# ddemidov/amgcl

Hardware: NVIDIA H100
Metric: cg_iterations_per_second (higher is better)
Workload: dtype f64

## Files before the change

### amgcl_b200/__init__.py

```python
import ctypes
import os

import numpy as np

from . import build as _build

__all__ = ["lib", "dropin_lib", "Context", "Vector", "Csr", "Coarse", "Krylov", "DropinSolver",
           "poisson3d", "unstructured3d", "B200Error", "RELAX", "KRYLOV", "nccl_unique_id",
           "partition", "dist_split", "coarse_lu_plan"]

_c = ctypes
_i64 = _c.c_int64
_dbl = _c.c_double
_vp = _c.c_void_p
_P = _c.POINTER

RELAX = {"damped_jacobi": 0, "spai0": 1, "chebyshev": 2, "ilu0": 3}
KRYLOV = {"cg": 0, "bicgstab": 1, "gmres": 2, "bicgstabl": 3}


class B200Error(RuntimeError):
    pass


class ProfileEntry(_c.Structure):
    _fields_ = [("nrows", _i64), ("ncols", _i64), ("nnz", _i64), ("mode", _c.c_int),
                ("launches", _i64), ("total_ms", _dbl), ("min_ms", _dbl)]


class ProfileFormatEntry(_c.Structure):
    _fields_ = [("entry", ProfileEntry), ("format", _c.c_int), ("value_bytes", _c.c_int)]


FORMAT_NAMES = ("plain", "window", "offset", "pattern", "col16", "col24")


MODE_NAMES = {0: "spmv", 1: "spmv_acc", 2: "residual", 3: "relax", 4: "residual_scaled", 10: "vec1", 11: "vec2",
              12: "vec3", 13: "vec4", 14: "vec5", 15: "vec6", 16: "vec7",
              20: "dot", 21: "relax_zero", 22: "coarse_gemv", 23: "memset", 24: "coarse_tail", 25: "coarse_lu",
              30: "comm"}


_lib = None
_dropin = None


def lib():
    global _lib
    if _lib is not None:
        return _lib
    path = os.environ.get("B200_LIB") or _build.LIB_CUDA
    if not os.path.isfile(path):
        path = _build.build_cuda()
    L = _c.CDLL(path, mode=_c.RTLD_GLOBAL)
    L.b200_last_error.restype = _c.c_char_p
    L.b200_version.restype = _c.c_char_p
    sigs = {
        "b200_device_count": [],
        "b200_ctx_create": [_c.c_int, _P(_vp)],
        "b200_ctx_destroy": [_vp],
        "b200_ctx_default": [_P(_vp)],
        "b200_ctx_set_stream": [_vp, _vp],
        "b200_ctx_get_stream": [_vp, _P(_vp)],
        "b200_ctx_device": [_vp, _P(_c.c_int)],
        "b200_ctx_sync": [_vp],
        "b200_ctx_flush": [_vp],
        "b200_tail_stats": [_vp, _P(_c.c_uint64), _P(_c.c_uint64)],
        "b200_ctx_launch_count": [_vp, _P(_c.c_uint64)],
        "b200_ctx_reset_launch_count": [_vp],
        "b200_ctx_set_option": [_vp, _c.c_char_p, _i64],
        "b200_ctx_get_option": [_vp, _c.c_char_p, _P(_i64)],
        "b200_vec_create": [_vp, _c.c_size_t, _P(_vp)],
        "b200_vec_wrap": [_vp, _vp, _c.c_size_t, _P(_vp)],
        "b200_vec_destroy": [_vp],
        "b200_vec_size": [_vp, _P(_c.c_size_t)],
        "b200_vec_bytes": [_vp, _P(_c.c_size_t)],
        "b200_vec_data": [_vp, _P(_vp)],
        "b200_vec_upload": [_vp, _vp, _c.c_size_t],
        "b200_vec_download": [_vp, _vp, _c.c_size_t],
        "b200_vec_download_local": [_vp, _vp, _c.c_size_t],
        "b200_vec_local_range": [_vp, _P(_c.c_size_t), _P(_c.c_size_t)],
        "b200_vec_create_f32": [_vp, _c.c_size_t, _P(_vp)],
        "b200_vec_upload_f32": [_vp, _vp, _c.c_size_t],
        "b200_vec_download_f32": [_vp, _vp, _c.c_size_t],
        "b200_vec_dtype": [_vp, _P(_c.c_int)],
        "b200_csr_create_i64_f32": [_vp, _i64, _i64, _vp, _vp, _vp, _P(_vp)],
        "b200_csr_create_i32_f32": [_vp, _i64, _i64, _vp, _vp, _vp, _P(_vp)],
        "b200_csr_dtype": [_vp, _P(_c.c_int)],
        "b200_coarse_create_i64_f32": [_vp, _i64, _vp, _vp, _vp, _P(_vp)],
        "b200_coarse_create_i32_f32": [_vp, _i64, _vp, _vp, _vp, _P(_vp)],
        "b200_csr_create_i64": [_vp, _i64, _i64, _vp, _vp, _vp, _P(_vp)],
        "b200_csr_create_i32": [_vp, _i64, _i64, _vp, _vp, _vp, _P(_vp)],
        "b200_csr_destroy": [_vp],
        "b200_csr_rows": [_vp, _P(_c.c_size_t)],
        "b200_csr_cols": [_vp, _P(_c.c_size_t)],
        "b200_csr_nonzeros": [_vp, _P(_c.c_size_t)],
        "b200_csr_bytes": [_vp, _P(_c.c_size_t)],
        "b200_csr_plan": [_vp, _P(_c.c_int), _P(_i64), _P(_i64)],
        "b200_spmv": [_vp, _dbl, _vp, _vp, _dbl, _vp],
        "b200_residual": [_vp, _vp, _vp, _vp, _vp],
        "b200_clear": [_vp, _vp],
        "b200_copy": [_vp, _vp, _vp],
        "b200_dot": [_vp, _vp, _vp, _P(_dbl)],
        "b200_axpby": [_vp, _dbl, _vp, _dbl, _vp],
        "b200_axpbypcz": [_vp, _dbl, _vp, _dbl, _vp, _dbl, _vp],
        "b200_vmul": [_vp, _dbl, _vp, _vp, _dbl, _vp],
        "b200_relax": [_vp, _vp, _vp, _vp, _vp, _vp, _dbl],
        "b200_coarse_create_i64": [_vp, _i64, _vp, _vp, _vp, _P(_vp)],
        "b200_coarse_create_i32": [_vp, _i64, _vp, _vp, _vp, _P(_vp)],
        "b200_coarse_destroy": [_vp],
        "b200_coarse_bytes": [_vp, _P(_c.c_size_t)],
        "b200_coarse_info": [_vp, _P(_c.c_int), _P(_i64), _P(_i64), _P(_i64)],
        "b200_coarse_lu_plan_i64": [_i64, _vp, _vp, _vp, _vp, _vp, _vp, _vp, _i64, _P(_i64), _P(_c.c_int),
                                    _P(_i64), _P(_c.c_size_t), _P(_c.c_size_t)],
        "b200_coarse_solve": [_vp, _vp, _vp, _vp],
        "b200_nccl_unique_id": [_c.c_char_p, _c.c_size_t],
        "b200_dist_init": [_vp, _c.c_char_p, _c.c_size_t, _c.c_int, _c.c_int, _i64],
        "b200_dist_info": [_vp, _P(_c.c_int), _P(_c.c_int), _P(_i64), _P(_c.c_int)],
        "b200_partition": [_i64, _c.c_int, _c.c_int, _P(_i64), _P(_i64), _P(_i64)],
        "b200_dist_split_i64": [_c.c_int, _c.c_int, _c.c_int, _i64, _i64, _vp, _vp, _vp, _P(_vp)],
        "b200_split_info": [_vp, _P(_i64), _P(_i64), _P(_i64), _P(_i64), _P(_i64), _P(_i64)],
        "b200_split_copy": [_vp, _vp, _vp, _vp, _vp],
        "b200_split_destroy": [_vp],
        "b200_plan_i64": [_i64, _vp, _c.c_int, _c.c_int, _vp, _i64, _P(_i64), _P(_c.c_int),
                          _P(_c.c_int), _P(_i64)],
        "b200_ctx_largest_operator": [_vp, _P(_i64), _P(_c.c_int)],
        "b200_csr_patterns": [_vp, _P(_c.c_int), _P(_c.c_int), _P(_c.c_int)],
        "b200_pattern_plan_i64": [_i64, _i64, _vp, _vp, _vp, _vp, _vp, _P(_c.c_int), _P(_c.c_int), _P(_c.c_int)],
        "b200_csr_offsets": [_vp, _P(_c.c_int), _P(_c.c_int)],
        "b200_offset_plan_i64": [_i64, _i64, _vp, _vp, _vp, _vp, _P(_c.c_int), _P(_c.c_int)],
        "b200_csr_narrow": [_vp, _P(_c.c_int)],
        "b200_csr_value_bytes": [_vp, _P(_c.c_int)],
        "b200_values_fit_f32": [_vp, _i64, _P(_c.c_int)],
        "b200_value_index_plan_i64": [_vp, _i64, _vp, _i64, _vp, _P(_c.c_int), _P(_c.c_int)],
        "b200_narrow_plan_i64": [_i64, _i64, _vp, _vp, _c.c_int, _c.c_int, _vp, _i64, _vp, _vp, _vp,
                                 _P(_i64), _P(_c.c_int)],
        "b200_csr_window": [_vp, _P(_c.c_int), _P(_c.c_int), _P(_c.c_int), _P(_i64)],
        "b200_window_plan_i64": [_i64, _i64, _vp, _vp, _c.c_int, _c.c_int, _c.c_int, _c.c_int, _c.c_int, _vp, _vp, _i64,
                                 _vp, _i64, _P(_i64), _P(_i64), _P(_c.c_int), _P(_c.c_int), _P(_c.c_int)],
        "b200_index_create_i64": [_vp, _vp, _c.c_size_t, _c.c_size_t, _P(_vp)],
        "b200_index_destroy": [_vp],
        "b200_index_size": [_vp, _P(_c.c_size_t)],
        "b200_gather": [_vp, _vp, _vp, _vp],
        "b200_gather_host": [_vp, _vp, _vp, _vp],
        "b200_scatter": [_vp, _vp, _vp, _vp],
        "b200_graph_begin": [_vp, _P(_c.c_int)],
        "b200_graph_end": [_vp, _P(_vp)],
        "b200_graph_abort": [_vp],
        "b200_graph_launch": [_vp, _vp, _P(_c.c_int)],
        "b200_graph_info": [_vp, _P(_i64), _P(_i64), _P(_i64), _P(_c.c_int)],
        "b200_graph_destroy": [_vp],
        "b200_krylov_create": [_vp, _c.c_size_t, _P(_vp)],
        "b200_krylov_destroy": [_vp],
        "b200_krylov_residual": [_vp, _vp, _vp, _vp, _vp, _P(_dbl)],
        "b200_krylov_scalars": [_vp, _vp, _c.c_int],
        "b200_cg_direction": [_vp, _vp, _vp, _vp],
        "b200_cg_step": [_vp, _vp, _vp, _vp, _vp, _vp, _P(_dbl)],
        "b200_bicg_start": [_vp, _vp, _vp],
        "b200_bicg_direction": [_vp, _vp, _vp, _vp],
        "b200_bicg_step_s": [_vp, _vp, _vp, _vp, _vp, _vp, _vp, _vp, _P(_dbl), _P(_dbl)],
        "b200_bicg_step_r": [_vp, _vp, _vp, _vp, _vp, _vp, _vp, _vp, _P(_dbl), _P(_dbl)],
        "b200_profile_begin": [_vp],
        "b200_profile_end": [_vp, _vp, _i64, _P(_i64)],
        "b200_profile_end_formats": [_vp, _vp, _i64, _P(_i64)],
    }
    for name, args in sigs.items():
        fn = getattr(L, name)
        fn.argtypes = args
        fn.restype = _c.c_int
    _lib = L
    return L


def dropin_lib():
    global _dropin
    if _dropin is not None:
        return _dropin
    lib()
    path = _build.LIB_DROPIN
    if not os.path.isfile(path):
        path = _build.build_dropin()
    D = _c.CDLL(path)
    D.dropin_last_error.restype = _c.c_char_p
    D.dropin_create.argtypes = [_vp, _i64, _vp, _vp, _vp, _c.c_int, _c.c_int, _dbl, _c.c_int,
                                _c.c_int, _P(_vp)]
    D.dropin_create.restype = _c.c_int
    D.dropin_create_mixed.argtypes = D.dropin_create.argtypes
    D.dropin_create_mixed.restype = _c.c_int
    D.dropin_create_graph.argtypes = [_vp, _i64, _vp, _vp, _vp, _c.c_int, _c.c_int, _c.c_int, _dbl,
                                      _c.c_int, _c.c_int, _P(_vp)]
    D.dropin_create_graph.restype = _c.c_int
    D.dropin_graph_stats.argtypes = [_vp, _P(_i64), _P(_i64), _P(_i64)]
    D.dropin_graph_stats.restype = _c.c_int
    D.dropin_gather_scatter.argtypes = [_vp, _i64, _vp, _i64, _vp, _dbl, _vp, _vp, _vp]
    D.dropin_gather_scatter.restype = _c.c_int
    D.dropin_destroy.argtypes = [_vp]
    D.dropin_destroy.restype = None
    D.dropin_solve.argtypes = [_vp, _vp, _vp, _P(_i64), _P(_dbl)]
    D.dropin_solve.restype = _c.c_int
    D.dropin_solve_zero_guess.argtypes = [_vp, _vp, _vp, _P(_i64), _P(_dbl)]
    D.dropin_solve_zero_guess.restype = _c.c_int
    D.dropin_upload_rhs.argtypes = [_vp, _vp]
    D.dropin_upload_rhs.restype = _c.c_int
    D.dropin_solve_resident.argtypes = [_vp, _P(_i64), _P(_dbl)]
    D.dropin_solve_resident.restype = _c.c_int
    D.dropin_download_x.argtypes = [_vp, _vp]
    D.dropin_download_x.restype = _c.c_int
    D.dropin_apply_precond.argtypes = [_vp, _vp, _vp]
    D.dropin_apply_precond.restype = _c.c_int
    D.dropin_report.argtypes = [_vp, _c.c_char_p, _i64]
    D.dropin_report.restype = _i64
    D.dropin_bytes.argtypes = [_vp]
    D.dropin_bytes.restype = _i64
    D.dropin_set_num_threads.argtypes = [_c.c_int]
    D.dropin_set_num_threads.restype = None
    D.dropin_num_threads.restype = _c.c_int
    _dropin = D
    return D


def _check(rc, what=""):
    if rc != 0:
        msg = lib().b200_last_error().decode(errors="replace")
        raise B200Error("%s failed (%d): %s" % (what or "b200 call", rc, msg))


def _f64(a):
    a = np.ascontiguousarray(a, dtype=np.float64)
    return a


def _ptr(a):
    return a.ctypes.data_as(_vp)


class Context:

    def __init__(self, device=0, stream=None):
        L = lib()
        if L.b200_device_count() <= 0:
            raise B200Error("amgcl_b200 requires a CUDA device (no CPU fallback)")
        self.h = _vp()
        _check(L.b200_ctx_create(int(device), _c.byref(self.h)), "b200_ctx_create")
        if stream is not None:
            self.set_stream(stream)

    def set_stream(self, cuda_stream):
        if cuda_stream is None:
            handle = 0
        else:
            handle = int(cuda_stream) or 1
        _check(lib().b200_ctx_set_stream(self.h, _vp(handle)))

    def sync(self):
        _check(lib().b200_ctx_sync(self.h), "b200_ctx_sync")

    def flush(self):
        _check(lib().b200_ctx_flush(self.h), "b200_ctx_flush")

    def tail_stats(self):
        f, c = _c.c_uint64(), _c.c_uint64()
        _check(lib().b200_tail_stats(self.h, _c.byref(f), _c.byref(c)))
        return f.value, c.value

    def set_option(self, key, value):
        _check(lib().b200_ctx_set_option(self.h, key.encode(), int(value)), "b200_ctx_set_option")

    def get_option(self, key):
        v = _i64()
        _check(lib().b200_ctx_get_option(self.h, key.encode(), _c.byref(v)))
        return v.value

    @property
    def launches(self):
        v = _c.c_uint64()
        _check(lib().b200_ctx_launch_count(self.h, _c.byref(v)))
        return v.value

    def reset_launches(self):
        _check(lib().b200_ctx_reset_launch_count(self.h))

    def dist_init(self, unique_id, nranks, rank, dist_min_rows):
        buf = _c.create_string_buffer(bytes(unique_id), 128)
        _check(lib().b200_dist_init(self.h, buf, 128, int(nranks), int(rank), int(dist_min_rows)),
               "b200_dist_init")

    def dist_info(self):
        r, n, p = _c.c_int(), _c.c_int(), _c.c_int()
        m = _i64()
        _check(lib().b200_dist_info(self.h, _c.byref(r), _c.byref(n), _c.byref(m), _c.byref(p)))
        return {"rank": r.value, "nranks": n.value, "dist_min_rows": m.value, "p2p": bool(p.value)}

    def largest_operator(self):
        nnz, fmt = _i64(), _c.c_int()
        _check(lib().b200_ctx_largest_operator(self.h, _c.byref(nnz), _c.byref(fmt)))
        return nnz.value, FORMAT_NAMES[fmt.value]

    def profile_begin(self):
        _check(lib().b200_profile_begin(self.h), "b200_profile_begin")

    def profile_end(self):
        cap = 256
        buf = (ProfileFormatEntry * cap)()
        cnt = _i64()
        _check(lib().b200_profile_end_formats(self.h, buf, cap, _c.byref(cnt)), "b200_profile_end_formats")
        out = []
        for i in range(min(cap, cnt.value)):
            e, fmt, vb = buf[i].entry, buf[i].format, buf[i].value_bytes
            out.append({"nrows": e.nrows, "ncols": e.ncols, "nnz": e.nnz,
                        "mode": MODE_NAMES.get(e.mode, str(e.mode)), "launches": e.launches,
                        "total_ms": e.total_ms, "min_ms": e.min_ms, "format": FORMAT_NAMES[fmt],
                        "value_bytes": vb})
        return out

    def close(self):
        if self.h:
            lib().b200_ctx_destroy(self.h)
            self.h = _vp()

    def vector(self, data_or_n):
        return Vector(self, data_or_n)

    def csr(self, nrows, ncols, ptr, col, val):
        return Csr(self, nrows, ncols, ptr, col, val)

    def coarse(self, n, ptr, col, val):
        return Coarse(self, n, ptr, col, val)

    def spmv(self, alpha, A, x, beta, y):
        _check(lib().b200_spmv(self.h, alpha, A.h, x.h, beta, y.h), "b200_spmv")

    def residual(self, f, A, x, r):
        _check(lib().b200_residual(self.h, f.h, A.h, x.h, r.h), "b200_residual")

    def clear(self, x):
        _check(lib().b200_clear(self.h, x.h), "b200_clear")

    def copy(self, x, y):
        _check(lib().b200_copy(self.h, x.h, y.h), "b200_copy")

    def dot(self, x, y):
        r = _dbl()
        _check(lib().b200_dot(self.h, x.h, y.h, _c.byref(r)), "b200_dot")
        return r.value

    def axpby(self, a, x, b, y):
        _check(lib().b200_axpby(self.h, a, x.h, b, y.h), "b200_axpby")

    def axpbypcz(self, a, x, b, y, c, z):
        _check(lib().b200_axpbypcz(self.h, a, x.h, b, y.h, c, z.h), "b200_axpbypcz")

    def vmul(self, alpha, x, y, beta, z):
        _check(lib().b200_vmul(self.h, alpha, x.h, y.h, beta, z.h), "b200_vmul")

    def index(self, idx, size):
        return Index(self, idx, size)

    def gather(self, I, src, dst):
        _check(lib().b200_gather(self.h, I.h, src.h, dst.h), "b200_gather")

    def gather_host(self, I, src):
        out = np.empty(I.n, dtype=np.float64)
        _check(lib().b200_gather_host(self.h, I.h, src.h, _ptr(out)), "b200_gather_host")
        return out

    def scatter(self, I, src, dst):
        _check(lib().b200_scatter(self.h, I.h, src.h, dst.h), "b200_scatter")

    def graph_begin(self):
        rec = _c.c_int(0)
        _check(lib().b200_graph_begin(self.h, _c.byref(rec)), "b200_graph_begin")
        return bool(rec.value)

    def graph_end(self):
        g = _vp()
        _check(lib().b200_graph_end(self.h, _c.byref(g)), "b200_graph_end")
        return Graph(self, g)

    def graph_abort(self):
        _check(lib().b200_graph_abort(self.h), "b200_graph_abort")

    def relax(self, A, rhs, x, tmp, diag, omega):
        _check(lib().b200_relax(self.h, A.h, rhs.h, x.h, tmp.h, diag.h, omega), "b200_relax")

    def coarse_solve(self, S, rhs, x):
        _check(lib().b200_coarse_solve(self.h, S.h, rhs.h, x.h), "b200_coarse_solve")


class Krylov:

    SCALARS = ("rho", "qp", "alpha", "ts", "tt", "omega", "rr", "ss", "rho_next")

    def __init__(self, ctx, n):
        self.ctx = ctx
        self.h = _vp()
        _check(lib().b200_krylov_create(ctx.h, int(n), _c.byref(self.h)), "b200_krylov_create")

    def residual(self, rhs, A, x, r):
        out = _dbl()
        _check(lib().b200_krylov_residual(self.h, rhs.h, A.h, x.h, r.h, _c.byref(out)), "b200_krylov_residual")
        return out.value

    def scalars(self):
        buf = (_dbl * 9)()
        _check(lib().b200_krylov_scalars(self.h, buf, 9), "b200_krylov_scalars")
        return dict(zip(self.SCALARS, list(buf)))

    def cg_direction(self, r, s, p):
        _check(lib().b200_cg_direction(self.h, r.h, s.h, p.h), "b200_cg_direction")

    def cg_step(self, A, p, q, x, r):
        out = _dbl()
        _check(lib().b200_cg_step(self.h, A.h, p.h, q.h, x.h, r.h, _c.byref(out)), "b200_cg_step")
        return out.value

    def bicg_start(self, r, rh):
        _check(lib().b200_bicg_start(self.h, r.h, rh.h), "b200_bicg_start")

    def bicg_direction(self, r, v, p):
        _check(lib().b200_bicg_direction(self.h, r.h, v.h, p.h), "b200_bicg_direction")

    def bicg_step_s(self, A, rh, T, v, r, s, x):
        out = _dbl()
        _check(lib().b200_bicg_step_s(self.h, A.h, rh.h, T.h, v.h, r.h, s.h, x.h, _c.byref(out), None),
               "b200_bicg_step_s")
        return out.value

    def bicg_step_r(self, A, rh, T, t, s, r, x):
        out = _dbl()
        _check(lib().b200_bicg_step_r(self.h, A.h, rh.h, T.h, t.h, s.h, r.h, x.h, _c.byref(out), None),
               "b200_bicg_step_r")
        return out.value

    def close(self):
        if self.h:
            lib().b200_krylov_destroy(self.h)
            self.h = _vp()

    def __del__(self):
        try:
            self.close()
        except Exception:
            pass


class Vector:

    def __init__(self, ctx, data_or_n):
        self.ctx = ctx
        self.h = _vp()
        if isinstance(data_or_n, (int, np.integer)):
            self.n = int(data_or_n)
            _check(lib().b200_vec_create(ctx.h, self.n, _c.byref(self.h)), "b200_vec_create")
        else:
            a = _f64(data_or_n)
            self.n = a.size
            _check(lib().b200_vec_create(ctx.h, self.n, _c.byref(self.h)), "b200_vec_create")
            self.upload(a)

    def upload(self, a):
        a = _f64(a)
        _check(lib().b200_vec_upload(self.h, _ptr(a), a.size), "b200_vec_upload")

    def numpy(self):
        out = np.empty(self.n, dtype=np.float64)
        _check(lib().b200_vec_download(self.h, _ptr(out), self.n), "b200_vec_download")
        return out

    def data_ptr(self):
        p = _vp()
        _check(lib().b200_vec_data(self.h, _c.byref(p)))
        return p.value or 0

    def __del__(self):
        try:
            if self.h:
                lib().b200_vec_destroy(self.h)
                self.h = _vp()
        except Exception:
            pass


class Csr:

    def __init__(self, ctx, nrows, ncols, ptr, col, val):
        self.ctx = ctx
        self.h = _vp()
        val = _f64(val)
        ptr = np.ascontiguousarray(ptr)
        col = np.ascontiguousarray(col)
        if ptr.dtype == np.int32 and col.dtype == np.int32:
            fn = lib().b200_csr_create_i32
        else:
            ptr = np.ascontiguousarray(ptr, dtype=np.int64)
            col = np.ascontiguousarray(col, dtype=np.int64)
            fn = lib().b200_csr_create_i64
        _check(fn(ctx.h, int(nrows), int(ncols), _ptr(ptr), _ptr(col), _ptr(val),
                  _c.byref(self.h)), "b200_csr_create")
        self.nrows, self.ncols, self.nnz = int(nrows), int(ncols), int(ptr[-1])

    def plan(self):
        lanes = _c.c_int()
        nb = _i64()
        nl = _i64()
        _check(lib().b200_csr_plan(self.h, _c.byref(lanes), _c.byref(nb), _c.byref(nl)))
        return {"lanes": lanes.value, "blocks": nb.value, "long_blocks": nl.value}

    def bytes(self):
        b = _c.c_size_t()
        _check(lib().b200_csr_bytes(self.h, _c.byref(b)))
        return b.value

    def patterns(self):
        on, cnt, tot = _c.c_int(), _c.c_int(), _c.c_int()
        _check(lib().b200_csr_patterns(self.h, _c.byref(on), _c.byref(cnt), _c.byref(tot)))
        return {"pattern_indexed": bool(on.value), "count": cnt.value, "total": tot.value}

    def offsets(self):
        on, cnt = _c.c_int(), _c.c_int()
        _check(lib().b200_csr_offsets(self.h, _c.byref(on), _c.byref(cnt)))
        return {"offset_indexed": bool(on.value), "count": cnt.value}

    def narrow(self):
        w = _c.c_int()
        _check(lib().b200_csr_narrow(self.h, _c.byref(w)))
        return w.value

    def value_bytes(self):
        b = _c.c_int()
        _check(lib().b200_csr_value_bytes(self.h, _c.byref(b)))
        return b.value

    def window(self):
        w, ms, mr, tot = _c.c_int(), _c.c_int(), _c.c_int(), _i64()
        _check(lib().b200_csr_window(self.h, _c.byref(w), _c.byref(ms), _c.byref(mr), _c.byref(tot)))
        return {"windowed": bool(w.value), "max_slots": ms.value, "max_runs": mr.value, "total_slots": tot.value}

    def __del__(self):
        try:
            if self.h and lib().b200_csr_destroy(self.h) == 0:
                self.h = _vp()
        except Exception:
            pass


def pattern_plan(nrows, ncols, ptr, col):
    ptr = np.ascontiguousarray(ptr, dtype=np.int64)
    col = np.ascontiguousarray(col, dtype=np.int64)
    pid = np.zeros(max(1, nrows), dtype=np.uint8)
    start = np.zeros(257, dtype=np.uint16)
    off = np.zeros(1024, dtype=np.int32)
    cnt, tot, ok = _c.c_int(), _c.c_int(), _c.c_int()
    _check(lib().b200_pattern_plan_i64(nrows, ncols, ptr.ctypes.data, col.ctypes.data, pid.ctypes.data,
                                       start.ctypes.data, off.ctypes.data, _c.byref(cnt), _c.byref(tot),
                                       _c.byref(ok)))
    if not ok.value:
        return None
    return {"pid": pid[:nrows], "start": start, "off": off, "count": cnt.value, "total": tot.value}


def offset_plan(nrows, ncols, ptr, col):
    ptr = np.ascontiguousarray(ptr, dtype=np.int64)
    col = np.ascontiguousarray(col, dtype=np.int64)
    nnz = int(ptr[-1]) if nrows else 0
    idx8 = np.zeros(max(1, nnz), dtype=np.uint8)
    tab = np.zeros(256, dtype=np.int32)
    cnt, ok = _c.c_int(), _c.c_int()
    _check(lib().b200_offset_plan_i64(nrows, ncols, ptr.ctypes.data, col.ctypes.data, idx8.ctypes.data,
                                      tab.ctypes.data, _c.byref(cnt), _c.byref(ok)))
    if not ok.value:
        return None
    return {"idx8": idx8[:nnz], "tab": tab, "count": cnt.value}


def narrow_plan(nrows, ncols, ptr, col, lanes=0, nnz_cap=2048):
    ptr = np.ascontiguousarray(ptr, dtype=np.int64)
    col = np.ascontiguousarray(col, dtype=np.int64)
    nnz = int(ptr[-1]) if nrows else 0
    cap = nrows // 4 + 2 + (nnz // 256 + 1)
    base = np.zeros(cap, dtype=np.int32)
    lo16 = np.zeros(max(1, nnz), dtype=np.uint16)
    hi8 = np.zeros(max(1, nnz), dtype=np.uint8)
    ptr16 = np.zeros(max(1, nrows), dtype=np.uint16)
    nb, w = _i64(), _c.c_int()
    _check(lib().b200_narrow_plan_i64(nrows, ncols, ptr.ctypes.data, col.ctypes.data, int(lanes), int(nnz_cap),
                                      base.ctypes.data, cap, lo16.ctypes.data, hi8.ctypes.data,
                                      ptr16.ctypes.data, _c.byref(nb), _c.byref(w)))
    out = {"nblocks": nb.value, "ptr16": ptr16[:nrows], "width": w.value}
    if w.value:
        out.update(base=base[:nb.value], lo16=lo16[:nnz])
        if w.value == 24:
            out["hi8"] = hi8[:nnz]
    return out


def values_fit_f32(val):
    val = np.ascontiguousarray(val, dtype=np.float64)
    ok = _c.c_int()
    _check(lib().b200_values_fit_f32(val.ctypes.data, val.size, _c.byref(ok)))
    return bool(ok.value)


def value_index_plan(val):
    val = np.ascontiguousarray(val, dtype=np.float64)
    tab = np.zeros(4096, dtype=np.float64)
    idx = np.zeros(max(1, 2 * val.size), dtype=np.uint8)
    cnt, w = _c.c_int(), _c.c_int()
    _check(lib().b200_value_index_plan_i64(val.ctypes.data, val.size, tab.ctypes.data, tab.size,
                                            idx.ctypes.data, _c.byref(cnt), _c.byref(w)))
    out = {"width": w.value, "count": cnt.value}
    if w.value:
        out["table"] = tab[:cnt.value]
        out["index"] = idx[:val.size] if w.value == 8 else idx[:2 * val.size].view(np.uint16)
    return out


def window_plan(nrows, ncols, ptr, col, lanes=0, nnz_cap=2048, slot_cap=1400, max_ratio=75, gap=2):
    ptr = np.ascontiguousarray(ptr, dtype=np.int64)
    col = np.ascontiguousarray(col, dtype=np.int64)
    nnz = int(ptr[-1]) if nrows else 0
    nb, nr = _i64(), _i64()
    ms, mr, ok = _c.c_int(), _c.c_int(), _c.c_int()
    L = lib()
    _check(L.b200_window_plan_i64(nrows, ncols, ptr.ctypes.data, col.ctypes.data, lanes, nnz_cap, slot_cap,
                                  max_ratio, gap, None, None, 0, None, 0, _c.byref(nb), _c.byref(nr),
                                  _c.byref(ms), _c.byref(mr), _c.byref(ok)))
    if not ok.value:
        return None
    blk = np.zeros((nb.value, 6), dtype=np.int32)
    runs = np.zeros((max(1, nr.value), 2), dtype=np.int32)
    col16 = np.zeros(max(1, nnz), dtype=np.uint16)
    _check(L.b200_window_plan_i64(nrows, ncols, ptr.ctypes.data, col.ctypes.data, lanes, nnz_cap, slot_cap,
                                  max_ratio, gap, col16.ctypes.data, runs.ctypes.data, runs.shape[0],
                                  blk.ctypes.data, blk.shape[0], _c.byref(nb), _c.byref(nr),
                                  _c.byref(ms), _c.byref(mr), _c.byref(ok)))
    return {"blk": blk, "runs": runs[:nr.value], "col16": col16[:nnz], "max_slots": ms.value,
            "max_runs": mr.value}


def coarse_lu_plan(n, ptr, col):
    L = lib()
    n = int(n)
    ptr = np.ascontiguousarray(ptr, dtype=np.int64)
    col = np.ascontiguousarray(col, dtype=np.int64)
    tiles, rows, bw = _i64(), _c.c_int(), _i64()
    fb, sb = _c.c_size_t(), _c.c_size_t()
    _check(L.b200_coarse_lu_plan_i64(n, _ptr(ptr), _ptr(col), None, None, None, None, None, 0,
                                     _c.byref(tiles), _c.byref(rows), _c.byref(bw), _c.byref(fb),
                                     _c.byref(sb)), "b200_coarse_lu_plan_i64")
    perm = np.empty(n, dtype=np.int32)
    lower = np.empty(n, dtype=np.int32)
    upper = np.empty(n, dtype=np.int32)
    lfirst = np.empty(tiles.value, dtype=np.int64)
    ulast = np.empty(tiles.value, dtype=np.int64)
    _check(L.b200_coarse_lu_plan_i64(n, _ptr(ptr), _ptr(col), _ptr(perm), _ptr(lower), _ptr(upper),
                                     _ptr(lfirst), _ptr(ulast), tiles.value, None, None, None, None, None),
           "b200_coarse_lu_plan_i64")
    return {"perm": perm, "lower": lower, "upper": upper, "lfirst": lfirst, "ulast": ulast,
            "tile_rows": rows.value, "bandwidth": bw.value, "factor_bytes": fb.value,
            "setup_bytes": sb.value}


class Coarse:

    def __init__(self, ctx, n, ptr, col, val):
        self.ctx = ctx
        self.h = _vp()
        ptr = np.ascontiguousarray(ptr, dtype=np.int64)
        col = np.ascontiguousarray(col, dtype=np.int64)
        val = _f64(val)
        _check(lib().b200_coarse_create_i64(ctx.h, int(n), _ptr(ptr), _ptr(col), _ptr(val),
                                            _c.byref(self.h)), "b200_coarse_create")
        self.n = int(n)

    COARSE_KINDS = ("dense_inverse", "banded_lu")

    def info(self):
        k, n, bw, t = _c.c_int(), _i64(), _i64(), _i64()
        _check(lib().b200_coarse_info(self.h, _c.byref(k), _c.byref(n), _c.byref(bw), _c.byref(t)),
               "b200_coarse_info")
        return {"kind": self.COARSE_KINDS[k.value], "n": n.value, "bandwidth": bw.value, "tiles": t.value}

    def bytes(self):
        b = _c.c_size_t()
        _check(lib().b200_coarse_bytes(self.h, _c.byref(b)), "b200_coarse_bytes")
        return b.value

    def __del__(self):
        try:
            if self.h and lib().b200_coarse_destroy(self.h) == 0:
                self.h = _vp()
        except Exception:
            pass


class Index:

    def __init__(self, ctx, idx, size):
        idx = np.ascontiguousarray(idx, dtype=np.int64)
        self.ctx = ctx
        self.n = idx.size
        self.h = _vp()
        _check(lib().b200_index_create_i64(ctx.h, _ptr(idx), idx.size, int(size), _c.byref(self.h)),
               "b200_index_create_i64")

    def __del__(self):
        try:
            if self.h and lib().b200_index_destroy(self.h) == 0:
                self.h = _vp()
        except Exception:
            pass


class Graph:

    def __init__(self, ctx, h):
        self.ctx = ctx
        self.h = h

    def launch(self):
        ok = _c.c_int(0)
        _check(lib().b200_graph_launch(self.ctx.h, self.h, _c.byref(ok)), "b200_graph_launch")
        return bool(ok.value)

    def info(self):
        k, n, r, st = _i64(), _i64(), _i64(), _c.c_int(0)
        _check(lib().b200_graph_info(self.h, _c.byref(k), _c.byref(n), _c.byref(r), _c.byref(st)))
        return {"kernels": k.value, "nodes": n.value, "replays": r.value, "stale": bool(st.value)}

    def close(self):
        if self.h:
            lib().b200_graph_destroy(self.h)
            self.h = _vp()

    def __del__(self):
        try:
            self.close()
        except Exception:
            pass


class DropinSolver:

    def __init__(self, ptr, col, val, relax="damped_jacobi", krylov="cg", tol=1e-8,
                 maxiter=100, coarse_enough=-1, ctx=None, precision="f64", graph=False):
        D = dropin_lib()
        self.ptr = np.ascontiguousarray(ptr, dtype=np.int64)
        self.col = np.ascontiguousarray(col, dtype=np.int64)
        self.val = _f64(val)
        self.n = self.ptr.size - 1
        self.ctx = ctx
        self.h = _vp()
        if graph:
            rc = D.dropin_create_graph(ctx.h if ctx is not None else None, self.n, _ptr(self.ptr),
                                       _ptr(self.col), _ptr(self.val), RELAX[relax], KRYLOV[krylov],
                                       1 if precision == "mixed" else 0, float(tol), int(maxiter),
                                       int(coarse_enough), _c.byref(self.h))
        else:
            create = D.dropin_create_mixed if precision == "mixed" else D.dropin_create
            rc = create(ctx.h if ctx is not None else None, self.n, _ptr(self.ptr),
                        _ptr(self.col), _ptr(self.val), RELAX[relax], KRYLOV[krylov],
                        float(tol), int(maxiter), int(coarse_enough), _c.byref(self.h))
        if rc != 0:
            raise B200Error("dropin_create: " + D.dropin_last_error().decode(errors="replace"))

    def _err(self, what):
        raise B200Error(what + ": " + dropin_lib().dropin_last_error().decode(errors="replace"))

    def solve(self, rhs, x0=None):
        rhs = _f64(rhs)
        x = np.zeros(self.n) if x0 is None else _f64(x0).copy()
        it = _i64()
        res = _dbl()
        if dropin_lib().dropin_solve(self.h, _ptr(rhs), _ptr(x), _c.byref(it), _c.byref(res)):
            self._err("dropin_solve")
        return x, it.value, res.value

    def solve_into(self, rhs, x):
        it = _i64()
        res = _dbl()
        if dropin_lib().dropin_solve(self.h, _ptr(rhs), _ptr(x), _c.byref(it), _c.byref(res)):
            self._err("dropin_solve")
        return it.value, res.value

    def solve_zero_guess_into(self, rhs, x_out):
        it = _i64()
        res = _dbl()
        if dropin_lib().dropin_solve_zero_guess(self.h, _ptr(rhs), _ptr(x_out), _c.byref(it),
                                                _c.byref(res)):
            self._err("dropin_solve_zero_guess")
        return it.value, res.value

    def upload_rhs(self, rhs):
        rhs = _f64(rhs)
        if dropin_lib().dropin_upload_rhs(self.h, _ptr(rhs)):
            self._err("dropin_upload_rhs")

    def solve_resident(self):
        it = _i64()
        res = _dbl()
        if dropin_lib().dropin_solve_resident(self.h, _c.byref(it), _c.byref(res)):
            self._err("dropin_solve_resident")
        return it.value, res.value

    def download_x(self):
        x = np.empty(self.n)
        if dropin_lib().dropin_download_x(self.h, _ptr(x)):
            self._err("dropin_download_x")
        return x

    def apply_precond(self, f):
        f = _f64(f)
        x = np.empty(self.n)
        if dropin_lib().dropin_apply_precond(self.h, _ptr(f), _ptr(x)):
            self._err("dropin_apply_precond")
        return x

    def graph_stats(self):
        g, k, r = _i64(), _i64(), _i64()
        dropin_lib().dropin_graph_stats(self.h, _c.byref(g), _c.byref(k), _c.byref(r))
        return g.value, k.value, r.value

    def report(self):
        need = dropin_lib().dropin_report(self.h, None, 0)
        buf = _c.create_string_buffer(int(need))
        dropin_lib().dropin_report(self.h, buf, need)
        return buf.value.decode(errors="replace")

    def close(self):
        if self.h:
            dropin_lib().dropin_destroy(self.h)
            self.h = _vp()

    def __del__(self):
        try:
            self.close()
        except Exception:
            pass


def set_setup_threads(n):
    dropin_lib().dropin_set_num_threads(int(n))


def nccl_unique_id():
    buf = _c.create_string_buffer(128)
    _check(lib().b200_nccl_unique_id(buf, 128), "b200_nccl_unique_id")
    return bytes(buf.raw)


def partition(n, nranks, rank):
    b, lo, hi = _i64(), _i64(), _i64()
    _check(lib().b200_partition(int(n), int(nranks), int(rank), _c.byref(b), _c.byref(lo),
                                _c.byref(hi)), "b200_partition")
    return b.value, lo.value, hi.value


def dist_split(kind, nranks, rank, nrows, ncols, ptr, col, val):
    k = {"halo": 1, "square": 1, "replicated": 2}[kind]
    ptr = np.ascontiguousarray(ptr, dtype=np.int64)
    col = np.ascontiguousarray(col, dtype=np.int64)
    val = _f64(val)
    h = _vp()
# ... 82 lines not shown
```

### amgcl_b200/csrc/api_context.cu

```cuda
#include "internal.cuh"

#include <mutex>

namespace b200 {

static thread_local std::string g_last_error;

void set_error(const std::string &msg) { g_last_error = msg; }

int fail(int code, const std::string &msg) {
    g_last_error = msg;
    return code;
}

int cuda_fail(cudaError_t rc, const char *what, const char *file, int line) {
    char buf[512];
    snprintf(buf, sizeof(buf), "CUDA error %d (%s) in %s at %s:%d", (int)rc,
             cudaGetErrorString(rc), what, file, line);
    g_last_error = buf;
    cudaGetLastError();
    return rc == cudaErrorMemoryAllocation ? B200_ENOMEM : B200_ECUDA;
}

}

using namespace b200;

extern "C" const char *b200_last_error(void) { return g_last_error.c_str(); }

extern "C" const char *b200_version(void) { return "amgcl_b200 0.1.0 sm_90a"; }

extern "C" int b200_device_count(void) {
    int n = 0;
    if (cudaGetDeviceCount(&n) != cudaSuccess) {
        cudaGetLastError();
        return 0;
    }
    return n;
}

static int ctx_init(b200_ctx_t ctx, int device) {
    cudaDeviceProp prop;
    B200_CUDA(cudaGetDeviceProperties(&prop, device));
    ctx->sm_count = prop.multiProcessorCount;
    if (prop.major != 9 || prop.minor != 0)
        return fail(B200_ECUDA, "amgcl_b200 needs an sm_90a (Hopper H100) device");
    B200_CUDA(cudaStreamCreateWithFlags(&ctx->own_stream, cudaStreamNonBlocking));
    ctx->stream = ctx->own_stream;
    B200_CUDA(cudaMalloc(&ctx->dot_partial, kDotMaxBlocks * sizeof(double)));
    B200_CUDA(cudaMalloc(&ctx->dot_ticket, sizeof(unsigned int)));
    B200_CUDA(cudaMemset(ctx->dot_ticket, 0, sizeof(unsigned int)));
    B200_CUDA(cudaHostAlloc(&ctx->dot_result_h, 8 * sizeof(double), cudaHostAllocMapped));
    B200_CUDA(cudaHostGetDevicePointer(&ctx->dot_result_d, ctx->dot_result_h, 0));
    B200_CUDA(cudaMalloc(&ctx->dot_dev, 2 * sizeof(double)));
    return scal_create(ctx);
}

extern "C" int b200_ctx_create(int device, b200_ctx_t *out) {
    B200_REQUIRE(out != nullptr, "null output pointer");
    *out = nullptr;
    int ndev = 0;
    B200_CUDA(cudaGetDeviceCount(&ndev));
    if (device < 0 || device >= ndev) return fail(B200_EINVAL, "no such CUDA device");
    DeviceGuard guard(device);
    if (!guard.ok) return fail(B200_ECUDA, "cudaSetDevice failed");

    b200_ctx_s *ctx = new (std::nothrow) b200_ctx_s();
    if (!ctx) return fail(B200_ENOMEM, "out of host memory");
    ctx->device = device;
    if (const char *e = getenv("B200_PDL")) ctx->opt_pdl = atoi(e) ? 1 : 0;
    if (const char *e = getenv("B200_CYCLE_GRAPH")) ctx->opt_cycle_graph = atoi(e) ? 1 : 0;
    if (const char *e = getenv("B200_GRAPH_PDL")) ctx->opt_graph_pdl = atoi(e) ? 1 : 0;
    if (const char *e = getenv("B200_FUSED_KRYLOV")) ctx->opt_fused_krylov = atoi(e) ? 1 : 0;
    if (const char *e = getenv("B200_COARSE_TAIL")) ctx->opt_coarse_tail = atoi(e) ? 1 : 0;
    if (const char *e = getenv("B200_FUSE_FIRST_SWEEP")) ctx->opt_fuse_first_sweep = atoi(e) ? 1 : 0;
    if (const char *e = getenv("B200_POLL_SCALARS")) ctx->opt_poll_scalars = atoi(e) ? 1 : 0;
    if (const char *e = getenv("B200_PATTERNS")) ctx->opt_patterns = atoi(e) ? 1 : 0;
    if (const char *e = getenv("B200_PATTERNS_MIN_NNZ")) ctx->opt_patterns_min_nnz = atoll(e);
    if (const char *e = getenv("B200_OFFSETS")) ctx->opt_offsets = atoi(e) ? 1 : 0;
    if (const char *e = getenv("B200_OFFSETS_MIN_NNZ")) ctx->opt_offsets_min_nnz = atoll(e);
    if (const char *e = getenv("B200_NARROW_COLUMNS")) ctx->opt_narrow = atoi(e) ? 1 : 0;
    if (const char *e = getenv("B200_NARROW_VALUES")) ctx->opt_narrow_values = atoi(e) ? 1 : 0;
    if (const char *e = getenv("B200_WINDOW")) ctx->opt_window = atoi(e) ? 1 : 0;
    if (const char *e = getenv("B200_WINDOW_MIN_NNZ")) ctx->opt_window_min_nnz = atoll(e);
    if (const char *e = getenv("B200_WINDOW_GAP")) ctx->opt_window_gap = std::max(1, std::min(8, atoi(e)));
    if (const char *e = getenv("B200_WINDOW_RATIO")) ctx->opt_window_ratio = atoll(e);
    if (const char *e = getenv("B200_WINDOW_LANES")) ctx->opt_window_lanes = atoll(e) & 15;
    if (const char *e = getenv("B200_SMALL_KERNEL_MAX_NNZ")) ctx->opt_small_kernel_max_nnz = atoll(e);
    const int rc = ctx_init(ctx, device);
    if (rc != B200_OK) {
        const std::string msg = g_last_error;
        b200_ctx_destroy(ctx);
        g_last_error = msg;
        return rc;
    }
    *out = ctx;
    return B200_OK;
}

extern "C" int b200_ctx_destroy(b200_ctx_t ctx) {
    if (!ctx) return B200_OK;
    tail_destroy(ctx);
    ctx->lazy_vec = nullptr;
    GUARD(ctx);
    if (ctx->stream) cudaStreamSynchronize(ctx->stream);
    scal_destroy(ctx);
    tail_destroy(ctx);
    for (int k = 0; k < 2; ++k) {
        if (ctx->stage_host[k]) cudaFreeHost(ctx->stage_host[k]);
        if (ctx->stage_event[k]) cudaEventDestroy(ctx->stage_event[k]);
    }
    if (ctx->gather_ticket) cudaFree(ctx->gather_ticket);
    if (ctx->scal_x_local) {
        for (int q = 0; q < ctx->nranks; ++q)
            if (q != ctx->rank && ctx->scal_x_peer[q]) cudaIpcCloseMemHandle(ctx->scal_x_peer[q]);
        cudaFree(ctx->scal_x_local);
    }
    if (ctx->dot_partial) cudaFree(ctx->dot_partial);
    if (ctx->dot_ticket) cudaFree(ctx->dot_ticket);
    if (ctx->dot_result_h) cudaFreeHost(ctx->dot_result_h);
    if (ctx->dot_dev) cudaFree(ctx->dot_dev);
    if (ctx->push_ticket) cudaFree(ctx->push_ticket);
    if (ctx->ipc_dev) cudaFree(ctx->ipc_dev);
    if (ctx->probe_pb_local) {
        for (int q = 0; q < ctx->nranks; ++q)
            if (q != ctx->rank && ctx->probe_pb_peer[q]) cudaIpcCloseMemHandle(ctx->probe_pb_peer[q]);
        cudaFree(ctx->probe_pb_local);
    }
    for (void *ptr : ctx->deferred_free) cudaFree(ptr);
    if (ctx->comm && nccl().handle) nccl().CommDestroy(comm_of(ctx));
    if (ctx->own_stream) cudaStreamDestroy(ctx->own_stream);
    for (cudaEvent_t e : ctx->prof_events) cudaEventDestroy(e);
    delete ctx;
    return B200_OK;
}

extern "C" int b200_ctx_default(b200_ctx_t *out) {
    B200_REQUIRE(out != nullptr, "null output pointer");
    static std::mutex mtx;
    static b200_ctx_t def = nullptr;
    std::lock_guard<std::mutex> lock(mtx);
    if (!def) {
        int dev = 0;
        B200_CUDA(cudaGetDevice(&dev));
        int rc = b200_ctx_create(dev, &def);
        if (rc != B200_OK) return rc;
    }
    *out = def;
    return B200_OK;
}

extern "C" int b200_ctx_set_stream(b200_ctx_t ctx, void *cuda_stream) {
    CHECK_CTX(ctx);
    NOT_RECORDING(ctx, "stream change");
    {
        GUARD(ctx);
    }
    ctx->option_epoch++;
    ctx->stream = cuda_stream ? static_cast<cudaStream_t>(cuda_stream) : ctx->own_stream;
    return B200_OK;
}

extern "C" int b200_ctx_get_stream(b200_ctx_t ctx, void **cuda_stream) {
    CHECK_CTX(ctx);
    B200_REQUIRE(cuda_stream != nullptr, "null output pointer");
    *cuda_stream = ctx->stream;
    return B200_OK;
}

extern "C" int b200_ctx_device(b200_ctx_t ctx, int *device) {
    CHECK_CTX(ctx);
    B200_REQUIRE(device != nullptr, "null output pointer");
    *device = ctx->device;
    return B200_OK;
}

extern "C" int b200_ctx_sync(b200_ctx_t ctx) {
    CHECK_CTX(ctx);
    NOT_RECORDING(ctx, "sync");
    GUARD(ctx);
    B200_CUDA(cudaStreamSynchronize(ctx->stream));
    return B200_OK;
}

extern "C" int b200_ctx_flush(b200_ctx_t ctx) {
    CHECK_CTX(ctx);
    GUARD(ctx);
    return B200_OK;
}

extern "C" int b200_ctx_launch_count(b200_ctx_t ctx, uint64_t *count) {
    CHECK_CTX(ctx);
    B200_REQUIRE(count != nullptr, "null output pointer");
    *count = ctx->launches;
    return B200_OK;
}

extern "C" int b200_ctx_reset_launch_count(b200_ctx_t ctx) {
    CHECK_CTX(ctx);
    ctx->launches = 0;
    return B200_OK;
}

extern "C" int b200_profile_begin(b200_ctx_t ctx) {
    CHECK_CTX(ctx);
    NOT_RECORDING(ctx, "profiling");
    {
        GUARD(ctx);
    }
    ctx->prof_used = 0;
    ctx->prof_recs.clear();
    ctx->profiling = true;
    return B200_OK;
}

static int profile_collect(b200_ctx_t ctx, std::vector<b200_profile_format_entry> &agg) {
    GUARD(ctx);
    ctx->profiling = false;
    B200_CUDA(cudaStreamSynchronize(ctx->stream));
    for (const auto &r : ctx->prof_recs) {
        float ms = 0.f;
        B200_CUDA(cudaEventElapsedTime(&ms, ctx->prof_events[r.ev], ctx->prof_events[r.ev + 1]));
        b200_profile_format_entry *hit = nullptr;
        for (auto &a : agg)
            if (a.entry.nrows == r.nrows && a.entry.ncols == r.ncols && a.entry.nnz == r.nnz &&
                a.entry.mode == r.mode && a.format == r.fmt && a.value_bytes == r.vbytes) {
                hit = &a;
                break;
            }
        if (!hit) {
            agg.push_back({{r.nrows, r.ncols, r.nnz, r.mode, 0, 0.0, 1e30}, r.fmt, r.vbytes});
            hit = &agg.back();
        }
        hit->entry.launches += 1;
        hit->entry.total_ms += ms;
        if (ms < hit->entry.min_ms) hit->entry.min_ms = ms;
    }
    ctx->prof_recs.clear();
    ctx->prof_used = 0;
    return B200_OK;
}

extern "C" int b200_profile_end(b200_ctx_t ctx, b200_profile_entry *out, int64_t capacity,
                                int64_t *count) {
    CHECK_CTX(ctx);
    B200_REQUIRE(count != nullptr, "null output pointer");
    std::vector<b200_profile_format_entry> agg;
    const int rc = profile_collect(ctx, agg);
    if (rc) return rc;
    *count = (int64_t)agg.size();
    if (out) {
        const int64_t m = std::min<int64_t>(capacity, (int64_t)agg.size());
        for (int64_t i = 0; i < m; ++i) out[i] = agg[(size_t)i].entry;
    }
    return B200_OK;
}

extern "C" int b200_profile_end_formats(b200_ctx_t ctx, b200_profile_format_entry *out, int64_t capacity,
                                        int64_t *count) {
    CHECK_CTX(ctx);
    B200_REQUIRE(count != nullptr, "null output pointer");
    std::vector<b200_profile_format_entry> agg;
    const int rc = profile_collect(ctx, agg);
    if (rc) return rc;
    *count = (int64_t)agg.size();
    if (out) {
        const int64_t m = std::min<int64_t>(capacity, (int64_t)agg.size());
        for (int64_t i = 0; i < m; ++i) out[i] = agg[(size_t)i];
    }
    return B200_OK;
}


static int64_t *option_slot(b200_ctx_t ctx, const char *key) {
    if (!key) return nullptr;
    if (!strcmp(key, "spmv_variant")) return &ctx->opt_spmv_variant;
    if (!strcmp(key, "fuse_relax")) return &ctx->opt_fuse_relax;
    if (!strcmp(key, "zero_shortcut")) return &ctx->opt_zero_shortcut;
    if (!strcmp(key, "nnz_cap")) return &ctx->opt_nnz_cap;
    if (!strcmp(key, "lanes")) return &ctx->opt_lanes;
    if (!strcmp(key, "ctas_per_sm")) return &ctx->opt_ctas_per_sm;
    if (!strcmp(key, "stages")) return &ctx->opt_stages;
    if (!strcmp(key, "p2p")) return &ctx->opt_p2p;
    if (!strcmp(key, "pdl")) return &ctx->opt_pdl;
    if (!strcmp(key, "cycle_graph")) return &ctx->opt_cycle_graph;
    if (!strcmp(key, "graph_pdl")) return &ctx->opt_graph_pdl;
    if (!strcmp(key, "fused_krylov")) return &ctx->opt_fused_krylov;
    if (!strcmp(key, "coarse_tail")) return &ctx->opt_coarse_tail;
    if (!strcmp(key, "poll_scalars")) return &ctx->opt_poll_scalars;
    if (!strcmp(key, "small_kernel_max_nnz")) return &ctx->opt_small_kernel_max_nnz;
    if (!strcmp(key, "patterns")) return &ctx->opt_patterns;
    if (!strcmp(key, "patterns_min_nnz")) return &ctx->opt_patterns_min_nnz;
    if (!strcmp(key, "offsets")) return &ctx->opt_offsets;
    if (!strcmp(key, "offsets_min_nnz")) return &ctx->opt_offsets_min_nnz;
    if (!strcmp(key, "narrow_columns")) return &ctx->opt_narrow;
    if (!strcmp(key, "narrow_values")) return &ctx->opt_narrow_values;
    if (!strcmp(key, "narrow_values_min_nnz")) return &ctx->opt_narrow_values_min_nnz;
    if (!strcmp(key, "window")) return &ctx->opt_window;
    if (!strcmp(key, "window_min_nnz")) return &ctx->opt_window_min_nnz;
    if (!strcmp(key, "window_ratio")) return &ctx->opt_window_ratio;
    if (!strcmp(key, "window_gap")) return &ctx->opt_window_gap;
    if (!strcmp(key, "window_lanes")) return &ctx->opt_window_lanes;
    if (!strcmp(key, "fuse_first_sweep")) return &ctx->opt_fuse_first_sweep;
    if (!strcmp(key, "tail_max_nnz")) return &ctx->opt_tail_max_nnz;
    if (!strcmp(key, "tail_max_vec")) return &ctx->opt_tail_max_vec;
    return nullptr;
}

extern "C" int b200_ctx_set_option(b200_ctx_t ctx, const char *key, int64_t value) {
    CHECK_CTX(ctx);
    int64_t *slot = option_slot(ctx, key);
    if (!slot) return fail(B200_EINVAL, std::string("unknown option: ") + (key ? key : "(null)"));
    if (slot == &ctx->opt_nnz_cap) {
        if (value < 256 || value > kNnzCapMax || (value % 8))
            return fail(B200_EINVAL, "nnz_cap must be a multiple of 8 in [256, 6144]");
    } else if (slot == &ctx->opt_lanes) {
        if (value != 0 && (value < 1 || value > 32 || (value & (value - 1))))
            return fail(B200_EINVAL, "lanes must be 0 (auto) or a power of two <= 32");
    } else if (slot == &ctx->opt_stages) {
        if (value < 1 || value > 8) return fail(B200_EINVAL, "stages must be in [1, 8]");
    } else if (slot == &ctx->opt_ctas_per_sm) {
        if (value < 1 || value > 8) return fail(B200_EINVAL, "ctas_per_sm must be in [1, 8]");
    } else if (slot == &ctx->opt_spmv_variant) {
        if (value < 0 || value > 1) return fail(B200_EINVAL, "spmv_variant must be 0 or 1");
    }
    B200_REQUIRE(!ctx->recording, "options cannot change while a graph is being recorded");
    {
        GUARD(ctx);
    }
    if (*slot != value) ctx->option_epoch++;
    *slot = value;
    return B200_OK;
}

extern "C" int b200_ctx_get_option(b200_ctx_t ctx, const char *key, int64_t *value) {
    CHECK_CTX(ctx);
    B200_REQUIRE(value != nullptr, "null output pointer");
    int64_t *slot = option_slot(ctx, key);
    if (!slot) return fail(B200_EINVAL, std::string("unknown option: ") + (key ? key : "(null)"));
    *value = *slot;
    return B200_OK;
}

namespace b200 {
static void graph_free(b200_graph_s *g) {
    if (!g) return;
    if (g->exec) cudaGraphExecDestroy(g->exec);
    if (g->graph) cudaGraphDestroy(g->graph);
    delete g;
}
static void graph_release_deferred(b200_ctx_t ctx) {
    for (void *p : ctx->graph_deferred) cudaFree(p);
    ctx->graph_deferred.clear();
}
static void graph_rollback(b200_graph_s *g) {
    for (const GraphSlot &s : g->slots) {
        *s.slot = s.p0;
        if (s.zp) *s.zp = s.z0;
        if (s.gen) ++*s.gen;
    }
}
}

extern "C" int b200_graph_begin(b200_ctx_t ctx, int *recording) {
    CHECK_CTX(ctx);
    B200_REQUIRE(recording != nullptr, "null output pointer");
    B200_REQUIRE(!ctx->recording, "graph_begin: already recording");
    *recording = 0;
    if (ctx->profiling || ctx->dist || !ctx->opt_cycle_graph) return B200_OK;
    if (ctx->stream == nullptr || ctx->stream == cudaStreamLegacy) return B200_OK;
    GUARD(ctx);
    b200_graph_s *g = new (std::nothrow) b200_graph_s();
    if (!g) return fail(B200_ENOMEM, "out of host memory");
    g->ctx = ctx;
    g->destroy_epoch = ctx->destroy_epoch;
    g->option_epoch = ctx->option_epoch;
    g->launches0 = ctx->launches;
    const cudaError_t rc = cudaStreamBeginCapture(ctx->stream, cudaStreamCaptureModeRelaxed);
    if (rc != cudaSuccess) {
        delete g;
        return cuda_fail(rc, "cudaStreamBeginCapture", __FILE__, __LINE__);
    }
    ctx->recording = g;
    *recording = 1;
    return B200_OK;
}

extern "C" int b200_graph_abort(b200_ctx_t ctx) {
    CHECK_CTX(ctx);
    b200_graph_s *g = ctx->recording;
    if (!g) return B200_OK;
    GUARD(ctx);
    cudaGraph_t junk = nullptr;
    cudaStreamEndCapture(ctx->stream, &junk);
    if (junk) cudaGraphDestroy(junk);
    cudaGetLastError();
    graph_rollback(g);
    ctx->launches = g->launches0;
    ctx->recording = nullptr;
    graph_free(g);
    graph_release_deferred(ctx);
    return B200_OK;
}

extern "C" int b200_graph_end(b200_ctx_t ctx, b200_graph_t *out) {
    CHECK_CTX(ctx);
    B200_REQUIRE(out != nullptr, "null output pointer");
    *out = nullptr;
    b200_graph_s *g = ctx->recording;
    B200_REQUIRE(g != nullptr, "graph_end: not recording");
    GUARD(ctx);
    ctx->recording = nullptr;
    cudaError_t rc = cudaStreamEndCapture(ctx->stream, &g->graph);
    if (rc == cudaSuccess) rc = cudaGraphInstantiate(&g->exec, g->graph, 0);
    if (rc == cudaSuccess) rc = cudaGraphGetNodes(g->graph, nullptr, &g->nodes);
    if (rc == cudaSuccess) rc = cudaGraphLaunch(g->exec, ctx->stream);
    if (rc != cudaSuccess) {
        cudaGetLastError();
        graph_rollback(g);
        ctx->launches = g->launches0;
        graph_free(g);
        graph_release_deferred(ctx);
        return cuda_fail(rc, "graph_end (capture / instantiate / launch)", __FILE__, __LINE__);
    }
    graph_release_deferred(ctx);
    for (GraphSlot &s : g->slots) {
        s.p1 = *s.slot;
        s.z1 = s.zp ? *s.zp : false;
    }
    g->launches = ctx->launches - g->launches0;
    *out = g;
    return B200_OK;
}

extern "C" int b200_graph_launch(b200_ctx_t ctx, b200_graph_t g, int *launched) {
    CHECK_CTX(ctx);
    B200_REQUIRE(g && launched, "null argument");
    *launched = 0;
    B200_REQUIRE(g->ctx == ctx, "graph belongs to another context");
    B200_REQUIRE(!ctx->recording, "graph_launch: a graph is being recorded");
    if (ctx->profiling || !ctx->opt_cycle_graph) return B200_OK;
    if (g->destroy_epoch != ctx->destroy_epoch || g->option_epoch != ctx->option_epoch)
        return B200_OK;
    for (const GraphSlot &s : g->slots)
        if (*s.slot != s.p0 || (s.zp && *s.zp != s.z0)) return B200_OK;
    GUARD(ctx);
    B200_CUDA(cudaGraphLaunch(g->exec, ctx->stream));
    for (const GraphSlot &s : g->slots) {
        *s.slot = s.p1;
        if (s.zp) *s.zp = s.z1;
        if (s.gen) ++*s.gen;
    }
    for (const GraphProduct &p : g->products) product_record(ctx, p.a, p.b, p.slot);
    ctx->launches += g->launches;
    g->replays++;
    *launched = 1;
    return B200_OK;
}

extern "C" int b200_graph_info(b200_graph_t g, int64_t *kernels, int64_t *nodes, int64_t *replays,
                               int *stale) {
    B200_REQUIRE(g != nullptr, "null argument");
    if (kernels) *kernels = (int64_t)g->launches;
    if (nodes) *nodes = (int64_t)g->nodes;
    if (replays) *replays = (int64_t)g->replays;
    if (stale)
        *stale = (g->destroy_epoch != g->ctx->destroy_epoch || g->option_epoch != g->ctx->option_epoch);
    return B200_OK;
}

extern "C" int b200_graph_destroy(b200_graph_t g) {
    if (!g) return B200_OK;
    GUARD(g->ctx);
    graph_free(g);
    return B200_OK;
}
```

### amgcl_b200/csrc/api_matrices.cu

```cuda
#include "internal.cuh"
#include "csr_kernels.cuh"
#include "csr_launch.cuh"
#include "window.cuh"
#include "offsets.cuh"
#include "patterns.cuh"
#include "narrow.cuh"
#include "values.cuh"

namespace b200 {
int tail_enqueue_csr(b200_ctx_t ctx, int mode, b200_csr_t A, const CsrArgsT<PrecDD> &a);
bool small_csr_accepts(b200_ctx_t ctx, b200_csr_t A);
int small_csr_launch(b200_ctx_t ctx, int mode, b200_csr_t A, const CsrArgsT<PrecDD> &a);
}

using namespace b200;

namespace b200 {

static int choose_lanes(double avg) {
    if (avg <= 12.0) return 1;
    if (avg <= 40.0) return 2;
    if (avg <= 64.0) return 4;
    if (avg <= 160.0) return 8;
    if (avg <= 320.0) return 16;
    return 32;
}

struct RowBlockPlan {
    int lanes = 1, rows_cap = 256, nnz_cap = 2048;
    int64_t nlong = 0;
    std::vector<int2> blk;
};

template <class Ptr>
static void build_plan(int64_t nrows, const Ptr *ptr, int lanes_opt, int nnz_cap,
                       RowBlockPlan &plan) {
    const int64_t nnz = nrows ? (int64_t)ptr[nrows] : 0;
    const double avg = nrows ? (double)nnz / (double)nrows : 0.0;
    const int lanes = lanes_opt ? lanes_opt : choose_lanes(avg);
    const int groups = kThreads / lanes;
    int k = 1;
    if (avg > 0.0) k = (int)std::floor((double)nnz_cap / (avg * groups));
    k = std::max(1, std::min(k, kRowsCapMax / groups));
    int rows_cap = std::min(kRowsCapMax, groups * k);
    rows_cap = std::max(4, rows_cap & ~3);
    plan.lanes = lanes; plan.rows_cap = rows_cap; plan.nnz_cap = nnz_cap; plan.nlong = 0;
    plan.blk.clear();
    plan.blk.reserve((size_t)(nnz / std::max(1, nnz_cap / 2) + nrows / rows_cap + 16));
    int64_t r = 0;
    while (r < nrows) {
        const int64_t r0 = r;
        const int64_t e0 = (int64_t)ptr[r0];
        int64_t r1 = std::min<int64_t>(nrows, r0 + 4);
        while (r1 < nrows) {
            const int64_t rn = std::min<int64_t>(nrows, r1 + 4);
            if (rn - r0 > rows_cap) break;
            if ((int64_t)ptr[rn] - e0 > nnz_cap) break;
            r1 = rn;
        }
        if ((int64_t)ptr[r1] - e0 > nnz_cap) ++plan.nlong;
        plan.blk.push_back(make_int2((int)r0, (int)e0));
        r = r1;
    }
    plan.blk.push_back(make_int2((int)nrows, (int)nnz));
}

template <class Ptr, class Col>
static int csr_validate(int64_t nrows, int64_t ncols, const Ptr *ptr, const Col *col, bool have_val) {
    B200_REQUIRE(nrows >= 0 && ncols >= 0, "negative matrix dimension");
    B200_REQUIRE(ptr != nullptr, "null row pointer array");
    const int64_t imax = std::numeric_limits<int32_t>::max();
    if (nrows >= imax - 8 || ncols >= imax) return fail(B200_ERANGE, "matrix dimension exceeds int32");
    B200_REQUIRE(ptr[0] == 0, "ptr[0] must be 0");
    for (int64_t i = 1; i <= nrows; ++i)
        if ((int64_t)ptr[i] < (int64_t)ptr[i - 1]) return fail(B200_EINVAL, "row pointers not monotone");
    const int64_t nnz = (int64_t)ptr[nrows];
    if (nnz < 0) return fail(B200_EINVAL, "negative number of non-zeros");
    if (nnz >= imax - 8) return fail(B200_ERANGE, "number of non-zeros exceeds int32");
    B200_REQUIRE(nnz == 0 || (col != nullptr && have_val), "null col/val array");
    int bad = 0;
#pragma omp parallel for reduction(| : bad) schedule(static)
    for (int64_t e = 0; e < nnz; ++e) {
        const int64_t c = (int64_t)col[e];
        bad |= (c < 0 || c >= ncols) ? 1 : 0;
    }
    if (bad) return fail(B200_EINVAL, "column index out of range");
    return B200_OK;
}

template <class Dst, class Src>
static cudaError_t staged_upload(b200_ctx_t ctx, Dst *dst, const Src *src, size_t count) {
    const size_t stage_bytes = (size_t)32 << 20;
    cudaError_t rc = cudaSuccess;
    for (int k = 0; k < 2 && rc == cudaSuccess; ++k) {
        if (!ctx->stage_host[k]) rc = cudaHostAlloc(&ctx->stage_host[k], stage_bytes, cudaHostAllocDefault);
        if (rc == cudaSuccess && !ctx->stage_event[k])
            rc = cudaEventCreateWithFlags(&ctx->stage_event[k], cudaEventDisableTiming);
    }
    if (rc != cudaSuccess) return rc;
    const size_t chunk = stage_bytes / sizeof(Dst);
    int k = 0;
    for (size_t off = 0; off < count && rc == cudaSuccess; off += chunk, k ^= 1) {
        const size_t m = std::min(chunk, count - off);
        rc = cudaEventSynchronize(ctx->stage_event[k]);
        if (rc != cudaSuccess) break;
        Dst *buf = static_cast<Dst *>(ctx->stage_host[k]);
        const Src *from = src + off;
#pragma omp parallel for schedule(static)
        for (int64_t i = 0; i < (int64_t)m; ++i) buf[i] = (Dst)from[i];
        rc = cudaMemcpyAsync(dst + off, buf, m * sizeof(Dst), cudaMemcpyHostToDevice, ctx->stream);
        if (rc == cudaSuccess) rc = cudaEventRecord(ctx->stage_event[k], ctx->stream);
    }
    return rc;
}

static bool values_fit_f32(const double *val, int64_t n) {
    int bad = 0;
#pragma omp parallel for reduction(| : bad) schedule(static)
    for (int64_t e = 0; e < n; ++e) {
        const double w = (double)(float)val[e];
        uint64_t a, b;
        memcpy(&a, val + e, 8);
        memcpy(&b, &w, 8);
        bad |= a != b ? 1 : 0;
    }
    return !bad;
}

template <class Ptr, class Col, class Val>
static int csr_upload(b200_ctx_t ctx, int64_t nrows, int64_t ncols, const Ptr *ptr,
                      const Col *col, const Val *val, b200_csr_t *out, int64_t halo_from = -1) {
    CHECK_CTX(ctx);
    B200_REQUIRE(out != nullptr, "null output pointer");
    *out = nullptr;
    int vrc = csr_validate(nrows, ncols, ptr, col, val != nullptr);
    if (vrc) return vrc;
    const int64_t nnz = (int64_t)ptr[nrows];
    GUARD(ctx);

    std::vector<int32_t> hptr((size_t)nrows + 1);
#pragma omp parallel for schedule(static)
    for (int64_t i = 0; i <= nrows; ++i) hptr[(size_t)i] = (int32_t)ptr[i];

    RowBlockPlan plan;
    build_plan(nrows, hptr.data(), (int)ctx->opt_lanes, (int)ctx->opt_nnz_cap, plan);
    const int lanes = plan.lanes, rows_cap = plan.rows_cap, nnz_cap = plan.nnz_cap;
    const int64_t nlong = plan.nlong;
    std::vector<int2> &blk = plan.blk;
    int64_t nblocks = (int64_t)blk.size() - 1;

    std::vector<int4> blk4((size_t)nblocks + 1);
    if (halo_from >= 0 && nblocks > 0) {
        std::vector<char> outer((size_t)nblocks, 0);
#pragma omp parallel for schedule(dynamic, 64)
        for (int64_t b = 0; b < nblocks; ++b) {
            bool halo = false;
            for (int64_t e = blk[(size_t)b].y; e < blk[(size_t)b + 1].y && !halo; ++e)
                halo = (int64_t)col[e] >= halo_from;
            outer[(size_t)b] = halo;
        }
        size_t k = 0;
        for (int pass = 0; pass < 2; ++pass)
            for (int64_t b = 0; b < nblocks; ++b)
                if (outer[(size_t)b] == pass) {
                    const int2 lo = blk[(size_t)b], hi = blk[(size_t)b + 1];
                    blk4[k++] = make_int4(pass ? ~lo.x : lo.x, hi.x, lo.y, hi.y);
                }
    } else {
        for (int64_t b = 0; b < nblocks; ++b)
            blk4[(size_t)b] = make_int4(blk[(size_t)b].x, blk[(size_t)b + 1].x, blk[(size_t)b].y, blk[(size_t)b + 1].y);
    }
    blk4[(size_t)nblocks] = make_int4((int)nrows, (int)nrows, (int)nnz, (int)nnz);

    PatternPlan patp;
    const bool pattern_indexed = ctx->opt_patterns && nnz >= ctx->opt_patterns_min_nnz && nlong == 0 &&
                                 lanes <= 4 && build_patterns(nrows, hptr.data(), col, patp);

    OffsetPlan offp;
    const bool offset_indexed = !pattern_indexed && ctx->opt_offsets && nnz >= ctx->opt_offsets_min_nnz && nlong == 0 && lanes <= 4 &&
                                build_offsets(nrows, hptr.data(), col, offp);

    WindowPlan win;
    bool windowed = false;
    if (!offset_indexed && ctx->opt_window && nnz >= ctx->opt_window_min_nnz && nlong == 0 && lanes <= 8 &&
        ((ctx->opt_window_lanes >> (lanes == 1 ? 0 : lanes == 2 ? 1 : lanes == 4 ? 2 : 3)) & 1)) {
        const StageLayout wl = stage_layout(rows_cap, nnz_cap, (int)sizeof(Val), FMT_WINDOW, kWinRunCapMax);
        const int budget = ring_budget(4) - kHeaderBytes - 2 * wl.bytes;
        const int slot_cap = std::min(8192, (budget / 8) & ~3);
        windowed = build_windows(blk4.data(), nblocks, hptr.data(), col, ncols, nnz, slot_cap, kWinRunCapMax,
                                 (double)ctx->opt_window_ratio / 100.0, (int)ctx->opt_window_gap, win);
        if (windowed) {
            blk4.swap(win.blk4);
            nblocks = (int64_t)blk4.size() - 1;
        }
    }

    NarrowPlan nar;
    const bool narrowed = !pattern_indexed && !offset_indexed && !windowed && ctx->opt_narrow && nlong == 0 &&
                          lanes <= 8 && build_narrow(blk4.data(), nblocks, col, nnz, nar);

    bool values32 = false;
    if constexpr (std::is_same<Val, double>::value)
        values32 = ctx->opt_narrow_values && nnz >= ctx->opt_narrow_values_min_nnz && values_fit_f32(val, nnz);

    ValueIndexPlan vip;
    bool indexed = false;
    if constexpr (std::is_same<Val, double>::value) {
        const int fmt = pattern_indexed ? FMT_PATTERN : offset_indexed ? FMT_OFFSET
                      : narrowed ? (nar.width == 24 ? FMT_COL24 : FMT_COL16) : FMT_PLAIN;
        indexed = !values32 && ctx->opt_narrow_values && nnz > 0 && nnz >= ctx->opt_narrow_values_min_nnz &&
                  nlong == 0 && !windowed && !ctx->dist && build_value_index(val, nnz, vip) &&
                  value_index_fits(ctx, rows_cap, nnz_cap, fmt, vip.width / 8, vip.count);
    }

    std::vector<unsigned short> ptr16((size_t)nrows, 0);
    build_ptr16(blk4.data(), nblocks, hptr.data(), nnz_cap, ptr16);

    b200_csr_s *A = new (std::nothrow) b200_csr_s();
    if (!A) return fail(B200_ENOMEM, "out of host memory");
    A->ctx = ctx; A->nrows = nrows; A->ncols = ncols; A->nnz = nnz;
    A->gl_rows = nrows; A->gl_cols = ncols; A->gl_nnz = nnz;
    A->dtype = std::is_same<Val, float>::value ? B200_F32 : B200_F64;
    A->lanes = lanes; A->rows_cap = rows_cap; A->nnz_cap = nnz_cap;
    A->nblocks = nblocks; A->nlong = nlong;
    {
        const int rw = 32 / lanes;
        int64_t few = 0;
        for (int64_t b = 0; b < nblocks; ++b) {
            const int4 q = blk4[(size_t)b];
            const int nr = q.y - (q.x < 0 ? ~q.x : q.x);
            if (q.w - q.z <= nnz_cap && (nr + rw - 1) / rw < kThreads / 32) ++few;
        }
        A->row_stream = 2 * few > nblocks;
    }
    const size_t ptr_bytes = ((size_t)nrows + 1 + 8) * sizeof(int);
    const size_t col_bytes = ((size_t)nnz + 8) * sizeof(int);
    const size_t val_bytes = ((size_t)nnz + 8) * sizeof(Val);
    const size_t v32_bytes = values32 ? ((size_t)nnz + 8) * sizeof(float) : 0;
    const size_t vix_bytes = indexed ? (((size_t)nnz + 32) * (size_t)(vip.width / 8) + 15) & ~(size_t)15 : 0;
    const size_t vtb_bytes = indexed ? (size_t)vip.count * sizeof(double) : 0;
    const size_t blk_bytes = ((size_t)nblocks + 1) * sizeof(int4);
    const size_t c16_bytes = windowed ? ((size_t)nnz + 16) * sizeof(unsigned short) : 0;
    const size_t run_bytes = windowed ? (win.runs.size() + 4) * sizeof(int2) : 0;
    const size_t wbk_bytes = windowed ? ((size_t)nblocks + 1) * sizeof(int2) : 0;
    const size_t ix8_bytes = offset_indexed ? (((size_t)nnz + 32 + 15) & ~(size_t)15) : 0;
    const size_t tab_bytes = offset_indexed ? kOffTabLen * sizeof(int) : 0;
    const size_t pid_bytes = pattern_indexed ? (((size_t)nrows + 32 + 15) & ~(size_t)15) : 0;
    const size_t pat_bytes = pattern_indexed ? kPatOffCap * sizeof(int) + (kPatCap + 1 + 7) * sizeof(unsigned short) : 0;
    const size_t p16_bytes = ((size_t)nrows + 16) * sizeof(unsigned short);
    const size_t lo_bytes  = narrowed ? ((size_t)nnz + 16) * sizeof(unsigned short) : 0;
    const size_t hi_bytes  = narrowed && nar.width == 24 ? (((size_t)nnz + 32 + 15) & ~(size_t)15) : 0;
    const size_t cb_bytes  = narrowed ? ((size_t)nblocks + 1) * sizeof(int) : 0;
    auto cleanup = [&]() {
        if (A->ptr) cudaFree(A->ptr);
        if (A->col) cudaFree(A->col);
        if (A->val) cudaFree(A->val);
        if (A->val32) cudaFree(A->val32);
        if (A->vidx) cudaFree(A->vidx);
        if (A->vtab) cudaFree(A->vtab);
        if (A->blk) cudaFree(A->blk);
        if (A->col16) cudaFree(A->col16);
        if (A->wrun) cudaFree(A->wrun);
        if (A->wblk) cudaFree(A->wblk);
        if (A->idx8) cudaFree(A->idx8);
        if (A->off_tab) cudaFree(A->off_tab);
        if (A->pid) cudaFree(A->pid);
        if (A->pat_start) cudaFree(A->pat_start);
        if (A->pat_off) cudaFree(A->pat_off);
        if (A->ptr16) cudaFree(A->ptr16);
        if (A->clo16) cudaFree(A->clo16);
        if (A->chi8) cudaFree(A->chi8);
        if (A->cbase) cudaFree(A->cbase);
        delete A;
    };
#define CSR_CUDA(call)                                                         \
    do {                                                                       \
        cudaError_t rc__ = (call);                                             \
        if (rc__ != cudaSuccess) {                                             \
            cleanup();                                                         \
            return cuda_fail(rc__, #call, __FILE__, __LINE__);                 \
        }                                                                      \
    } while (0)
    CSR_CUDA(cudaMalloc(&A->ptr, ptr_bytes));
    CSR_CUDA(cudaMalloc(&A->col, col_bytes));
    CSR_CUDA(cudaMalloc(&A->val, val_bytes));
    CSR_CUDA(cudaMalloc(&A->blk, blk_bytes));
    CSR_CUDA(cudaMemsetAsync(A->ptr, 0, ptr_bytes, ctx->stream));
    CSR_CUDA(cudaMemsetAsync(A->col, 0, col_bytes, ctx->stream));
    CSR_CUDA(cudaMemsetAsync(A->val, 0, val_bytes, ctx->stream));
    CSR_CUDA(staged_upload(ctx, A->ptr, hptr.data(), (size_t)nrows + 1));
    if (nnz) {
        CSR_CUDA(staged_upload(ctx, A->col, col, (size_t)nnz));
        CSR_CUDA(staged_upload(ctx, static_cast<Val *>(A->val), val, (size_t)nnz));
    }
    if (values32) {
        CSR_CUDA(cudaMalloc(&A->val32, v32_bytes));
        CSR_CUDA(cudaMemsetAsync(A->val32, 0, v32_bytes, ctx->stream));
        CSR_CUDA(staged_upload(ctx, A->val32, val, (size_t)nnz));
    }
    if (indexed) {
        CSR_CUDA(cudaMalloc(&A->vidx, vix_bytes));
        CSR_CUDA(cudaMalloc(&A->vtab, vtb_bytes));
        CSR_CUDA(cudaMemsetAsync(A->vidx, 0, vix_bytes, ctx->stream));
        if (vip.width == 8) CSR_CUDA(staged_upload(ctx, static_cast<unsigned char *>(A->vidx), vip.idx8.data(), (size_t)nnz));
        else CSR_CUDA(staged_upload(ctx, static_cast<unsigned short *>(A->vidx), vip.idx16.data(), (size_t)nnz));
        CSR_CUDA(staged_upload(ctx, reinterpret_cast<uint64_t *>(A->vtab), vip.tab.data(), (size_t)vip.count));
        A->vidx_bytes = vip.width / 8;
        A->vtab_n = vip.count;
    }
    CSR_CUDA(cudaMemcpyAsync(A->blk, blk4.data(), blk_bytes, cudaMemcpyHostToDevice, ctx->stream));
    CSR_CUDA(cudaMalloc(&A->ptr16, p16_bytes));
    CSR_CUDA(cudaMemsetAsync(A->ptr16, 0, p16_bytes, ctx->stream));
    if (nrows) CSR_CUDA(staged_upload(ctx, A->ptr16, ptr16.data(), (size_t)nrows));
    if (narrowed) {
        CSR_CUDA(cudaMalloc(&A->clo16, lo_bytes));
        CSR_CUDA(cudaMalloc(&A->cbase, cb_bytes));
        CSR_CUDA(cudaMemsetAsync(A->clo16, 0, lo_bytes, ctx->stream));
        CSR_CUDA(cudaMemsetAsync(A->cbase, 0, cb_bytes, ctx->stream));
        CSR_CUDA(staged_upload(ctx, A->clo16, nar.lo16.data(), (size_t)nnz));
        CSR_CUDA(staged_upload(ctx, A->cbase, nar.base.data(), (size_t)nblocks));
        if (nar.width == 24) {
            CSR_CUDA(cudaMalloc(&A->chi8, hi_bytes));
            CSR_CUDA(cudaMemsetAsync(A->chi8, 0, hi_bytes, ctx->stream));
            CSR_CUDA(staged_upload(ctx, A->chi8, nar.hi8.data(), (size_t)nnz));
        }
        A->narrow = nar.width;
    }
    if (windowed) {
        CSR_CUDA(cudaMalloc(&A->col16, c16_bytes));
        CSR_CUDA(cudaMalloc(&A->wrun, run_bytes));
        CSR_CUDA(cudaMalloc(&A->wblk, wbk_bytes));
        CSR_CUDA(cudaMemsetAsync(A->col16, 0, c16_bytes, ctx->stream));
        CSR_CUDA(cudaMemsetAsync(A->wrun, 0, run_bytes, ctx->stream));
        CSR_CUDA(cudaMemsetAsync(A->wblk, 0, wbk_bytes, ctx->stream));
        CSR_CUDA(staged_upload(ctx, A->col16, win.col16.data(), (size_t)nnz));
        if (!win.runs.empty()) CSR_CUDA(staged_upload(ctx, A->wrun, win.runs.data(), win.runs.size()));
        CSR_CUDA(staged_upload(ctx, A->wblk, win.wblk.data(), (size_t)nblocks));
        A->win_slots = (win.max_slots + 3) & ~3;
        A->win_runs = win.max_runs;
        A->win_total = win.total_slots;
    }
    if (offset_indexed) {
        CSR_CUDA(cudaMalloc(&A->idx8, ix8_bytes));
        CSR_CUDA(cudaMalloc(&A->off_tab, tab_bytes));
        CSR_CUDA(cudaMemsetAsync(A->idx8, 0, ix8_bytes, ctx->stream));
        CSR_CUDA(staged_upload(ctx, A->idx8, offp.idx8.data(), (size_t)nnz));
        CSR_CUDA(staged_upload(ctx, A->off_tab, offp.tab, (size_t)kOffTabLen));
        A->off_count = offp.count;
    }
    if (pattern_indexed) {
        CSR_CUDA(cudaMalloc(&A->pid, pid_bytes));
        CSR_CUDA(cudaMalloc(&A->pat_start, (kPatCap + 1 + 7) * sizeof(unsigned short)));
        CSR_CUDA(cudaMalloc(&A->pat_off, kPatOffCap * sizeof(int)));
        CSR_CUDA(cudaMemsetAsync(A->pid, 0, pid_bytes, ctx->stream));
        CSR_CUDA(staged_upload(ctx, A->pid, patp.pid.data(), (size_t)nrows));
        CSR_CUDA(staged_upload(ctx, A->pat_start, patp.start.data(), (size_t)kPatCap + 1));
        CSR_CUDA(staged_upload(ctx, A->pat_off, patp.off.data(), (size_t)kPatOffCap));
        A->pat_count = patp.count;
        A->pat_total = patp.total;
    }
    CSR_CUDA(cudaStreamSynchronize(ctx->stream));
#undef CSR_CUDA
    A->bytes = ptr_bytes + col_bytes + val_bytes + v32_bytes + vix_bytes + vtb_bytes + blk_bytes + c16_bytes + run_bytes + wbk_bytes + ix8_bytes +
               tab_bytes + pid_bytes + pat_bytes + p16_bytes + lo_bytes + hi_bytes + cb_bytes;
    if (nnz > ctx->big_nnz) {
        ctx->big_nnz = nnz;
        ctx->big_fmt = stored_format(A);
    }
    *out = A;
    return B200_OK;
}

static void csr_free(b200_csr_t A) {
    if (!A) return;
    if (A->ptr) cudaFree(A->ptr);
    if (A->col) cudaFree(A->col);
    if (A->val) cudaFree(A->val);
    if (A->val32) cudaFree(A->val32);
    if (A->vidx) cudaFree(A->vidx);
    if (A->vtab) cudaFree(A->vtab);
    if (A->blk) cudaFree(A->blk);
    if (A->col16) cudaFree(A->col16);
    if (A->wrun) cudaFree(A->wrun);
    if (A->wblk) cudaFree(A->wblk);
    if (A->idx8) cudaFree(A->idx8);
    if (A->off_tab) cudaFree(A->off_tab);
    if (A->pid) cudaFree(A->pid);
    if (A->pat_start) cudaFree(A->pat_start);
    if (A->pat_off) cudaFree(A->pat_off);
    if (A->ptr16) cudaFree(A->ptr16);
    if (A->clo16) cudaFree(A->clo16);
    if (A->chi8) cudaFree(A->chi8);
    if (A->cbase) cudaFree(A->cbase);
    if (A->send_idx) cudaFree(A->send_idx);
    if (A->halo_owned) cudaFree(A->halo_owned);
    if (A->ybuf) cudaFree(A->ybuf);
    if (A->scratch64) cudaFree(A->scratch64);
    if (A->pb_local) peer_release(A->ctx, A->pb_local, A->pb_peer);
    if (A->gb_local) peer_release(A->ctx, A->gb_local, A->gb_peer);
    delete A;
}

template <class Ptr, class Col, class Val>
static int csr_create(b200_ctx_t ctx, int64_t nrows, int64_t ncols, const Ptr *ptr,
                      const Col *col, const Val *val, b200_csr_t *out) {
    CHECK_CTX(ctx);
    NOT_RECORDING(ctx, "matrix creation");
    B200_REQUIRE(out != nullptr, "null output pointer");
    *out = nullptr;
    if (!ctx->dist) return csr_upload(ctx, nrows, ncols, ptr, col, val, out);

    int rc = csr_validate(nrows, ncols, ptr, col, val != nullptr);
    if (rc) return rc;
    const int64_t nnz = (int64_t)ptr[nrows];
    const int64_t T = ctx->dist_min_rows;
    const bool rd = nrows >= T, cd = ncols >= T;
    if (!rd && !cd) return csr_upload(ctx, nrows, ncols, ptr, col, val, out);
    GUARD(ctx);

    const int P = ctx->nranks, rank = ctx->rank;
    const Partition rows(nrows, P), cols(ncols, P);
    SplitMatrix sp;
    split_rows(rows, cols, cd, rank, ptr, col, sp);

    b200_csr_t A = nullptr;
    rc = csr_upload(ctx, sp.nrows, sp.ncols, sp.ptr.data(), sp.col.data(), val + sp.val_offset, &A,
                     cd ? sp.n_loc : (int64_t)-1);
    if (rc) return rc;
    A->kind = cd ? B200_CK_HALO : B200_CK_LOCAL;
    A->gl_rows = nrows; A->gl_cols = ncols; A->gl_nnz = nnz;
    A->rows_dist = rd; A->cols_dist = cd;
    A->gather_rows = !rd;
    A->row_off = rows.lo(rank); A->row_B = rows.B;
    A->n_loc = sp.n_loc;
#define DCSR_CUDA(call)                                                        \
    do {                                                                       \
        cudaError_t rc__ = (call);                                             \
        if (rc__ != cudaSuccess) {                                             \
            csr_free(A);                                                       \
            return cuda_fail(rc__, #call, __FILE__, __LINE__);                 \
        }                                                                      \
    } while (0)
    if (cd) {
        A->S = sp.S;
        A->n_send = (int64_t)sp.send_idx.size();
        std::vector<int32_t> idx(sp.send_idx.begin(), sp.send_idx.end());
        DCSR_CUDA(cudaMalloc(&A->send_idx, std::max<size_t>(1, idx.size()) * sizeof(int)));
        const size_t halo_n = std::max<size_t>(2, (size_t)(P * sp.S));
        DCSR_CUDA(cudaMalloc(&A->halo_owned, halo_n * sizeof(double)));
        A->halo = A->halo_owned;
        DCSR_CUDA(cudaMemsetAsync(A->halo, 0, halo_n * sizeof(double), ctx->stream));
        if (!idx.empty())
            DCSR_CUDA(cudaMemcpyAsync(A->send_idx, idx.data(), idx.size() * sizeof(int),
                                      cudaMemcpyHostToDevice, ctx->stream));
        A->bytes += idx.size() * sizeof(int) + (size_t)(P * sp.S) * sizeof(double);
        for (int q = 0; q < P; ++q)
            A->xchg[q] = q != rank && (sp.dep[(size_t)rank * P + q] || sp.dep[(size_t)q * P + rank]);
    }
    if (A->gather_rows && !ctx->p2p) {
        DCSR_CUDA(cudaMalloc((void **)&A->ybuf, ((size_t)P * (size_t)rows.B + 2) * sizeof(double)));
        DCSR_CUDA(cudaMemsetAsync(A->ybuf, 0, ((size_t)P * (size_t)rows.B + 2) * sizeof(double), ctx->stream));
        A->bytes += (size_t)P * (size_t)rows.B * sizeof(double);
    }
    DCSR_CUDA(cudaStreamSynchronize(ctx->stream));
#undef DCSR_CUDA
    if (ctx->p2p) {
        if (cd) {
            size_t half = (size_t)P * (size_t)A->S * sizeof(double);
            half = (std::max<size_t>(half, 16) + 255) & ~size_t(255);
            A->pb_half = half;
            rc = peer_alloc(ctx, kFlagBytes + 2 * half, &A->pb_local, A->pb_peer);
            if (rc) {
                csr_free(A);
                return rc;
            }
            A->bytes += kFlagBytes + 2 * half;
        }
        if (A->gather_rows) {
            size_t half = (size_t)P * (size_t)rows.B * sizeof(double);
            half = (std::max<size_t>(half, 16) + 255) & ~size_t(255);
            A->gb_half = half;
            rc = peer_alloc(ctx, kFlagBytes + 2 * half, &A->gb_local, A->gb_peer);
            if (rc) {
                csr_free(A);
                return rc;
            }
            A->bytes += kFlagBytes + 2 * half;
        }
    }
    *out = A;
    return B200_OK;
}

template <int MODE, int L, bool HALO, class P>
static int launch_csr_LH(b200_ctx_t ctx, b200_csr_t A, const CsrArgsT<P> &args) {
    constexpr bool fp64 = std::is_same<P, PrecDD>::value;
    const StageLayout lay = stage_layout(A->rows_cap, A->nnz_cap, (int)sizeof(typename P::TV));
    if (fp64 && ctx->opt_spmv_variant == 0 && !HALO) {
        const int smem = kHeaderBytes + lay.bytes;
        static bool attr_set[64] = {};
        if (!attr_set[ctx->device & 63]) {
            B200_CUDA(cudaFuncSetAttribute(csr_block_kernel<MODE, L, HALO, PrecDD>,
                                           cudaFuncAttributeMaxDynamicSharedMemorySize, 200 * 1024));
            attr_set[ctx->device & 63] = true;
        }
        csr_block_kernel<MODE, L, HALO, PrecDD><<<(unsigned)A->nblocks, kThreads, smem, ctx->stream>>>(
            *reinterpret_cast<const CsrArgsT<PrecDD> *>(&args));
    } else {
        int rc = B200_OK;
        bool done = false;
        const int fmt = launch_format<P>(ctx, A);
        if constexpr (L <= 4) {
            if (fmt == FMT_PATTERN) {
                rc = launch_ring_pat<MODE, L, HALO, P>(ctx, A, args);
                done = true;
            }
        }
        if constexpr (L <= 4) {
            if (fmt == FMT_OFFSET) {
                rc = launch_ring_off<MODE, L, HALO, P>(ctx, A, args);
                done = true;
            }
        }
        if constexpr (L <= 8 && !IndexedValues<typename P::TV>::value) {
            if (fmt == FMT_WINDOW) {
                rc = launch_ring_win<MODE, L, HALO, P>(ctx, A, args);
                done = true;
            }
        }
        if constexpr (L <= 8) {
            if (fmt == FMT_COL16) {
                rc = launch_ring_c16<MODE, L, HALO, P>(ctx, A, args);
                done = true;
            }
            if (fmt == FMT_COL24) {
                rc = launch_ring_c24<MODE, L, HALO, P>(ctx, A, args);
                done = true;
            }
        }
        if (!done) rc = launch_ring_impl<MODE, L, HALO, P, FMT_PLAIN>(ctx, A, args);
        if (rc) return rc;
    }
    B200_CHECK_LAUNCH();
    ctx->launches++;
    return B200_OK;
}

template <int MODE, int L, class P>
static int launch_csr_L(b200_ctx_t ctx, b200_csr_t A, const CsrArgsT<P> &args) {
    if constexpr (!IndexedValues<typename P::TV>::value) {
        if (args.xh) return launch_csr_LH<MODE, L, true, P>(ctx, A, args);
    }
    return launch_csr_LH<MODE, L, false, P>(ctx, A, args);
}

template <int MODE, class P>
static int launch_csr_lanes(b200_ctx_t ctx, b200_csr_t A, const CsrArgsT<P> &args) {
    if (ctx->recording) A->in_graph = true;
    ProfScope prof(ctx, MODE, A->nrows, A->ncols, A->nnz, launch_format<P>(ctx, A), (int)sizeof(typename P::TV));
    switch (A->lanes) {
    case 1:  return launch_csr_L<MODE, 1>(ctx, A, args);
    case 2:  return launch_csr_L<MODE, 2>(ctx, A, args);
    case 4:  return launch_csr_L<MODE, 4>(ctx, A, args);
    case 8:  return launch_csr_L<MODE, 8>(ctx, A, args);
    case 16: return launch_csr_L<MODE, 16>(ctx, A, args);
    default: return launch_csr_L<MODE, 32>(ctx, A, args);
    }
}

template <class PI>
static CsrArgsT<PI> indexed_args(b200_csr_t A, const CsrArgsT<PrecDD> &args) {
    CsrArgsT<PI> s;
    static_assert(sizeof(s) == sizeof(args), "indexed arguments differ from PrecDD only in the value type");
    memcpy(&s, &args, sizeof(s));
    s.val = static_cast<const typename PI::TV *>(A->vidx);
    s.vtab = A->vtab;
    s.vtab_n = A->vtab_n;
    return s;
}

template <int MODE, class P>
static int launch_csr(b200_ctx_t ctx, b200_csr_t A, const CsrArgsT<P> &args) {
    if (A->nblocks == 0) return B200_OK;
    if (std::is_same<P, PrecDD>::value && !args.ndot && !args.xh && !args.gather_on &&
        tail_accepts_csr(ctx, A))
        return tail_enqueue_csr(ctx, MODE, A, *reinterpret_cast<const CsrArgsT<PrecDD> *>(&args));
    {
        const int trc = tail_flush(ctx);
        if (trc) return trc;
    }
    if (std::is_same<P, PrecDD>::value && MODE != MODE_RESID_SCALED && !args.ndot && !args.xh &&
        !args.gather_on && small_csr_accepts(ctx, A))
        return small_csr_launch(ctx, MODE, A, *reinterpret_cast<const CsrArgsT<PrecDD> *>(&args));
    if constexpr (std::is_same<P, PrecDD>::value) {
        if (A->val32 && ctx->opt_narrow_values && ctx->opt_spmv_variant == 1) {
            CsrArgsT<PrecSD> s;
            static_assert(sizeof(s) == sizeof(args), "PrecSD arguments differ from PrecDD only in the value type");
            memcpy(&s, &args, sizeof(s));
            s.val = A->val32;
            return launch_csr_lanes<MODE>(ctx, A, s);
        }
        if (A->vidx && ctx->opt_narrow_values && ctx->opt_spmv_variant == 1 &&
            value_index_fits(ctx, A->rows_cap, A->nnz_cap, launch_format<PrecDD>(ctx, A), A->vidx_bytes, A->vtab_n)) {
            if (A->vidx_bytes == 1) return launch_csr_lanes<MODE>(ctx, A, indexed_args<PrecI8D>(A, args));
            return launch_csr_lanes<MODE>(ctx, A, indexed_args<PrecI16D>(A, args));
        }
    }
    return launch_csr_lanes<MODE>(ctx, A, args);
}

template <class P>
static CsrArgsT<P> base_args_t(b200_csr_t A) {
    CsrArgsT<P> a;
    memset(&a, 0, sizeof(a));
    a.ptr = A->ptr; a.ptr16 = A->ptr16; a.col = A->col; a.val = static_cast<const typename P::TV *>(A->val); a.blk = A->blk;
    a.nrows = (int)A->nrows; a.nblocks = (int)A->nblocks;
    a.rows_cap = A->rows_cap; a.nnz_cap = A->nnz_cap; a.row_stream = A->row_stream;
    a.col16 = A->col16; a.wrun = A->wrun; a.wblk = A->wblk; a.run_cap = A->win_runs;
    a.idx8 = A->idx8; a.off_tab = A->off_tab;
    a.pid = A->pid; a.pat_start = A->pat_start; a.pat_off = A->pat_off; a.pat_total = A->pat_total;
    a.clo16 = A->clo16; a.chi8 = A->chi8; a.cbase = A->cbase;
    return a;
}
static CsrArgs base_args(b200_csr_t A) { return base_args_t<PrecDD>(A); }

template <class P>
static int halo_into(b200_ctx_t ctx, b200_csr_t A, CsrArgsT<P> &a) {
    typedef typename P::TX TX;
    HaloArgs h;
    const int rc = halo_exchange(ctx, A, a.x, sizeof(TX), h);
    if (rc) return rc;
    a.xh = static_cast<const TX *>(h.xh); a.nloc = h.nloc;
    a.wait_flags = h.wait_flags; a.wait_mask = h.wait_mask; a.wait_seq = h.wait_seq;
    a.send_idx = h.send_idx; a.n_send = h.n_send; a.nranks = h.nranks;
    for (int q = 0; q < kMaxRanks; ++q) {
        a.push_data[q] = static_cast<TX *>(h.push_data[q]);
        a.push_flag[q] = h.push_flag[q];
    }
    a.push_ticket = h.push_ticket; a.push_seq = h.push_seq;
    return B200_OK;
}


}

extern "C" int b200_csr_create_i64(b200_ctx_t ctx, int64_t nrows, int64_t ncols,
                                   const int64_t *ptr, const int64_t *col, const double *val,
                                   b200_csr_t *A) {
    return csr_create(ctx, nrows, ncols, ptr, col, val, A);
}

extern "C" int b200_csr_create_i32(b200_ctx_t ctx, int64_t nrows, int64_t ncols,
                                   const int32_t *ptr, const int32_t *col, const double *val,
                                   b200_csr_t *A) {
    return csr_create(ctx, nrows, ncols, ptr, col, val, A);
}

extern "C" int b200_csr_create_i64_f32(b200_ctx_t ctx, int64_t nrows, int64_t ncols,
                                       const int64_t *ptr, const int64_t *col, const float *val,
                                       b200_csr_t *A) {
    return csr_create(ctx, nrows, ncols, ptr, col, val, A);
}

extern "C" int b200_csr_create_i32_f32(b200_ctx_t ctx, int64_t nrows, int64_t ncols,
                                       const int32_t *ptr, const int32_t *col, const float *val,
                                       b200_csr_t *A) {
    return csr_create(ctx, nrows, ncols, ptr, col, val, A);
}

extern "C" int b200_csr_dtype(b200_csr_t A, int *dtype) {
    B200_REQUIRE(A && dtype, "null argument");
    *dtype = A->dtype;
    return B200_OK;
}

extern "C" int b200_plan_i64(int64_t nrows, const int64_t *ptr, int lanes, int nnz_cap,
                             int32_t *blk_out, int64_t blk_capacity, int64_t *nblocks,
                             int *lanes_out, int *rows_cap_out, int64_t *nlong_out) {
    B200_REQUIRE(nrows >= 0 && ptr != nullptr && nblocks != nullptr, "bad argument");
    B200_REQUIRE(nnz_cap >= 256 && nnz_cap <= kNnzCapMax && nnz_cap % 8 == 0, "bad nnz_cap");
    B200_REQUIRE(lanes == 0 || (lanes >= 1 && lanes <= 32 && !(lanes & (lanes - 1))), "bad lanes");
    RowBlockPlan plan;
    build_plan(nrows, ptr, lanes, nnz_cap, plan);
    *nblocks = (int64_t)plan.blk.size() - 1;
    if (lanes_out) *lanes_out = plan.lanes;
    if (rows_cap_out) *rows_cap_out = plan.rows_cap;
    if (nlong_out) *nlong_out = plan.nlong;
    if (blk_out) {
        if ((int64_t)plan.blk.size() > blk_capacity)
            return fail(B200_EINVAL, "plan output buffer too small");
        for (size_t i = 0; i < plan.blk.size(); ++i) {
            blk_out[2 * i] = plan.blk[i].x;
            blk_out[2 * i + 1] = plan.blk[i].y;
        }
    }
    return B200_OK;
}

extern "C" int b200_window_plan_i64(int64_t nrows, int64_t ncols, const int64_t *ptr, const int64_t *col,
                                    int lanes, int nnz_cap, int slot_cap, int max_ratio_percent, int gap,
                                    uint16_t *col16_out, int32_t *runs_out, int64_t runs_capacity,
                                    int32_t *blk_out, int64_t blk_capacity, int64_t *nblocks_out,
                                    int64_t *nruns_out, int *max_slots_out, int *max_runs_out, int *qualifies) {
    B200_REQUIRE(nrows >= 0 && ncols >= 0 && ptr && nblocks_out && nruns_out && qualifies, "bad argument");
    B200_REQUIRE(nnz_cap >= 256 && nnz_cap <= kNnzCapMax && nnz_cap % 8 == 0, "bad nnz_cap");
    B200_REQUIRE(lanes == 0 || (lanes >= 1 && lanes <= 32 && !(lanes & (lanes - 1))), "bad lanes");
    int rc = csr_validate(nrows, ncols, ptr, col, true);
    if (rc) return rc;
    RowBlockPlan plan;
    build_plan(nrows, ptr, lanes, nnz_cap, plan);
    int64_t nblocks = (int64_t)plan.blk.size() - 1;
    std::vector<int4> blk4((size_t)nblocks + 1);
    for (int64_t b = 0; b < nblocks; ++b)
        blk4[(size_t)b] = make_int4(plan.blk[(size_t)b].x, plan.blk[(size_t)b + 1].x, plan.blk[(size_t)b].y,
                                    plan.blk[(size_t)b + 1].y);
    const int64_t nnz = nrows ? ptr[nrows] : 0;
    blk4[(size_t)nblocks] = make_int4((int)nrows, (int)nrows, (int)nnz, (int)nnz);
    std::vector<int32_t> hptr((size_t)nrows + 1);
    for (int64_t i = 0; i <= nrows; ++i) hptr[(size_t)i] = (int32_t)ptr[i];
    WindowPlan w;
    const bool ok = plan.nlong == 0 && plan.lanes <= 8 &&
                    build_windows(blk4.data(), nblocks, hptr.data(), col, ncols, nnz, slot_cap,
                                  kWinRunCapMax, max_ratio_percent / 100.0, gap, w);
    if (ok) {
        blk4.swap(w.blk4);
        nblocks = (int64_t)blk4.size() - 1;
    }
    *qualifies = ok ? 1 : 0;
    *nblocks_out = nblocks;
    *nruns_out = ok ? (int64_t)w.runs.size() : 0;
    if (max_slots_out) *max_slots_out = ok ? w.max_slots : 0;
    if (max_runs_out) *max_runs_out = ok ? w.max_runs : 0;
    if (!ok) return B200_OK;
    if (blk_out) {
        B200_REQUIRE(blk_capacity >= nblocks, "block output buffer too small");
        for (int64_t b = 0; b < nblocks; ++b) {
            blk_out[6 * b + 0] = blk4[(size_t)b].x; blk_out[6 * b + 1] = blk4[(size_t)b].y;
            blk_out[6 * b + 2] = blk4[(size_t)b].z; blk_out[6 * b + 3] = blk4[(size_t)b].w;
            blk_out[6 * b + 4] = w.wblk[(size_t)b].x; blk_out[6 * b + 5] = w.wblk[(size_t)b].y;
        }
    }
    if (runs_out) {
        B200_REQUIRE(runs_capacity >= (int64_t)w.runs.size(), "run output buffer too small");
        for (size_t i = 0; i < w.runs.size(); ++i) {
            runs_out[2 * i] = w.runs[i].x;
            runs_out[2 * i + 1] = w.runs[i].y;
        }
    }
    if (col16_out) std::copy(w.col16.begin(), w.col16.end(), col16_out);
    return B200_OK;
}

extern "C" int b200_offset_plan_i64(int64_t nrows, int64_t ncols, const int64_t *ptr, const int64_t *col,
                                    uint8_t *idx8_out, int32_t *tab_out, int *count, int *qualifies) {
    B200_REQUIRE(nrows >= 0 && ncols >= 0 && ptr && qualifies, "bad argument");
    int rc = csr_validate(nrows, ncols, ptr, col, true);
    if (rc) return rc;
    std::vector<int32_t> hptr((size_t)nrows + 1);
    for (int64_t i = 0; i <= nrows; ++i) hptr[(size_t)i] = (int32_t)ptr[i];
    OffsetPlan o;
    const bool ok = build_offsets(nrows, hptr.data(), col, o);
    *qualifies = ok ? 1 : 0;
    if (count) *count = ok ? o.count : 0;
    if (!ok) return B200_OK;
    if (idx8_out) std::copy(o.idx8.begin(), o.idx8.end(), idx8_out);
    if (tab_out) std::copy(o.tab, o.tab + kOffTabLen, tab_out);
    return B200_OK;
}

extern "C" int b200_pattern_plan_i64(int64_t nrows, int64_t ncols, const int64_t *ptr, const int64_t *col,
                                     uint8_t *pid_out, uint16_t *start_out, int32_t *off_out, int *count,
                                     int *total, int *qualifies) {
    B200_REQUIRE(nrows >= 0 && ncols >= 0 && ptr && qualifies, "bad argument");
    int rc = csr_validate(nrows, ncols, ptr, col, true);
    if (rc) return rc;
    std::vector<int32_t> hptr((size_t)nrows + 1);
    for (int64_t i = 0; i <= nrows; ++i) hptr[(size_t)i] = (int32_t)ptr[i];
    PatternPlan o;
    const bool ok = build_patterns(nrows, hptr.data(), col, o);
    *qualifies = ok ? 1 : 0;
    if (count) *count = ok ? o.count : 0;
    if (total) *total = ok ? o.total : 0;
    if (!ok) return B200_OK;
    if (pid_out) std::copy(o.pid.begin(), o.pid.end(), pid_out);
    if (start_out) std::copy(o.start.begin(), o.start.end(), start_out);
    if (off_out) std::copy(o.off.begin(), o.off.end(), off_out);
    return B200_OK;
}

extern "C" int b200_narrow_plan_i64(int64_t nrows, int64_t ncols, const int64_t *ptr, const int64_t *col,
                                    int lanes, int nnz_cap, int32_t *base_out, int64_t base_capacity,
                                    uint16_t *lo16_out, uint8_t *hi8_out, uint16_t *ptr16_out,
                                    int64_t *nblocks_out, int *width_out) {
    B200_REQUIRE(nrows >= 0 && ncols >= 0 && ptr && nblocks_out && width_out, "bad argument");
    B200_REQUIRE(nnz_cap >= 256 && nnz_cap <= kNnzCapMax && nnz_cap % 8 == 0, "bad nnz_cap");
    B200_REQUIRE(lanes == 0 || (lanes >= 1 && lanes <= 32 && !(lanes & (lanes - 1))), "bad lanes");
    int rc = csr_validate(nrows, ncols, ptr, col, true);
    if (rc) return rc;
    RowBlockPlan plan;
    build_plan(nrows, ptr, lanes, nnz_cap, plan);
    const int64_t nblocks = (int64_t)plan.blk.size() - 1;
    std::vector<int4> blk4((size_t)nblocks + 1);
    for (int64_t b = 0; b < nblocks; ++b)
        blk4[(size_t)b] = make_int4(plan.blk[(size_t)b].x, plan.blk[(size_t)b + 1].x, plan.blk[(size_t)b].y,
                                    plan.blk[(size_t)b + 1].y);
    const int64_t nnz = nrows ? ptr[nrows] : 0;
    std::vector<int32_t> hptr((size_t)nrows + 1);
    for (int64_t i = 0; i <= nrows; ++i) hptr[(size_t)i] = (int32_t)ptr[i];
    *nblocks_out = nblocks;
    if (ptr16_out) {
        std::vector<unsigned short> p16((size_t)nrows, 0);
        build_ptr16(blk4.data(), nblocks, hptr.data(), nnz_cap, p16);
        std::copy(p16.begin(), p16.end(), ptr16_out);
    }
    NarrowPlan o;
    const bool ok = plan.nlong == 0 && plan.lanes <= 8 && build_narrow(blk4.data(), nblocks, col, nnz, o);
    *width_out = ok ? o.width : 0;
    if (!ok) return B200_OK;
    if (base_out) {
        B200_REQUIRE(base_capacity >= nblocks, "block output buffer too small");
        std::copy(o.base.begin(), o.base.end(), base_out);
    }
    if (lo16_out) std::copy(o.lo16.begin(), o.lo16.end(), lo16_out);
    if (hi8_out && o.width == 24) std::copy(o.hi8.begin(), o.hi8.end(), hi8_out);
    return B200_OK;
}

extern "C" int b200_ctx_largest_operator(b200_ctx_t ctx, int64_t *nnz, int *format) {
    CHECK_CTX(ctx);
    if (nnz) *nnz = ctx->big_nnz;
    if (format) *format = ctx->big_fmt;
    return B200_OK;
}

extern "C" int b200_csr_patterns(b200_csr_t A, int *pattern_indexed, int *count, int *total) {
    B200_REQUIRE(A, "null argument");
    if (pattern_indexed) *pattern_indexed = A->pid ? 1 : 0;
    if (count) *count = A->pat_count;
    if (total) *total = A->pat_total;
    return B200_OK;
}

extern "C" int b200_csr_offsets(b200_csr_t A, int *offset_indexed, int *count) {
    B200_REQUIRE(A, "null argument");
    if (offset_indexed) *offset_indexed = A->idx8 ? 1 : 0;
    if (count) *count = A->off_count;
    return B200_OK;
}

extern "C" int b200_csr_narrow(b200_csr_t A, int *width) {
    B200_REQUIRE(A && width, "null argument");
    *width = A->narrow;
    return B200_OK;
}

extern "C" int b200_csr_value_bytes(b200_csr_t A, int *bytes) {
    B200_REQUIRE(A && bytes, "null argument");
    *bytes = A->val32 || A->dtype == B200_F32 ? 4 : A->vidx ? A->vidx_bytes : 8;
    return B200_OK;
}

extern "C" int b200_value_index_plan_i64(const double *val, int64_t n, double *table_out, int64_t table_capacity,
                                         void *idx_out, int *count_out, int *width_out) {
    B200_REQUIRE(n >= 0 && (val || n == 0) && count_out && width_out, "bad argument");
    ValueIndexPlan p;
    const bool ok = build_value_index(val, n, p);
    *count_out = p.count;
    *width_out = ok ? p.width : 0;
    if (!ok) return B200_OK;
    if (table_out) {
        B200_REQUIRE(table_capacity >= p.count, "table_out too small");
        memcpy(table_out, p.tab.data(), (size_t)p.count * sizeof(double));
    }
    if (idx_out && n) {
        if (p.width == 8) memcpy(idx_out, p.idx8.data(), (size_t)n);
        else memcpy(idx_out, p.idx16.data(), (size_t)n * 2);
    }
    return B200_OK;
}

extern "C" int b200_values_fit_f32(const double *val, int64_t n, int *qualifies) {
    B200_REQUIRE(n >= 0 && (val || n == 0) && qualifies, "bad argument");
    *qualifies = values_fit_f32(val, n) ? 1 : 0;
    return B200_OK;
}

extern "C" int b200_csr_window(b200_csr_t A, int *windowed, int *max_slots, int *max_runs, int64_t *total_slots) {
    B200_REQUIRE(A, "null argument");
    if (windowed) *windowed = A->col16 ? 1 : 0;
    if (max_slots) *max_slots = A->win_slots;
    if (max_runs) *max_runs = A->win_runs;
    if (total_slots) *total_slots = A->win_total;
    return B200_OK;
}

extern "C" int b200_csr_destroy(b200_csr_t A) {
    if (!A) return B200_OK;
    NOT_RECORDING(A->ctx, "matrix destruction");
    if (A->in_graph) A->ctx->destroy_epoch++;
    GUARD(A->ctx);
    csr_free(A);
    return B200_OK;
}

extern "C" int b200_csr_rows(b200_csr_t A, size_t *n) {
    B200_REQUIRE(A && n, "null argument");
    *n = (size_t)A->gl_rows;
    return B200_OK;
}
extern "C" int b200_csr_cols(b200_csr_t A, size_t *n) {
    B200_REQUIRE(A && n, "null argument");
    *n = (size_t)A->gl_cols;
    return B200_OK;
}
extern "C" int b200_csr_nonzeros(b200_csr_t A, size_t *n) {
    B200_REQUIRE(A && n, "null argument");
    *n = (size_t)A->gl_nnz;
    return B200_OK;
}
extern "C" int b200_csr_bytes(b200_csr_t A, size_t *bytes) {
    B200_REQUIRE(A && bytes, "null argument");
    *bytes = A->bytes;
    return B200_OK;
}
extern "C" int b200_csr_plan(b200_csr_t A, int *lanes_per_row, int64_t *n_blocks,
                             int64_t *n_long_blocks) {
    B200_REQUIRE(A, "null argument");
    if (lanes_per_row) *lanes_per_row = A->lanes;
    if (n_blocks) *n_blocks = A->nblocks;
    if (n_long_blocks) *n_long_blocks = A->nlong;
    return B200_OK;
}

namespace b200 {

struct DotReq {
    int           ndot  = 0;
    const double *w     = nullptr;
    const int    *slots = nullptr;
    unsigned      host_mask = 0;
    bool          done  = false;
};
template <class P>
static void apply_req(b200_ctx_t ctx, b200_csr_t A, CsrArgsT<P> &a, DotReq *req) {
    if (!req || !req->ndot || ctx->opt_spmv_variant != 1 || a.nblocks == 0) return;
    if (!std::is_same<typename P::TY, double>::value) return;
    const bool across = A->rows_dist;
    if (across && !ctx->scal_x_table) return;
    a.ndot = req->ndot;
    a.w = req->w;
    red_out(ctx, req->ndot, req->slots, a.red, across, req->host_mask);
    req->done = true;
}

template <class P>
static int spmv_typed(b200_ctx_t ctx, double alpha, b200_csr_t A, b200_vec_t x, double beta,
                      b200_vec_t y, DotReq *req = nullptr) {
    typedef typename P::TX TX;
    typedef typename P::TY TY;
    CsrArgsT<P> a = base_args_t<P>(A);
    const double *px;
    int rc = rd(x, &px);
    if (rc) return rc;
    a.x = tp<TX>(px);
    a.alpha = alpha; a.beta = beta;
    if (ctx->dist) {
        B200_REQUIRE((x->kind == B200_VK_DIST) == A->cols_dist && (y->kind == B200_VK_DIST) == A->rows_dist,
                     "spmv: vectors are not laid out like the operator (partitioned vs replicated)");
    }
    if (A->kind == B200_CK_HALO) {
        rc = halo_into(ctx, A, a);
        if (rc) return rc;
    }
    if (A->gather_rows) {
        B200_REQUIRE(beta == 0.0 || y->zero_pending, "spmv onto a replicated level needs beta == 0");
        GatherArgs g;
        rc = gather_begin(ctx, A, sizeof(TY), g);
        if (rc) return rc;
        a.gather_on = g.on; a.nranks = ctx->nranks;
        for (int q = 0; q < kMaxRanks; ++q) {
            a.gather_data[q] = static_cast<TY *>(g.data[q]);
            a.gather_flag[q] = g.flag[q];
        }
        a.gather_ticket = g.ticket; a.gather_seq = g.seq;
        a.y = static_cast<TY *>(g.y_local);
        rc = launch_csr<MODE_SPMV>(ctx, A, a);
        if (rc) return rc;
        return gather_end(ctx, A, g, y);
    }
    apply_req(ctx, A, a, req);
    if (beta == 0.0 || y->zero_pending) {
        a.y = tp<TY>(wr(y));
        return launch_csr<MODE_SPMV>(ctx, A, a);
    }
    a.y = tp<TY>(mut(y));
    return launch_csr<MODE_SPMV_ACC>(ctx, A, a);
}

template <class P>
static int residual_typed(b200_ctx_t ctx, b200_vec_t f, b200_csr_t A, b200_vec_t x, b200_vec_t r,
                          DotReq *req = nullptr) {
    CsrArgsT<P> a = base_args_t<P>(A);
    const double *px, *pf;
    int rc = rd(x, &px);
    if (rc) return rc;
    rc = rd(f, &pf);
    if (rc) return rc;
    a.x = tp<typename P::TX>(px);
    a.f = tp<typename P::TF>(pf);
    if (A->kind == B200_CK_HALO) {
        B200_REQUIRE(x->kind == B200_VK_DIST && f->kind == B200_VK_DIST && r->kind == B200_VK_DIST,
                     "residual: vectors must be partitioned like the operator");
        rc = halo_into(ctx, A, a);
        if (rc) return rc;
    }
    a.y = tp<typename P::TY>((f == r) ? mut(r) : wr(r));
    apply_req(ctx, A, a, req);
    return launch_csr<MODE_RESID>(ctx, A, a);
}


}

namespace b200 {
static bool first_sweep_fusable(b200_ctx_t ctx, b200_csr_t A);

static int spmv_impl(b200_ctx_t ctx, double alpha, b200_csr_t A, b200_vec_t x, double beta,
                     b200_vec_t y, DotReq *req) {
    CHECK_CTX(ctx);
    B200_REQUIRE(A && x && y, "null argument");
    touch(ctx, {x, y});
    B200_REQUIRE((int64_t)x->n == A->gl_cols, "spmv: x size != matrix columns");
    B200_REQUIRE((int64_t)y->n == A->gl_rows, "spmv: y size != matrix rows");
    B200_REQUIRE(x != y && (x->ptr != y->ptr || !x->ptr), "spmv: x and y must not alias");
    GUARD_DEFER(ctx);
    TailHold hold(ctx, {x, y});
    if (A->dtype == B200_F32) {
        if (all32({x, y})) return spmv_typed<PrecFF>(ctx, alpha, A, x, beta, y);
        if (all64({x, y})) return spmv_typed<PrecFD>(ctx, alpha, A, x, beta, y, req);
        if (x->dtype == B200_F32 && y->dtype == B200_F64)
            return spmv_typed<PrecFFD>(ctx, alpha, A, x, beta, y);
        return B200_BAD_MIX("spmv");
    }
    if (!all64({x, y})) return B200_BAD_MIX("spmv");
    return spmv_typed<PrecDD>(ctx, alpha, A, x, beta, y, req);
}

static int residual_impl(b200_ctx_t ctx, b200_vec_t f, b200_csr_t A, b200_vec_t x, b200_vec_t r,
                         DotReq *req) {
    CHECK_CTX(ctx);
    B200_REQUIRE(f && A && x && r, "null argument");
    touch(ctx, {f, x, r});
    B200_REQUIRE((int64_t)x->n == A->gl_cols, "residual: x size != matrix columns");
    B200_REQUIRE((int64_t)f->n == A->gl_rows && (int64_t)r->n == A->gl_rows,
                 "residual: rhs/r size != matrix rows");
    B200_REQUIRE(x != r && (x->ptr != r->ptr || !x->ptr), "residual: x and r must not alias");
    B200_REQUIRE(!A->gather_rows && (!ctx->dist || A->gl_rows == A->gl_cols || A->kind == B200_CK_LOCAL),
                 "residual: operator must be square");
    GUARD_RAW(ctx);
    TailHold hold(ctx, {f, x, r});
    if (ctx->lazy_vec) {
        if (ctx->lazy_vec == x && x->sc_fvec == f && f != r && x != r && r->ptr != x->ptr &&
            r->ptr != f->ptr && first_sweep_fusable(ctx, A) && all64({f, x, r}) && (!req || !req->ndot) &&
            r->owned && !r->escaped && f->ptr == x->sc_f && !f->zero_pending) {
            ctx->lazy_vec = nullptr;
            x->scale_pending = false;
            CsrArgs a = base_args(A);
            a.x = x->ptr;
            a.xw = x->ptr;
            a.f = x->sc_f; a.d = x->sc_d; a.alpha = x->sc_omega;
            x->sc_d = x->sc_f = nullptr; x->sc_fvec = nullptr;
            a.y = wr(r);
            ctx->fused_first_sweeps++;
            return launch_csr<MODE_RESID_SCALED>(ctx, A, a);
        }
        const int lrc = lazy_flush(ctx);
        if (lrc) return lrc;
    }
    if (A->dtype == B200_F32) {
        if (all32({f, x, r})) return residual_typed<PrecFF>(ctx, f, A, x, r);
        if (all64({f, x, r})) return residual_typed<PrecFD>(ctx, f, A, x, r, req);
        if (all64({f, x}) && r->dtype == B200_F32) return residual_typed<PrecFDF>(ctx, f, A, x, r);
        return B200_BAD_MIX("residual");
    }
    if (!all64({f, x, r})) return B200_BAD_MIX("residual");
    return residual_typed<PrecDD>(ctx, f, A, x, r, req);
}

int spmv_with_dots(b200_ctx_t ctx, b200_csr_t A, b200_vec_t x, b200_vec_t y, b200_vec_t w, int ndot,
                   const int *slots) {
    DotReq req;
    req.ndot = ndot; req.slots = slots;
    const double *pw = nullptr;
    if (w != y) {
        int rc = rd(w, &pw);
        if (rc) return rc;
    }
    req.w = pw;
    int rc = spmv_impl(ctx, 1.0, A, x, 0.0, y, &req);
    if (rc || req.done) return rc;
    return launch_dot_slots(ctx, y, w, ndot == 2 ? y : nullptr, slots);
}

int residual_with_norm(b200_ctx_t ctx, b200_vec_t f, b200_csr_t A, b200_vec_t x, b200_vec_t r, int slot) {
    DotReq req;
    req.ndot = 1; req.slots = &slot; req.host_mask = 1u;
    int rc = residual_impl(ctx, f, A, x, r, &req);
    if (rc || req.done) return rc;
    return launch_dot_slots(ctx, r, r, nullptr, &slot, 1u);
}
}

extern "C" int b200_spmv(b200_ctx_t ctx, double alpha, b200_csr_t A, b200_vec_t x, double beta,
                         b200_vec_t y) {
    return spmv_impl(ctx, alpha, A, x, beta, y, nullptr);
}

extern "C" int b200_residual(b200_ctx_t ctx, b200_vec_t f, b200_csr_t A, b200_vec_t x,
                             b200_vec_t r) {
    return residual_impl(ctx, f, A, x, r, nullptr);
}

namespace b200 {

template <class TD, class TF, class TX>
static int relax_zero_t(b200_ctx_t ctx, double omega, const double *pd, const double *pf, b200_vec_t x) {
    if (x->len && std::is_same<TD, double>::value && std::is_same<TF, double>::value &&
        std::is_same<TX, double>::value && tail_enabled(ctx) && (int64_t)x->len <= ctx->opt_tail_max_vec &&
        x->kind == B200_VK_LOCAL) {
        const int rc = tail_enqueue_relax_zero(ctx, x->len, omega, pd, pf, wr(x));
        x->zero_pending = false;
        return rc;
    }
    if (x->len) {
        const int trc = tail_flush(ctx);
        if (trc) return trc;
        const int grid = grid_for(ctx, x->len, 2);
        ProfScope prof(ctx, B200_PROF_RELAX_ZERO, (int64_t)x->len, 1, 0);
        B200_CUDA(launch_pdl(ctx, relax_zero_kernel<TD, TF, TX>, dim3(grid), dim3(kThreads), 0, x->len, omega,
                             tp<TD>(pd), tp<TF>(pf), tp<TX>(wr(x))));
        B200_CHECK_LAUNCH();
        ctx->launches++;
    }
    x->zero_pending = false;
    return B200_OK;
}

}

namespace b200 {
int lazy_flush(b200_ctx_t ctx) {
    b200_vec_t v = ctx->lazy_vec;
    if (!v) return B200_OK;
    ctx->lazy_vec = nullptr;
    v->scale_pending = false;
    const double *pd = v->sc_d, *pf = v->sc_f;
    v->sc_d = v->sc_f = nullptr;
    v->sc_fvec = nullptr;
    DeviceGuard guard(ctx->device);
    if (!guard.ok) return fail(B200_ECUDA, "cudaSetDevice failed");
    return relax_zero_t<double, double, double>(ctx, v->sc_omega, pd, pf, v);
// ... 145 lines not shown
```

### amgcl_b200/csrc/common.cuh

```cuda
#pragma once

#include <cuda_runtime.h>
#include <stdint.h>
#include <stddef.h>
#include <string>
#include <vector>

#include "../../include/amgcl_b200.h"
#include "../../include/amgcl_b200_formats.h"
#include "../../include/amgcl_b200_coarse.h"

namespace b200 {

void set_error(const std::string &msg);
int  fail(int code, const std::string &msg);
int  cuda_fail(cudaError_t rc, const char *what, const char *file, int line);

#define B200_CUDA(call)                                                        \
    do {                                                                       \
        cudaError_t rc__ = (call);                                             \
        if (rc__ != cudaSuccess)                                               \
            return ::b200::cuda_fail(rc__, #call, __FILE__, __LINE__);         \
    } while (0)

#define B200_CHECK_LAUNCH()                                                    \
    do {                                                                       \
        cudaError_t rc__ = cudaGetLastError();                                 \
        if (rc__ != cudaSuccess)                                               \
            return ::b200::cuda_fail(rc__, "kernel launch", __FILE__, __LINE__); \
    } while (0)

#define B200_REQUIRE(cond, msg)                                                \
    do {                                                                       \
        if (!(cond)) return ::b200::fail(B200_EINVAL, msg);                    \
    } while (0)

constexpr int kThreads      = 256;
constexpr int kRowsCapMax   = 1024;
constexpr int kNnzCapMax    = 6144;
constexpr int kDotMaxBlocks = 2048;
constexpr int kMaxRed       = 3;
constexpr int kScalSlots    = 256;
struct ScalExchange;

constexpr int kMaxRanks   = 16;
constexpr int kFlagStride = 16;
constexpr size_t kFlagBytes = 2 * kFlagStride * sizeof(unsigned long long);

}

struct b200_graph_s;

struct b200_ctx_s {
    int          device      = 0;
    int          sm_count    = 132;
    cudaStream_t own_stream  = nullptr;
    cudaStream_t stream      = nullptr;
    uint64_t     launches    = 0;

    double       *dot_partial = nullptr;
    unsigned int *dot_ticket  = nullptr;
    double       *dot_result_h = nullptr;
    double       *dot_result_d = nullptr;

    double       *scal_d  = nullptr;
    double       *scal_h  = nullptr;
    double       *scal_hd = nullptr;
    unsigned long long *scal_ready_h  = nullptr;
    unsigned long long *scal_ready_hd = nullptr;
    double       *red_partial = nullptr;
    unsigned int *red_ticket  = nullptr;
    bool          scal_used[b200::kScalSlots] = {};
    unsigned long long scal_seq[b200::kScalSlots] = {};
    b200::ScalExchange  *scal_x_local = nullptr;
    void                *scal_x_peer[16] = {};
    b200::ScalExchange **scal_x_table = nullptr;

    struct Product { b200_vec_t a = nullptr, b = nullptr; uint64_t gen_a = 0, gen_b = 0; int slot = -1; };
    Product       products[4];
    int           product_next = 0;
    int           product_slot0 = -1;
    std::vector<size_t> krylov_sizes;

    b200_vec_t    lazy_vec = nullptr;
    int64_t       opt_fuse_first_sweep = 1;
    uint64_t      fused_first_sweeps = 0;

    void         *tail = nullptr;
    unsigned long long *tail_bar = nullptr;
    unsigned long long  tail_bar_count = 0;
    uint64_t      tail_flushes = 0, tail_commands = 0;
    bool          tail_hold = false;

    void        *stage_host[2]  = {};
    cudaEvent_t  stage_event[2] = {};

    bool                      profiling = false;
    std::vector<cudaEvent_t>  prof_events;
    size_t                    prof_used = 0;
    struct ProfRec { int64_t nrows, ncols, nnz; int mode; size_t ev; int fmt, vbytes; };
    std::vector<ProfRec>      prof_recs;

    bool     dist          = false;
    int      rank          = 0;
    int      nranks        = 1;
    void    *comm          = nullptr;
    int64_t  dist_min_rows = 0;
    double  *dot_dev       = nullptr;
    bool     p2p           = false;
    unsigned int *push_ticket = nullptr;
    unsigned int *gather_ticket = nullptr;
    void    *ipc_dev       = nullptr;
    void    *probe_pb_local = nullptr;
    void    *probe_pb_peer[16] = {};
    std::vector<void *> deferred_free;

    int64_t opt_spmv_variant  = 1;
    int64_t opt_fuse_relax    = 1;
    int64_t opt_zero_shortcut = 1;
    int64_t opt_nnz_cap       = 2048;
    int64_t opt_lanes         = 0;
    int64_t opt_ctas_per_sm   = 4;
    int64_t opt_stages        = 2;
    int64_t opt_p2p           = 1;
    int64_t opt_pdl           = 1;
    int64_t opt_cycle_graph   = 1;
    int64_t opt_graph_pdl     = 1;
    int64_t opt_coarse_tail   = 0;
    int64_t opt_tail_max_nnz  = 1500000;
    int64_t opt_tail_max_vec  = 262144;
    int64_t opt_poll_scalars  = 1;
    int64_t big_nnz = -1;
    int     big_fmt = 0;
    int64_t opt_patterns      = 1;
    int64_t opt_patterns_min_nnz = 1000000;
    int64_t opt_offsets       = 1;
    int64_t opt_offsets_min_nnz = 1000000;
    int64_t opt_narrow        = 1;
    int64_t opt_narrow_values = 1;
    int64_t opt_narrow_values_min_nnz = 1000000;
    int64_t opt_window        = 0;
    int64_t opt_window_min_nnz = 1000000;
    int64_t opt_window_ratio  = 75;
    int64_t opt_window_gap    = 2;
    int64_t opt_window_lanes  = 15;
    int64_t opt_small_kernel_max_nnz = 0;
    int64_t opt_fused_krylov  = 1;

    b200_graph_s *recording   = nullptr;
    std::vector<void *> graph_deferred;
    uint64_t     destroy_epoch = 0;
    uint64_t     option_epoch  = 0;
};

enum { B200_VK_LOCAL = 0, B200_VK_DIST = 1 };

struct b200_vec_s {
    b200_ctx_t ctx   = nullptr;
    double    *ptr   = nullptr;
    int        dtype = B200_F64;
    size_t     esz   = sizeof(double);
    size_t     n     = 0;
    size_t     len   = 0;
    size_t     off   = 0;
    size_t     cap   = 0;
    int        kind  = B200_VK_LOCAL;
    bool       owned = true;
    bool       zero_pending = false;
    bool       in_graph     = false;
    bool       scale_pending = false;
    const double *sc_d = nullptr, *sc_f = nullptr;
    b200_vec_t sc_fvec = nullptr;
    double     sc_omega = 0.0;
    uint64_t   gen          = 0;
    bool       escaped      = false;
};

enum { B200_CK_LOCAL = 0, B200_CK_HALO = 1 };

struct b200_csr_s {
    b200_ctx_t ctx   = nullptr;
    int64_t    nrows = 0, ncols = 0, nnz = 0;
    int        kind    = B200_CK_LOCAL;
    int64_t    gl_rows = 0, gl_cols = 0, gl_nnz = 0;
    bool       rows_dist = false;
    bool       cols_dist = false;
    bool       gather_rows = false;
    int64_t    row_off = 0, row_B = 0;
    int64_t    n_loc   = 0;
    int64_t    S       = 0;
    int64_t    n_send  = 0;
    int       *send_idx = nullptr;
    void      *halo    = nullptr;
    void      *halo_owned = nullptr;
    double    *ybuf    = nullptr;
    void      *pb_local = nullptr;
    void      *pb_peer[16] = {};
    size_t     pb_half  = 0;
    void      *gb_local = nullptr;
    void      *gb_peer[16] = {};
    size_t     gb_half  = 0;
    unsigned long long seq = 0;
    unsigned long long gseq = 0;
    bool       xchg[16] = {};
    int       *ptr   = nullptr;
    int       *col   = nullptr;
    void      *val   = nullptr;
    float     *val32 = nullptr;
    void      *vidx  = nullptr;
    double    *vtab  = nullptr;
    int        vidx_bytes = 0;
    int        vtab_n     = 0;
    int        dtype = B200_F64;
    double    *scratch64 = nullptr;
    bool       in_graph  = false;
    int        lanes    = 1;
    int        rows_cap = 256;
    int        nnz_cap  = 2048;
    int64_t    nblocks  = 0;
    int64_t    nlong    = 0;
    bool       row_stream = false;
    unsigned short *col16 = nullptr;
    int2      *wrun     = nullptr;
    int2      *wblk     = nullptr;
    int        win_slots = 0;
    int        win_runs  = 0;
    int64_t    win_total = 0;
    unsigned char *idx8 = nullptr;
    int       *off_tab  = nullptr;
    int        off_count = 0;
    unsigned char  *pid       = nullptr;
    unsigned short *pat_start = nullptr;
    int            *pat_off   = nullptr;
    int        pat_count = 0, pat_total = 0;
    unsigned short *ptr16 = nullptr;
    int        narrow   = 0;
    unsigned short *clo16 = nullptr;
    unsigned char  *chi8  = nullptr;
    int       *cbase    = nullptr;
    int4      *blk      = nullptr;
    size_t     bytes    = 0;
};

struct b200_index_s {
    b200_ctx_t ctx  = nullptr;
    size_t     n    = 0;
    size_t     range = 0;
    int       *idx  = nullptr;
    void      *stage_d = nullptr;
    bool       in_graph = false;
};

namespace b200 { struct CoarseLu; }

struct b200_coarse_s {
    b200_ctx_t ctx  = nullptr;
    int        kind = B200_COARSE_DENSE;
    b200::CoarseLu *lu = nullptr;
    int        dtype = B200_F64;
    bool       replicated = false;
    double    *gbuf = nullptr;
    int64_t    block = 0;
    int64_t    n    = 0;
    double    *Ainv = nullptr;
    size_t     bytes = 0;
    bool       in_graph = false;
};

namespace b200 {
namespace ptx {

__device__ __forceinline__ uint32_t smem_addr(const void *p) {
    return static_cast<uint32_t>(__cvta_generic_to_shared(p));
}

__device__ __forceinline__ void mbar_init(uint64_t *bar, uint32_t count) {
    asm volatile("mbarrier.init.shared::cta.b64 [%0], %1;" ::"r"(smem_addr(bar)), "r"(count)
                 : "memory");
}

__device__ __forceinline__ void fence_mbar_init() {
    asm volatile("fence.mbarrier_init.release.cluster;" ::: "memory");
}

__device__ __forceinline__ void fence_proxy_async() {
    asm volatile("fence.proxy.async.shared::cta;" ::: "memory");
}

__device__ __forceinline__ void mbar_expect_tx(uint64_t *bar, uint32_t bytes) {
    asm volatile("mbarrier.arrive.expect_tx.shared::cta.b64 _, [%0], %1;" ::"r"(smem_addr(bar)),
                 "r"(bytes)
                 : "memory");
}

__device__ __forceinline__ void mbar_wait(uint64_t *bar, uint32_t parity) {
    asm volatile(
        "{\n"
        ".reg .pred p;\n"
        "B200_WAIT_%=:\n"
        "mbarrier.try_wait.parity.shared::cta.b64 p, [%0], %1;\n"
        "@p bra B200_DONE_%=;\n"
        "bra B200_WAIT_%=;\n"
        "B200_DONE_%=:\n"
        "}\n" ::"r"(smem_addr(bar)),
        "r"(parity)
        : "memory");
}

__device__ __forceinline__ uint64_t policy_evict_first() {
    uint64_t pol;
    asm volatile("createpolicy.fractional.L2::evict_first.b64 %0, 1.0;" : "=l"(pol));
    return pol;
}

__device__ __forceinline__ void bulk_g2s(void *dst, const void *src, uint32_t bytes,
                                         uint64_t *bar, uint64_t policy) {
    asm volatile(
        "cp.async.bulk.shared::cluster.global.mbarrier::complete_tx::bytes.L2::cache_hint "
        "[%0], [%1], %2, [%3], %4;" ::"r"(smem_addr(dst)),
        "l"(src), "r"(bytes), "r"(smem_addr(bar)), "l"(policy)
        : "memory");
}

__device__ __forceinline__ void bulk_g2s(void *dst, const void *src, uint32_t bytes,
                                         uint64_t *bar) {
    asm volatile(
        "cp.async.bulk.shared::cluster.global.mbarrier::complete_tx::bytes "
        "[%0], [%1], %2, [%3];" ::"r"(smem_addr(dst)),
        "l"(src), "r"(bytes), "r"(smem_addr(bar))
        : "memory");
}

__device__ __forceinline__ void pdl_wait() { asm volatile("griddepcontrol.wait;" ::: "memory"); }

__device__ __forceinline__ double2 ld_stream2(const double *p) {
    double2 r;
    asm volatile("ld.global.nc.L1::no_allocate.v2.f64 {%0, %1}, [%2];"
                 : "=d"(r.x), "=d"(r.y)
                 : "l"(p));
    return r;
}

}
}
```

### amgcl_b200/csrc/csr_kernels.cuh

```cuda
#pragma once
#include "common.cuh"
#include "reduce.cuh"
#include <type_traits>

namespace b200 {

enum { FMT_PLAIN = 0,
       FMT_WINDOW = 1,
       FMT_OFFSET = 2,
       FMT_PATTERN = 3,
       FMT_COL16 = 4,
       FMT_COL24 = 5 };
static_assert(FMT_PLAIN == B200_FMT_PLAIN && FMT_WINDOW == B200_FMT_WINDOW && FMT_OFFSET == B200_FMT_OFFSET &&
              FMT_PATTERN == B200_FMT_PATTERN && FMT_COL16 == B200_FMT_COL16 && FMT_COL24 == B200_FMT_COL24,
              "formats as include/amgcl_b200_formats.h reports them");

enum { MODE_SPMV = 0, MODE_SPMV_ACC = 1, MODE_RESID = 2, MODE_RELAX = 3,
       MODE_RESID_SCALED = 4 };

#ifndef B200_GATHER_BATCH
#define B200_GATHER_BATCH 4
#endif
constexpr int kGatherBatch = B200_GATHER_BATCH;

template <class TV_, class TX_, class TF_, class TY_, class TD_>
struct Prec {
    typedef TV_ TV;
    typedef TX_ TX;
    typedef TF_ TF;
    typedef TY_ TY;
    typedef TD_ TD;
};
typedef Prec<double, double, double, double, double> PrecDD;
typedef Prec<float, float, float, float, float>      PrecFF;
typedef Prec<float, double, double, double, float>   PrecFD;
typedef Prec<float, double, double, float, float>    PrecFDF;
typedef Prec<float, float, float, double, float>     PrecFFD;
typedef Prec<float, double, double, double, double>  PrecSD;
typedef Prec<unsigned char, double, double, double, double>  PrecI8D;
typedef Prec<unsigned short, double, double, double, double> PrecI16D;

template <class TV> struct IndexedValues : std::false_type {};
template <> struct IndexedValues<unsigned char> : std::true_type {};
template <> struct IndexedValues<unsigned short> : std::true_type {};

template <class TS, class TV>
__device__ __forceinline__ TS value_of(TV v, const double *vtab) {
    if constexpr (IndexedValues<TV>::value) return (TS)vtab[v];
    else return (TS)v;
}

template <class P>
struct CsrArgsT {
    const int    *ptr;
    const unsigned short *ptr16;
    const int    *col;
    const typename P::TV *val;
    const double *vtab;
    int           vtab_n;
    const int4   *blk;
    int           nrows;
    int           nblocks;
    int           rows_cap;
    int           nnz_cap;
    int           row_stream;
    const typename P::TX *x;
    const typename P::TX *xh;
    int           nloc;
    const unsigned long long *wait_flags;
    unsigned int              wait_mask;
    unsigned long long        wait_seq;
    const int                *send_idx;
    int                       n_send;
    int                       nranks;
    typename P::TX           *push_data[kMaxRanks];
    unsigned long long       *push_flag[kMaxRanks];
    unsigned int             *push_ticket;
    unsigned long long        push_seq;
    int                       gather_on;
    typename P::TY           *gather_data[kMaxRanks];
    unsigned long long       *gather_flag[kMaxRanks];
    unsigned int             *gather_ticket;
    unsigned long long        gather_seq;
    const unsigned short *col16;
    const int2   *wrun;
    const int2   *wblk;
    int           run_cap;
    const unsigned char *idx8;
    const int    *off_tab;
    const unsigned char  *pid;
    const unsigned short *pat_start;
    const int    *pat_off;
    int           pat_total;
    const unsigned short *clo16;
    const unsigned char  *chi8;
    const int    *cbase;
    typename P::TY       *y;
    typename P::TX       *xw;
    const typename P::TF *f;
    const typename P::TD *d;
    double        alpha;
    double        beta;
    int           ndot;
    const double *w;
    RedOut        red;
};
typedef CsrArgsT<PrecDD> CsrArgs;

struct StageLayout {
    int val_off, col_off, hi_off, ptr_off, run_off, pid_off, bytes;
};
__host__ __device__ inline StageLayout stage_layout(int rows_cap, int nnz_cap, int val_size,
                                                    int fmt = FMT_PLAIN, int run_cap = 0) {
    StageLayout s;
    s.val_off = 0;
    int val_bytes = nnz_cap * val_size + 16;
    val_bytes = (val_bytes + 15) & ~15;
    s.col_off = s.val_off + val_bytes;
    const bool narrow = fmt == FMT_COL16 || fmt == FMT_COL24;
    int col_bytes = fmt == FMT_WINDOW || narrow ? (nnz_cap + 16) * 2
                  : fmt == FMT_OFFSET  ? (nnz_cap + 32)
                  : fmt == FMT_PATTERN ? 0
                                       : (nnz_cap + 8) * 4;
    col_bytes = (col_bytes + 15) & ~15;
    s.hi_off = s.col_off + col_bytes;
    int hi_bytes = fmt == FMT_COL24 ? nnz_cap + 32 : 0;
    hi_bytes = (hi_bytes + 15) & ~15;
    s.ptr_off = s.hi_off + hi_bytes;
    int ptr_bytes = (rows_cap + 16) * 2;
    ptr_bytes = (ptr_bytes + 15) & ~15;
    s.run_off = s.ptr_off + ptr_bytes;
    int run_bytes = fmt == FMT_WINDOW ? (run_cap + 2) * 8 : 0;
    run_bytes = (run_bytes + 15) & ~15;
    s.pid_off = s.run_off + run_bytes;
    int pid_bytes = fmt == FMT_PATTERN ? rows_cap + 32 : 0;
    pid_bytes = (pid_bytes + 15) & ~15;
    s.bytes = s.pid_off + pid_bytes;
    return s;
}
constexpr int kMaxStages   = 8;
constexpr int kHeaderBytes = 448;
constexpr int kWinRunLen   = 64;
constexpr int kOffTabLen   = 256;
constexpr int kPatCap      = 256;
constexpr int kPatOffCap   = 1024;
constexpr int kPatTabBytes = kPatOffCap * 4 + ((kPatCap + 1) * 2 + 15) / 16 * 16;
__host__ __device__ constexpr int fmt_table_bytes(int fmt) {
    return fmt == FMT_OFFSET ? kOffTabLen * 4 : fmt == FMT_PATTERN ? kPatTabBytes : 0;
}

struct BlockDesc {
    int r0, r1;
    int e0, e1;
    int halo;
    int q0, q1;
    int cb;
};
static_assert(sizeof(BlockDesc) * kMaxStages <= 384 - 128, "descriptors overflow the header");

template <int FMT = FMT_PLAIN, class P>
__device__ __forceinline__ BlockDesc load_desc(const CsrArgsT<P> &a, int b) {
    const int4 q = __ldg(a.blk + b);
    BlockDesc d;
    d.halo = q.x < 0;
    d.r0 = q.x < 0 ? ~q.x : q.x;
    d.r1 = q.y; d.e0 = q.z; d.e1 = q.w;
    d.q0 = d.q1 = 0; d.cb = 0;
    if (FMT == FMT_WINDOW) {
        const int2 w = __ldg(a.wblk + b);
        d.q0 = w.x; d.q1 = w.y;
    }
    if (FMT == FMT_COL16 || FMT == FMT_COL24) d.cb = __ldg(a.cbase + b);
    return d;
}

template <int FMT = FMT_PLAIN, class P>
__device__ __forceinline__ bool issue_block(const CsrArgsT<P> &a, const BlockDesc &d, char *stage,
                                            const StageLayout &lay, uint64_t *bar,
                                            uint64_t policy) {
    typedef typename P::TV TV;
    constexpr int VA = 16 / (int)sizeof(TV);
    const int nnz = d.e1 - d.e0;
    if (FMT == FMT_PLAIN && nnz > a.nnz_cap) {
        asm volatile("mbarrier.arrive.shared::cta.b64 _, [%0];" ::"r"(ptx::smem_addr(bar))
                     : "memory");
        return false;
    }
    const int a0 = d.e0 & ~(VA - 1);
    const int nval = ((d.e1 - a0) + VA - 1) & ~(VA - 1);
    const int p0 = d.r0 & ~7;
    const int nptr = ((d.r1 + 1 - p0) + 7) & ~7;
    int ncol = 0, nhi = 0, nrun = 0, npid = 0;
    const void *csrc = nullptr, *hsrc = nullptr, *psrc = nullptr;
    if (FMT == FMT_PLAIN) {
        const int c0 = d.e0 & ~3;
        ncol = (((d.e1 - c0) + 3) & ~3) * 4;
        csrc = a.col + c0;
    } else if (FMT == FMT_WINDOW || FMT == FMT_COL16 || FMT == FMT_COL24) {
        const int c0 = d.e0 & ~7;
        ncol = (((d.e1 - c0) + 7) & ~7) * 2;
        csrc = (FMT == FMT_WINDOW ? a.col16 : a.clo16) + c0;
    } else if (FMT == FMT_OFFSET) {
        const int c0 = d.e0 & ~15;
        ncol = ((d.e1 - c0) + 15) & ~15;
        csrc = a.idx8 + c0;
    }
    if (FMT == FMT_COL24) {
        const int h0 = d.e0 & ~15;
        nhi = ((d.e1 - h0) + 15) & ~15;
        hsrc = a.chi8 + h0;
    }
    if (FMT == FMT_WINDOW) {
        const int qa = d.q0 & ~1;
        nrun = (((d.q1 - qa) + 1) & ~1) * 8;
        psrc = a.wrun + qa;
    }
    if (FMT == FMT_PATTERN) {
        const int q0 = d.r0 & ~15;
        npid = ((d.r1 - q0) + 15) & ~15;
        psrc = a.pid + q0;
    }
    const uint32_t bytes = nval * (int)sizeof(TV) + ncol + nhi + nptr * 2 + nrun + npid;
    ptx::mbar_expect_tx(bar, bytes);
    if (nval) ptx::bulk_g2s(stage + lay.val_off, a.val + a0, nval * (int)sizeof(TV), bar, policy);
    if (ncol) ptx::bulk_g2s(stage + lay.col_off, csrc, ncol, bar, policy);
    if (nhi) ptx::bulk_g2s(stage + lay.hi_off, hsrc, nhi, bar, policy);
    ptx::bulk_g2s(stage + lay.ptr_off, a.ptr16 + p0, nptr * 2, bar, policy);
    if (nrun) ptx::bulk_g2s(stage + lay.run_off, psrc, nrun, bar, policy);
    if (npid) ptx::bulk_g2s(stage + lay.pid_off, psrc, npid, bar, policy);
    return true;
}

struct RowAcc { double s0, s1; };

template <class P>
struct RowOps {
    typename P::TF f;
    typename P::TD d;
    typename P::TX x;
    typename P::TY y;
    double         w;
};
template <int MODE, class P>
__device__ __forceinline__ RowOps<P> load_row_ops(const CsrArgsT<P> &a, int r) {
    RowOps<P> o;
    o.f = 0; o.d = 0; o.x = 0; o.y = 0; o.w = 0.0;
    if (MODE == MODE_SPMV_ACC) o.y = a.y[r];
    if (MODE == MODE_RESID || MODE == MODE_RESID_SCALED || MODE == MODE_RELAX) o.f = a.f[r];
    if (MODE == MODE_RESID_SCALED || MODE == MODE_RELAX) o.d = a.d[r];
    if (MODE == MODE_RELAX) o.x = a.x[r];
    if (a.ndot && a.w) o.w = a.w[r];
    return o;
}

template <int MODE, class P>
__device__ __forceinline__ void store_row(const CsrArgsT<P> &a, int r, typename P::TY sum, RowAcc &acc,
                                          const RowOps<P> &o) {
    typedef typename P::TY TY;
    TY out;
    double wv = 0.0;
    if (MODE == MODE_SPMV) {
        out = (TY)(a.alpha * sum);
    } else if (MODE == MODE_SPMV_ACC) {
        out = (TY)(a.alpha * sum + a.beta * o.y);
    } else if (MODE == MODE_RESID) {
        out = (TY)(o.f - sum);
    } else if (MODE == MODE_RESID_SCALED) {
        const typename P::TF fr = o.f;
        out = (TY)(fr - sum);
        a.xw[r] = fma((typename P::TX)(a.alpha * o.d), (typename P::TX)fr, (typename P::TX)0);
    } else {
        const typename P::TF fr = o.f;
        const TY t = (TY)(fr - sum);
        const TY w = (TY)(a.alpha * o.d);
        out = fma(w, t, (TY)o.x);
        wv = (double)fr;
    }
    a.y[r] = out;
    if (a.gather_on) {
#pragma unroll 1
        for (int q = 0; q < a.nranks; ++q)
            if (a.gather_data[q]) a.gather_data[q][r] = out;
    }
    if (a.ndot) {
        const double yv = (double)out;
        if (a.w) wv = o.w;
        else if (MODE != MODE_RELAX) wv = yv;
        acc.s0 = fma(yv, wv, acc.s0);
        if (a.ndot > 1) acc.s1 = fma(yv, yv, acc.s1);
    }
}
template <int MODE, class P>
__device__ __forceinline__ void store_row(const CsrArgsT<P> &a, int r, typename P::TY sum, RowAcc &acc) {
    store_row<MODE>(a, r, sum, acc, load_row_ops<MODE>(a, r));
}

template <bool HALO, class P>
__device__ __forceinline__ typename P::TX gather(const CsrArgsT<P> &a,
                                                 const typename P::TX *__restrict__ x, int c) {
    if (HALO) {
        if (c < a.nloc) return __ldg(x + c);
        return __ldcg(a.xh + (c - a.nloc));
    }
    return __ldg(x + c);
}

template <int MODE, bool HALO, class P>
__device__ __forceinline__ typename P::TX gather_m(const CsrArgsT<P> &a,
                                                   const typename P::TX *__restrict__ x, int c) {
    typedef typename P::TX TX;
    if (MODE == MODE_RESID_SCALED)
        return fma((TX)(a.alpha * __ldg(a.d + c)), (TX)__ldg(a.f + c), (TX)0);
    return gather<HALO>(a, x, c);
}

template <bool HALO, class P>
__device__ __forceinline__ void wait_for_halo(const CsrArgsT<P> &a, const BlockDesc &d) {
    if (!HALO) return;
    if (!d.halo || !a.wait_mask) return;
    if (threadIdx.x == 0) {
        unsigned int m = a.wait_mask;
        while (m) {
            const int q = __ffs(m) - 1;
            m &= m - 1;
            unsigned long long v;
            do {
                asm volatile("ld.acquire.sys.global.u64 %0, [%1];" : "=l"(v) : "l"(a.wait_flags + q) : "memory");
            } while (v < a.wait_seq);
        }
    }
    __syncthreads();
}

template <int MODE, bool HALO, class P>
__device__ __forceinline__ void fill_window(const CsrArgsT<P> &a, const BlockDesc &d, const char *stage,
                                            const StageLayout &lay, typename P::TX *win) {
    const int2 *runs = reinterpret_cast<const int2 *>(stage + lay.run_off) + (d.q0 & 1);
    const int nq   = d.q1 - d.q0;
    const int lane = threadIdx.x & 31;
    const typename P::TX *__restrict__ x = a.x;
    for (int q = threadIdx.x >> 5; q < nq; q += kThreads / 32) {
        const int2 rn   = runs[q];
        const int first = rn.x;
        const int len   = rn.y & 0xffff;
        const int slot  = (int)((unsigned)rn.y >> 16);
#pragma unroll
        for (int i = lane; i < kWinRunLen; i += 32)
            if (i < len) win[slot + i] = gather_m<MODE, HALO>(a, x, first + i);
    }
    __syncthreads();
}

template <int MODE, int L, bool HALO, class P, int FMT = FMT_PLAIN>
__device__ __forceinline__ void compute_staged(const CsrArgsT<P> &a, const BlockDesc &d,
                                               const char *stage, const StageLayout &lay, RowAcc &acc,
                                               const typename P::TX *win = nullptr, const int *off = nullptr,
                                               const unsigned short *pstart = nullptr, int k0 = 0,
                                               const double *vtab = nullptr) {
    constexpr bool WIN = FMT == FMT_WINDOW;
    constexpr bool OFF = FMT == FMT_OFFSET;
    constexpr bool PAT = FMT == FMT_PATTERN;
    constexpr bool NAR = FMT == FMT_COL16 || FMT == FMT_COL24;
    typedef typename P::TV TV;
    typedef typename P::TX TX;
    typedef typename P::TY TS;
    typedef typename std::conditional<WIN || NAR, unsigned short,
                                      typename std::conditional<OFF, unsigned char, int>::type>::type CI;
    static_assert(!((WIN || OFF || PAT || NAR) && L >= 16), "compressed column formats use at most 8 lanes per row");
    const unsigned char *pid_s = reinterpret_cast<const unsigned char *>(stage + lay.pid_off) + (d.r0 & 15);
    constexpr int VA = 16 / (int)sizeof(TV);
    const TV *val_s = reinterpret_cast<const TV *>(stage + lay.val_off);
    const CI     *col_s = reinterpret_cast<const CI *>(stage + lay.col_off);
    const unsigned char  *hi_s  = reinterpret_cast<const unsigned char *>(stage + lay.hi_off);
    const unsigned short *ptr_s = reinterpret_cast<const unsigned short *>(stage + lay.ptr_off) + (d.r0 & 7);
    const int vo = d.e0 & ~(VA - 1);
    const int nr = d.r1 - d.r0;
    const int co = WIN || NAR ? (d.e0 & ~7) : OFF ? (d.e0 & ~15) : (d.e0 & ~3);
    const int ho = d.e0 & ~15;
    auto stored_col = [&](int e) -> int {
        if (!NAR) return col_s[e - co];
        if (FMT == FMT_COL24) return d.cb + ((int)col_s[e - co] | (int)hi_s[e - ho] << 16);
        return d.cb + (int)col_s[e - co];
    };
    auto row_beg = [&](int rr) -> int { return d.e0 + (int)ptr_s[rr]; };
    auto row_end = [&](int rr) -> int { return d.e0 + (int)ptr_s[rr + 1] + (rr + 1 == nr ? d.e1 - d.e0 : 0); };
    constexpr int G = kThreads / L;
    const int c0   = (((int)threadIdx.x >> 5) - k0) & (kThreads / 32 - 1);
    const int g    = (threadIdx.x & 31) / L;
    const int lane = threadIdx.x % L;
    const TX *__restrict__ x = a.x;

    if (L >= 16) {
        constexpr int RU = kGatherBatch;
        for (int base = c0 * (32 / L); base < nr; base += G * RU) {
            int  beg[RU], end[RU], c[RU];
            TV   v[RU];
            TX   xv[RU];
            TS   sum[RU];
            bool rowok[RU], p[RU];
#pragma unroll
            for (int u = 0; u < RU; ++u) {
                const int rr = base + u * G + g;
                rowok[u] = rr < nr;
                beg[u] = rowok[u] ? row_beg(rr) : 0;
                end[u] = rowok[u] ? row_end(rr) : 0;
                sum[u] = 0;
            }
#pragma unroll
            for (int u = 0; u < RU; ++u) {
                const int e = beg[u] + lane;
                p[u] = e < end[u];
                c[u] = p[u] ? stored_col(e) : 0;
                v[u] = p[u] ? val_s[e - vo] : (TV)0;
            }
#pragma unroll
            for (int u = 0; u < RU; ++u) xv[u] = p[u] ? gather_m<MODE, HALO>(a, x, c[u]) : (TX)0;
#pragma unroll
            for (int u = 0; u < RU; ++u)
                if (p[u]) sum[u] = value_of<TS>(v[u], vtab) * (TS)xv[u];
#pragma unroll
            for (int u = 0; u < RU; ++u)
                for (int e = beg[u] + lane + L; e < end[u]; e += L)
                    sum[u] = fma(value_of<TS>(val_s[e - vo], vtab), (TS)gather_m<MODE, HALO>(a, x, stored_col(e)),
                                 sum[u]);
#pragma unroll
            for (int o = L / 2; o > 0; o >>= 1) {
#pragma unroll
                for (int u = 0; u < RU; ++u) sum[u] += __shfl_xor_sync(0xffffffffu, sum[u], o);
            }
#pragma unroll
            for (int u = 0; u < RU; ++u)
                if (rowok[u] && lane == 0) store_row<MODE>(a, d.r0 + base + u * G + g, sum[u], acc);
        }
    } else
    for (int base = c0 * (32 / L); base < nr; base += G) {
        const int  rr    = base + g;
        const bool valid = rr < nr;
        TS sum = 0;
        RowOps<P> ops;
        ops.f = 0; ops.d = 0; ops.x = 0; ops.y = 0; ops.w = 0.0;
        if (valid) {
            if (lane == 0) ops = load_row_ops<MODE>(a, d.r0 + rr);
            const int beg = row_beg(rr);
            const int end = row_end(rr);
            int pb = 0;
            if (PAT) pb = (int)pstart[pid_s[rr]] - beg;
            constexpr int U = (L == 1) ? 2 * kGatherBatch : kGatherBatch;
            for (int e = beg + lane; e < end; e += U * L) {
                int  c[U];
                TX   xv[U];
                bool p[U];
#pragma unroll
                for (int u = 0; u < U; ++u) {
                    const int eu = e + u * L;
                    p[u] = eu < end;
                    if (PAT) c[u] = d.r0 + rr + off[pb + (p[u] ? eu : e)];
                    else c[u] = stored_col(p[u] ? eu : e);
                }
                if (OFF) {
#pragma unroll
                    for (int u = 0; u < U; ++u) c[u] = d.r0 + rr + off[c[u]];
                }
#pragma unroll
                for (int u = 0; u < U; ++u)
                    xv[u] = !p[u] ? (TX)0 : WIN ? win[c[u]] : gather_m<MODE, HALO>(a, x, c[u]);
#pragma unroll
                for (int u = 0; u < U; ++u)
                    if (p[u]) sum = fma(value_of<TS>(val_s[e + u * L - vo], vtab), (TS)xv[u], sum);
            }
        }
        if (L > 1) {
#pragma unroll
            for (int o = L / 2; o > 0; o >>= 1) sum += __shfl_xor_sync(0xffffffffu, sum, o);
        }
        if (valid && lane == 0) store_row<MODE>(a, d.r0 + rr, sum, acc, ops);
    }
}

template <int MODE, bool HALO, class P>
__device__ __forceinline__ void compute_long(const CsrArgsT<P> &a, const BlockDesc &d,
                                             double *red_s , RowAcc &acc) {
    typedef typename P::TX TX;
    typedef typename P::TY TS;
    const TX *__restrict__ x = a.x;
    for (int r = d.r0; r < d.r1; ++r) {
        const int beg = __ldg(a.ptr + r), end = __ldg(a.ptr + r + 1);
        TS sum = 0;
        for (int e = beg + threadIdx.x; e < end; e += kThreads)
            sum = fma(value_of<TS>(__ldg(a.val + e), a.vtab), (TS)gather_m<MODE, HALO>(a, x, __ldg(a.col + e)), sum);
#pragma unroll
        for (int o = 16; o > 0; o >>= 1) sum += __shfl_xor_sync(0xffffffffu, sum, o);
        __syncthreads();
        if ((threadIdx.x & 31) == 0) red_s[threadIdx.x >> 5] = (double)sum;
        __syncthreads();
        if (threadIdx.x == 0) {
            TS tot = 0;
#pragma unroll
            for (int w = 0; w < kThreads / 32; ++w) tot += (TS)red_s[w];
            store_row<MODE>(a, r, tot, acc);
        }
    }
}

__device__ __forceinline__ void xchg_st_release_sys(unsigned long long *p, unsigned long long v) {
    asm volatile("st.release.sys.global.u64 [%0], %1;" ::"l"(p), "l"(v) : "memory");
}
template <class P>
__device__ __forceinline__ void halo_push(const CsrArgsT<P> &a) {
    if (!a.push_seq) return;
    const typename P::TX *__restrict__ x = a.x;
    for (int i = blockIdx.x * kThreads + threadIdx.x; i < a.n_send; i += gridDim.x * kThreads) {
        const typename P::TX v = x[a.send_idx[i]];
#pragma unroll 1
        for (int q = 0; q < a.nranks; ++q)
            if (a.push_data[q]) a.push_data[q][i] = v;
    }
    __threadfence_system();
    __shared__ bool push_last;
    __syncthreads();
    if (threadIdx.x == 0) {
        const unsigned int done = atomicAdd(a.push_ticket, 1u);
        push_last = (done == gridDim.x - 1);
    }
    __syncthreads();
    if (push_last) {
        if (threadIdx.x < a.nranks && a.push_flag[threadIdx.x])
            xchg_st_release_sys(a.push_flag[threadIdx.x], a.push_seq);
        if (threadIdx.x == 0) *a.push_ticket = 0;
    }
}
template <class P>
__device__ __forceinline__ void gather_finish(const CsrArgsT<P> &a) {
    __threadfence_system();
    __shared__ bool gather_last;
    __syncthreads();
    if (threadIdx.x == 0) {
        const unsigned int done = atomicAdd(a.gather_ticket, 1u);
        gather_last = (done == gridDim.x - 1);
    }
    __syncthreads();
    if (gather_last) {
        if (threadIdx.x < a.nranks && a.gather_flag[threadIdx.x])
            xchg_st_release_sys(a.gather_flag[threadIdx.x], a.gather_seq);
        if (threadIdx.x == 0) *a.gather_ticket = 0;
    }
}

template <int MODE, int L, bool HALO, class P>
__global__ void __launch_bounds__(kThreads, 4) csr_block_kernel(const CsrArgsT<P> a) {
    extern __shared__ __align__(128) char smem[];
    uint64_t *bar   = reinterpret_cast<uint64_t *>(smem);
    double   *red_s = reinterpret_cast<double *>(smem + 64);
    char     *stage = smem + kHeaderBytes;
    const StageLayout lay = stage_layout(a.rows_cap, a.nnz_cap, (int)sizeof(typename P::TV));

    const int b = blockIdx.x;
    const BlockDesc d = load_desc(a, b);
    const bool staged = (d.e1 - d.e0) <= a.nnz_cap;
    RowAcc acc = {0.0, 0.0};

    if (staged) {
        if (threadIdx.x == 0) {
            ptx::mbar_init(bar, 1);
            ptx::fence_mbar_init();
            issue_block(a, d, stage, lay, bar, ptx::policy_evict_first());
        }
        __syncthreads();
        ptx::mbar_wait(bar, 0);
        wait_for_halo<HALO>(a, d);
        compute_staged<MODE, L, HALO>(a, d, stage, lay, acc);
    } else {
        wait_for_halo<HALO>(a, d);
        compute_long<MODE, HALO>(a, d, red_s, acc);
    }
}

template <int MODE, int L, bool HALO, class P, int FMT = FMT_PLAIN>
__global__ void __launch_bounds__(kThreads, 4) csr_ring_kernel(const CsrArgsT<P> a, const int nstages) {
    extern __shared__ __align__(128) char smem[];
    uint64_t  *bars  = reinterpret_cast<uint64_t *>(smem);
    double    *red_s = reinterpret_cast<double *>(smem + 64);
    BlockDesc *descs = reinterpret_cast<BlockDesc *>(smem + 128);
    unsigned  *done  = reinterpret_cast<unsigned *>(smem + 384);
    const StageLayout lay = stage_layout(a.rows_cap, a.nnz_cap, (int)sizeof(typename P::TV), FMT, a.run_cap);
    char *stages = smem + kHeaderBytes;
    typename P::TX *win = reinterpret_cast<typename P::TX *>(stages + (size_t)nstages * lay.bytes);
    int *off_s = reinterpret_cast<int *>(stages + (size_t)nstages * lay.bytes);
    unsigned short *pstart_s = reinterpret_cast<unsigned short *>(off_s + kPatOffCap);
    constexpr bool IDX = IndexedValues<typename P::TV>::value;
    static_assert(!(IDX && (HALO || FMT == FMT_WINDOW)), "indexed values: single-GPU, fixed-size tables only");
    double *vtab_s = reinterpret_cast<double *>(stages + (size_t)nstages * lay.bytes + fmt_table_bytes(FMT));

    const int first = blockIdx.x;
    const int step  = gridDim.x;
    const int mine  = (a.nblocks - first + step - 1) / step;
    const uint64_t policy = ptx::policy_evict_first();

    if (threadIdx.x == 0) {
        for (int s = 0; s < nstages; ++s) { ptx::mbar_init(bars + s, 1); done[s] = 0; }
        ptx::fence_mbar_init();
        const int pre = mine < nstages ? mine : nstages;
        for (int i = 0; i < pre; ++i) {
            const BlockDesc d = load_desc<FMT>(a, first + i * step);
            descs[i] = d;
            issue_block<FMT>(a, d, stages + (size_t)i * lay.bytes, lay, bars + i, policy);
        }
    }
    if constexpr (FMT == FMT_OFFSET) {
        static_assert(kOffTabLen == kThreads, "one table entry per thread");
        off_s[threadIdx.x] = __ldg(a.off_tab + threadIdx.x);
    }
    if constexpr (FMT == FMT_PATTERN) {
        for (int i = threadIdx.x; i < a.pat_total; i += kThreads) off_s[i] = __ldg(a.pat_off + i);
        for (int i = threadIdx.x; i <= kPatCap; i += kThreads) pstart_s[i] = __ldg(a.pat_start + i);
    }
    if constexpr (IDX) {
        for (int i = threadIdx.x; i < a.vtab_n; i += kThreads) vtab_s[i] = __ldg(a.vtab + i);
    }
    __syncthreads();
    ptx::pdl_wait();
    if (HALO) halo_push(a);

    const bool decoupled = FMT == FMT_OFFSET || FMT == FMT_PATTERN || (FMT != FMT_WINDOW && a.row_stream);
    constexpr int LS = FMT == FMT_PLAIN || L < 16 ? L : 8;
    RowAcc acc = {0.0, 0.0};
    int k0 = 0;
    int s = 0, parity = 0;
    for (int i = 0; i < mine; ++i) {
        ptx::mbar_wait(bars + s, parity);
        const BlockDesc d = descs[s];
        wait_for_halo<HALO>(a, d);
        const char *stage = stages + (size_t)s * lay.bytes;
        if constexpr (FMT == FMT_WINDOW) {
            fill_window<MODE, HALO>(a, d, stage, lay, win);
            compute_staged<MODE, LS, HALO, P, FMT_WINDOW>(a, d, stage, lay, acc, win);
        } else if (FMT != FMT_PLAIN || (d.e1 - d.e0) <= a.nnz_cap) {
            compute_staged<MODE, LS, HALO, P, FMT>(a, d, stage, lay, acc, nullptr, off_s, pstart_s, k0, vtab_s);
            k0 += (d.r1 - d.r0 + 32 / LS - 1) / (32 / LS);
        } else {
            compute_long<MODE, HALO>(a, d, red_s, acc);
        }
        if (decoupled) {
            __syncwarp();
            if ((threadIdx.x & 31) == 0) {
                __threadfence_block();
                const unsigned arrived = atomicAdd(done + s, 1u);
                if (arrived == kThreads / 32 - 1) {
                    done[s] = 0;
                    __threadfence_block();
                    if (i + nstages < mine) {
                        const BlockDesc n = load_desc<FMT>(a, first + (i + nstages) * step);
                        descs[s] = n;
                        issue_block<FMT>(a, n, stages + (size_t)s * lay.bytes, lay, bars + s, policy);
                    }
                }
            }
        } else {
            __syncthreads();
            if (threadIdx.x == 0 && i + nstages < mine) {
                const BlockDesc n = load_desc<FMT>(a, first + (i + nstages) * step);
                descs[s] = n;
                issue_block<FMT>(a, n, stages + (size_t)s * lay.bytes, lay, bars + s, policy);
            }
        }
        if (++s == nstages) { s = 0; parity ^= 1; }
    }
    if (HALO && a.gather_on) gather_finish(a);
    if (a.ndot) {
        double v[2] = {acc.s0, acc.s1};
        red_finish<2>(a.red, v);
    }
}

template <class TD, class TF, class TX>
__global__ void __launch_bounds__(kThreads) relax_zero_kernel(size_t n, double omega,
                                                              const TD *__restrict__ d,
                                                              const TF *__restrict__ f,
                                                              TX *__restrict__ x) {
    ptx::pdl_wait();
    const size_t stride = (size_t)gridDim.x * blockDim.x;
    for (size_t i = (size_t)blockIdx.x * blockDim.x + threadIdx.x; i < n; i += stride) {
        x[i] = fma((TX)(omega * d[i]), (TX)f[i], (TX)0);
    }
}

}
```

### amgcl_b200/csrc/csr_launch.cuh

```cuda
#pragma once
#include "internal.cuh"
#include "csr_kernels.cuh"

namespace b200 {

inline int ring_budget(int ctas) { return 228 * 1024 / ctas - 1024 - 1536; }

inline int value_table_bytes(int count) { return (count * (int)sizeof(double) + 15) & ~15; }

inline bool value_index_fits(b200_ctx_t ctx, int rows_cap, int nnz_cap, int fmt, int idx_bytes, int count) {
    const StageLayout lay = stage_layout(rows_cap, nnz_cap, idx_bytes, fmt);
    return fmt != FMT_WINDOW && ctx->opt_stages >= 1 &&
           kHeaderBytes + (int)ctx->opt_stages * lay.bytes + fmt_table_bytes(fmt) + value_table_bytes(count) <=
               ring_budget((int)ctx->opt_ctas_per_sm);
}

template <class P>
inline int ring_smem(b200_ctx_t ctx, b200_csr_t A, int fmt, int *stages_out) {
    const StageLayout lay = stage_layout(A->rows_cap, A->nnz_cap, (int)sizeof(typename P::TV), fmt, A->win_runs);
    const int extra = (fmt == FMT_WINDOW ? (int)(((size_t)A->win_slots * sizeof(typename P::TX) + 15) & ~(size_t)15)
                                         : fmt_table_bytes(fmt)) +
                      (IndexedValues<typename P::TV>::value ? value_table_bytes(A->vtab_n) : 0);
    int stages = (int)ctx->opt_stages;
    const int per_cta_budget = ring_budget((int)ctx->opt_ctas_per_sm);
    while (stages > 1 && kHeaderBytes + stages * lay.bytes + extra > per_cta_budget) --stages;
    *stages_out = stages;
    const int smem = kHeaderBytes + stages * lay.bytes + extra;
    return (fmt == FMT_WINDOW && smem > per_cta_budget) ? 0 : smem;
}

template <int MODE, int L, bool HALO, class P, int FMT>
inline int launch_ring_impl(b200_ctx_t ctx, b200_csr_t A, const CsrArgsT<P> &args) {
    int stages = 1;
    const int smem = ring_smem<P>(ctx, A, FMT, &stages);
    static bool attr_set[64] = {};
    if (!attr_set[ctx->device & 63]) {
        cudaFuncAttributes fa;
        B200_CUDA(cudaFuncGetAttributes(&fa, csr_ring_kernel<MODE, L, HALO, P, FMT>));
        B200_CUDA(cudaFuncSetAttribute(csr_ring_kernel<MODE, L, HALO, P, FMT>,
                                       cudaFuncAttributeMaxDynamicSharedMemorySize,
                                       227 * 1024 - (int)fa.sharedSizeBytes));
        attr_set[ctx->device & 63] = true;
    }
    const int64_t cap = (int64_t)ctx->sm_count * ctx->opt_ctas_per_sm;
    const unsigned grid = (unsigned)std::min<int64_t>(A->nblocks, cap);
    B200_CUDA(launch_pdl(ctx, csr_ring_kernel<MODE, L, HALO, P, FMT>, dim3(grid), dim3(kThreads), (size_t)smem,
                         args, stages));
    return B200_OK;
}

template <int MODE, int L, bool HALO, class P>
int launch_ring_win(b200_ctx_t ctx, b200_csr_t A, const CsrArgsT<P> &args);
template <int MODE, int L, bool HALO, class P>
int launch_ring_off(b200_ctx_t ctx, b200_csr_t A, const CsrArgsT<P> &args);
template <int MODE, int L, bool HALO, class P>
int launch_ring_pat(b200_ctx_t ctx, b200_csr_t A, const CsrArgsT<P> &args);
template <int MODE, int L, bool HALO, class P>
int launch_ring_c16(b200_ctx_t ctx, b200_csr_t A, const CsrArgsT<P> &args);
template <int MODE, int L, bool HALO, class P>
int launch_ring_c24(b200_ctx_t ctx, b200_csr_t A, const CsrArgsT<P> &args);

inline int stored_format(b200_csr_t A) {
    if (A->pid) return FMT_PATTERN;
    if (A->idx8) return FMT_OFFSET;
    if (A->col16) return FMT_WINDOW;
    if (A->narrow) return A->narrow == 24 ? FMT_COL24 : FMT_COL16;
    return FMT_PLAIN;
}

template <class P>
inline int launch_format(b200_ctx_t ctx, b200_csr_t A) {
    if (ctx->opt_spmv_variant != 1) return FMT_PLAIN;
    if (A->pid && ctx->opt_patterns && A->lanes <= 4) return FMT_PATTERN;
    if (A->idx8 && ctx->opt_offsets && A->lanes <= 4) return FMT_OFFSET;
    if (A->col16 && ctx->opt_window && A->lanes <= 8 && A->win_runs >= 1) {
        int stages;
        if (ring_smem<P>(ctx, A, FMT_WINDOW, &stages) != 0) return FMT_WINDOW;
    }
    if (A->narrow && ctx->opt_narrow && A->lanes <= 8) return A->narrow == 24 ? FMT_COL24 : FMT_COL16;
    return FMT_PLAIN;
}

}
```

### amgcl_b200/csrc/patterns.cuh

```cuda
#pragma once
#include "common.cuh"
#include "csr_kernels.cuh"

#include <algorithm>
#include <cstdint>
#include <map>
#include <vector>
#include <omp.h>

namespace b200 {

struct PatternPlan {
    std::vector<unsigned char>  pid;
    std::vector<unsigned short> start;
    std::vector<int>            off;
    int count = 0, total = 0;
};

template <class Col>
inline bool build_patterns(int64_t nrows, const int32_t *ptr, const Col *col, PatternPlan &o) {
    const int64_t nnz = nrows ? ptr[nrows] : 0;
    if (nrows <= 0 || nnz <= 0) return false;
    const int nth = std::max(1, omp_get_max_threads());
    typedef std::vector<int> Pat;
    std::vector<std::vector<Pat>> lists((size_t)nth);
    std::vector<int> local((size_t)nrows);
    int bad = 0, used = 1;
#pragma omp parallel num_threads(nth)
    {
        const int tid = omp_get_thread_num(), nt = omp_get_num_threads();
#pragma omp single
        used = nt;
        std::vector<Pat> &list = lists[(size_t)tid];
        std::map<Pat, int> index;
        Pat cur;
        int prev = -1;
        bool fail = false;
        const int64_t lo = nrows * tid / nt, hi = nrows * (tid + 1) / nt;
        for (int64_t r = lo; r < hi && !fail; ++r) {
            const int64_t e0 = ptr[r], e1 = ptr[r + 1];
            const int len = (int)(e1 - e0);
            bool same = prev >= 0 && (int)list[(size_t)prev].size() == len;
            if (same) {
                const Pat &p = list[(size_t)prev];
                for (int k = 0; k < len && same; ++k) same = p[(size_t)k] == (int)((int64_t)col[e0 + k] - r);
            }
            if (!same) {
                if (len > kPatOffCap) { fail = true; break; }
                cur.resize((size_t)len);
                for (int k = 0; k < len; ++k) cur[(size_t)k] = (int)((int64_t)col[e0 + k] - r);
                std::map<Pat, int>::iterator it = index.find(cur);
                if (it == index.end()) {
                    if ((int)list.size() >= kPatCap) { fail = true; break; }
                    prev = (int)list.size();
                    list.push_back(cur);
                    index[cur] = prev;
                } else {
                    prev = it->second;
                }
            }
            local[(size_t)r] = prev;
        }
        if (fail) {
#pragma omp atomic write
            bad = 1;
        }
    }
    if (bad) return false;
    std::map<Pat, int> gindex;
    std::vector<const Pat *> gl;
    std::vector<std::vector<unsigned char>> xlat((size_t)used);
    int total = 0;
    for (int t = 0; t < used; ++t) {
        xlat[(size_t)t].resize(lists[(size_t)t].size());
        for (size_t i = 0; i < lists[(size_t)t].size(); ++i) {
            const Pat &p = lists[(size_t)t][i];
            std::map<Pat, int>::iterator it = gindex.find(p);
            int g;
            if (it == gindex.end()) {
                if ((int)gl.size() >= kPatCap || total + (int)p.size() > kPatOffCap) return false;
                g = (int)gl.size();
                gl.push_back(&p);
                gindex[p] = g;
                total += (int)p.size();
            } else {
                g = it->second;
            }
            xlat[(size_t)t][i] = (unsigned char)g;
        }
    }
    o.count = (int)gl.size();
    o.total = total;
    o.start.assign((size_t)kPatCap + 1, (unsigned short)total);
    o.off.assign((size_t)kPatOffCap, 0);
    int pos = 0;
    for (int g = 0; g < o.count; ++g) {
        o.start[(size_t)g] = (unsigned short)pos;
        std::copy(gl[(size_t)g]->begin(), gl[(size_t)g]->end(), o.off.begin() + pos);
        pos += (int)gl[(size_t)g]->size();
    }
    o.pid.resize((size_t)nrows);
#pragma omp parallel for schedule(static, 1)
    for (int t = 0; t < used; ++t) {
        const int64_t lo = nrows * t / used, hi = nrows * (t + 1) / used;
        const std::vector<unsigned char> &x = xlat[(size_t)t];
        for (int64_t r = lo; r < hi; ++r) o.pid[(size_t)r] = x[(size_t)local[(size_t)r]];
    }
    return true;
}

}
```

### include/amgcl_b200_formats.h

```cpp
#ifndef AMGCL_B200_FORMATS_H
#define AMGCL_B200_FORMATS_H

#include "amgcl_b200.h"

#ifdef __cplusplus
extern "C" {
#endif

#define B200_FMT_PLAIN    0
#define B200_FMT_WINDOW   1
#define B200_FMT_OFFSET   2
#define B200_FMT_PATTERN  3
#define B200_FMT_COL16    4
#define B200_FMT_COL24    5

int b200_csr_narrow(b200_csr_t A, int *width);
int b200_narrow_plan_i64(int64_t nrows, int64_t ncols, const int64_t *ptr, const int64_t *col, int lanes,
                         int nnz_cap, int32_t *base_out, int64_t base_capacity, uint16_t *lo16_out,
                         uint8_t *hi8_out, uint16_t *ptr16_out, int64_t *nblocks_out, int *width_out);

int b200_csr_value_bytes(b200_csr_t A, int *bytes);
int b200_values_fit_f32(const double *val, int64_t n, int *qualifies);
int b200_value_index_plan_i64(const double *val, int64_t n, double *table_out, int64_t table_capacity,
                              void *idx_out, int *count_out, int *width_out);

typedef struct {
    b200_profile_entry entry;
    int                format;
    int                value_bytes;
} b200_profile_format_entry;
int b200_profile_end_formats(b200_ctx_t ctx, b200_profile_format_entry *out, int64_t capacity,
                             int64_t *count);

#ifdef __cplusplus
}
#endif

#endif
```

Measured before the change: 393.8.

## Add pattern-value CSR format storing per-pattern coefficients instead of per-nonzero values

Extends the row-pattern deduplication so that a pattern key includes both column offsets and value bits. Rows with identical stencils and coefficients then share one small table, and the SpMV kernels can skip streaming the per-nonzero value and row-pointer arrays. It also keeps a float32 table when the values are exactly representable. This is meant to cut memory traffic on structured matrices such as Poisson stencils, at the cost of failing to qualify when coefficients vary, and it adds another shared-memory table and more kernel instantiations.

After: 452.7, median of 6. 1.15x the previous value.

```diff
diff --git a/amgcl_b200/__init__.py b/amgcl_b200/__init__.py
--- a/amgcl_b200/__init__.py
+++ b/amgcl_b200/__init__.py
@@ -32,7 +32,7 @@
     _fields_ = [("entry", ProfileEntry), ("format", _c.c_int), ("value_bytes", _c.c_int)]
 
 
-FORMAT_NAMES = ("plain", "window", "offset", "pattern", "col16", "col24")
+FORMAT_NAMES = ("plain", "window", "offset", "pattern", "col16", "col24", "pattern_values")
 
 
 MODE_NAMES = {0: "spmv", 1: "spmv_acc", 2: "residual", 3: "relax", 4: "residual_scaled", 10: "vec1", 11: "vec2",
@@ -127,6 +127,8 @@
         "b200_ctx_largest_operator": [_vp, _P(_i64), _P(_c.c_int)],
         "b200_csr_patterns": [_vp, _P(_c.c_int), _P(_c.c_int), _P(_c.c_int)],
         "b200_pattern_plan_i64": [_i64, _i64, _vp, _vp, _vp, _vp, _vp, _P(_c.c_int), _P(_c.c_int), _P(_c.c_int)],
+        "b200_pattern_value_plan_i64": [_i64, _i64, _vp, _vp, _vp, _vp, _vp, _vp, _vp, _P(_c.c_int), _P(_c.c_int),
+                                        _P(_c.c_int), _P(_c.c_int)],
         "b200_csr_offsets": [_vp, _P(_c.c_int), _P(_c.c_int)],
         "b200_offset_plan_i64": [_i64, _i64, _vp, _vp, _vp, _vp, _P(_c.c_int), _P(_c.c_int)],
         "b200_csr_narrow": [_vp, _P(_c.c_int)],
@@ -559,6 +561,24 @@
     return {"pid": pid[:nrows], "start": start, "off": off, "count": cnt.value, "total": tot.value}
 
 
+def pattern_value_plan(nrows, ncols, ptr, col, val):
+    ptr = np.ascontiguousarray(ptr, dtype=np.int64)
+    col = np.ascontiguousarray(col, dtype=np.int64)
+    val = np.ascontiguousarray(val, dtype=np.float64)
+    pid = np.zeros(max(1, nrows), dtype=np.uint8)
+    start = np.zeros(257, dtype=np.uint16)
+    off = np.zeros(1024, dtype=np.int32)
+    tab = np.zeros(1024, dtype=np.float64)
+    cnt, tot, exact, ok = _c.c_int(), _c.c_int(), _c.c_int(), _c.c_int()
+    _check(lib().b200_pattern_value_plan_i64(nrows, ncols, ptr.ctypes.data, col.ctypes.data, val.ctypes.data,
+                                             pid.ctypes.data, start.ctypes.data, off.ctypes.data, tab.ctypes.data,
+                                             _c.byref(cnt), _c.byref(tot), _c.byref(exact), _c.byref(ok)))
+    if not ok.value:
+        return None
+    return {"pid": pid[:nrows], "start": start, "off": off, "val": tab, "count": cnt.value, "total": tot.value,
+            "exact_f32": bool(exact.value)}
+
+
 def offset_plan(nrows, ncols, ptr, col):
     ptr = np.ascontiguousarray(ptr, dtype=np.int64)
     col = np.ascontiguousarray(col, dtype=np.int64)
diff --git a/amgcl_b200/csrc/api_context.cu b/amgcl_b200/csrc/api_context.cu
--- a/amgcl_b200/csrc/api_context.cu
+++ b/amgcl_b200/csrc/api_context.cu
@@ -77,6 +77,7 @@
     if (const char *e = getenv("B200_POLL_SCALARS")) ctx->opt_poll_scalars = atoi(e) ? 1 : 0;
     if (const char *e = getenv("B200_PATTERNS")) ctx->opt_patterns = atoi(e) ? 1 : 0;
     if (const char *e = getenv("B200_PATTERNS_MIN_NNZ")) ctx->opt_patterns_min_nnz = atoll(e);
+    if (const char *e = getenv("B200_PATTERN_VALUES")) ctx->opt_pattern_values = atoi(e) ? 1 : 0;
     if (const char *e = getenv("B200_OFFSETS")) ctx->opt_offsets = atoi(e) ? 1 : 0;
     if (const char *e = getenv("B200_OFFSETS_MIN_NNZ")) ctx->opt_offsets_min_nnz = atoll(e);
     if (const char *e = getenv("B200_NARROW_COLUMNS")) ctx->opt_narrow = atoi(e) ? 1 : 0;
@@ -291,6 +292,7 @@
     if (!strcmp(key, "small_kernel_max_nnz")) return &ctx->opt_small_kernel_max_nnz;
     if (!strcmp(key, "patterns")) return &ctx->opt_patterns;
     if (!strcmp(key, "patterns_min_nnz")) return &ctx->opt_patterns_min_nnz;
+    if (!strcmp(key, "pattern_values")) return &ctx->opt_pattern_values;
     if (!strcmp(key, "offsets")) return &ctx->opt_offsets;
     if (!strcmp(key, "offsets_min_nnz")) return &ctx->opt_offsets_min_nnz;
     if (!strcmp(key, "narrow_columns")) return &ctx->opt_narrow;
diff --git a/amgcl_b200/csrc/api_matrices.cu b/amgcl_b200/csrc/api_matrices.cu
--- a/amgcl_b200/csrc/api_matrices.cu
+++ b/amgcl_b200/csrc/api_matrices.cu
@@ -173,8 +173,13 @@
     blk4[(size_t)nblocks] = make_int4((int)nrows, (int)nrows, (int)nnz, (int)nnz);
 
     PatternPlan patp;
-    const bool pattern_indexed = ctx->opt_patterns && nnz >= ctx->opt_patterns_min_nnz && nlong == 0 &&
-                                 lanes <= 4 && build_patterns(nrows, hptr.data(), col, patp);
+    const bool pattern_ok = ctx->opt_patterns && nnz >= ctx->opt_patterns_min_nnz && nlong == 0 && lanes <= 4;
+    const bool pattern_values = pattern_ok && ctx->opt_pattern_values && !ctx->dist &&
+                                build_patterns(nrows, hptr.data(), col, patp, val);
+    const bool pattern_indexed = pattern_values || (pattern_ok && build_patterns(nrows, hptr.data(), col, patp));
+    const bool pattern_values32 = pattern_values &&
+        (std::is_same<Val, float>::value ||
+         (patp.val_f32 && ctx->opt_narrow_values && nnz >= ctx->opt_narrow_values_min_nnz));
 
     OffsetPlan offp;
     const bool offset_indexed = !pattern_indexed && ctx->opt_offsets && nnz >= ctx->opt_offsets_min_nnz && nlong == 0 && lanes <= 4 &&
@@ -201,14 +206,16 @@
 
     bool values32 = false;
     if constexpr (std::is_same<Val, double>::value)
-        values32 = ctx->opt_narrow_values && nnz >= ctx->opt_narrow_values_min_nnz && values_fit_f32(val, nnz);
+        values32 = !pattern_values && ctx->opt_narrow_values && nnz >= ctx->opt_narrow_values_min_nnz &&
+                   values_fit_f32(val, nnz);
 
     ValueIndexPlan vip;
     bool indexed = false;
     if constexpr (std::is_same<Val, double>::value) {
         const int fmt = pattern_indexed ? FMT_PATTERN : offset_indexed ? FMT_OFFSET
                       : narrowed ? (nar.width == 24 ? FMT_COL24 : FMT_COL16) : FMT_PLAIN;
-        indexed = !values32 && ctx->opt_narrow_values && nnz > 0 && nnz >= ctx->opt_narrow_values_min_nnz &&
+        indexed = !values32 && !pattern_values && ctx->opt_narrow_values && nnz > 0 &&
+                  nnz >= ctx->opt_narrow_values_min_nnz &&
                   nlong == 0 && !windowed && !ctx->dist && build_value_index(val, nnz, vip) &&
                   value_index_fits(ctx, rows_cap, nnz_cap, fmt, vip.width / 8, vip.count);
     }
@@ -247,6 +254,8 @@
     const size_t tab_bytes = offset_indexed ? kOffTabLen * sizeof(int) : 0;
     const size_t pid_bytes = pattern_indexed ? (((size_t)nrows + 32 + 15) & ~(size_t)15) : 0;
     const size_t pat_bytes = pattern_indexed ? kPatOffCap * sizeof(int) + (kPatCap + 1 + 7) * sizeof(unsigned short) : 0;
+    const size_t pvl_bytes = (pattern_values ? kPatOffCap * sizeof(double) : 0) +
+                             (pattern_values32 ? kPatOffCap * sizeof(float) : 0);
     const size_t p16_bytes = ((size_t)nrows + 16) * sizeof(unsigned short);
     const size_t lo_bytes  = narrowed ? ((size_t)nnz + 16) * sizeof(unsigned short) : 0;
     const size_t hi_bytes  = narrowed && nar.width == 24 ? (((size_t)nnz + 32 + 15) & ~(size_t)15) : 0;
@@ -267,6 +276,8 @@
         if (A->pid) cudaFree(A->pid);
         if (A->pat_start) cudaFree(A->pat_start);
         if (A->pat_off) cudaFree(A->pat_off);
+        if (A->pat_val) cudaFree(A->pat_val);
+        if (A->pat_val32) cudaFree(A->pat_val32);
         if (A->ptr16) cudaFree(A->ptr16);
         if (A->clo16) cudaFree(A->clo16);
         if (A->chi8) cudaFree(A->chi8);
@@ -359,10 +370,18 @@
         A->pat_count = patp.count;
         A->pat_total = patp.total;
     }
+    if (pattern_values) {
+        CSR_CUDA(cudaMalloc(&A->pat_val, kPatOffCap * sizeof(double)));
+        CSR_CUDA(staged_upload(ctx, A->pat_val, patp.val.data(), (size_t)kPatOffCap));
+        if (pattern_values32) {
+            CSR_CUDA(cudaMalloc(&A->pat_val32, kPatOffCap * sizeof(float)));
+            CSR_CUDA(staged_upload(ctx, A->pat_val32, patp.val32.data(), (size_t)kPatOffCap));
+        }
+    }
     CSR_CUDA(cudaStreamSynchronize(ctx->stream));
 #undef CSR_CUDA
     A->bytes = ptr_bytes + col_bytes + val_bytes + v32_bytes + vix_bytes + vtb_bytes + blk_bytes + c16_bytes + run_bytes + wbk_bytes + ix8_bytes +
-               tab_bytes + pid_bytes + pat_bytes + p16_bytes + lo_bytes + hi_bytes + cb_bytes;
+               tab_bytes + pid_bytes + pat_bytes + pvl_bytes + p16_bytes + lo_bytes + hi_bytes + cb_bytes;
     if (nnz > ctx->big_nnz) {
         ctx->big_nnz = nnz;
         ctx->big_fmt = stored_format(A);
@@ -388,6 +407,8 @@
     if (A->pid) cudaFree(A->pid);
     if (A->pat_start) cudaFree(A->pat_start);
     if (A->pat_off) cudaFree(A->pat_off);
+    if (A->pat_val) cudaFree(A->pat_val);
+    if (A->pat_val32) cudaFree(A->pat_val32);
     if (A->ptr16) cudaFree(A->ptr16);
     if (A->clo16) cudaFree(A->clo16);
     if (A->chi8) cudaFree(A->chi8);
@@ -510,6 +531,12 @@
         int rc = B200_OK;
         bool done = false;
         const int fmt = launch_format<P>(ctx, A);
+        if constexpr (L <= 4 && !HALO && !IndexedValues<typename P::TV>::value) {
+            if (fmt == FMT_PATVAL) {
+                rc = launch_ring_pv<MODE, L, P>(ctx, A, args);
+                done = true;
+            }
+        }
         if constexpr (L <= 4) {
             if (fmt == FMT_PATTERN) {
                 rc = launch_ring_pat<MODE, L, HALO, P>(ctx, A, args);
@@ -593,6 +620,14 @@
         !args.gather_on && small_csr_accepts(ctx, A))
         return small_csr_launch(ctx, MODE, A, *reinterpret_cast<const CsrArgsT<PrecDD> *>(&args));
     if constexpr (std::is_same<P, PrecDD>::value) {
+        if (A->pat_val32 && ctx->opt_narrow_values && launch_format<PrecSD>(ctx, A) == FMT_PATVAL) {
+            CsrArgsT<PrecSD> s;
+            static_assert(sizeof(s) == sizeof(args), "PrecSD arguments differ from PrecDD only in the value type");
+            memcpy(&s, &args, sizeof(s));
+            s.val = nullptr;
+            s.pat_val = A->pat_val32;
+            return launch_csr_lanes<MODE>(ctx, A, s);
+        }
         if (A->val32 && ctx->opt_narrow_values && ctx->opt_spmv_variant == 1) {
             CsrArgsT<PrecSD> s;
             static_assert(sizeof(s) == sizeof(args), "PrecSD arguments differ from PrecDD only in the value type");
@@ -619,6 +654,7 @@
     a.col16 = A->col16; a.wrun = A->wrun; a.wblk = A->wblk; a.run_cap = A->win_runs;
     a.idx8 = A->idx8; a.off_tab = A->off_tab;
     a.pid = A->pid; a.pat_start = A->pat_start; a.pat_off = A->pat_off; a.pat_total = A->pat_total;
+    a.pat_val = pattern_values<typename P::TV>(A);
     a.clo16 = A->clo16; a.chi8 = A->chi8; a.cbase = A->cbase;
     return a;
 }
@@ -788,6 +824,29 @@
     return B200_OK;
 }
 
+extern "C" int b200_pattern_value_plan_i64(int64_t nrows, int64_t ncols, const int64_t *ptr, const int64_t *col,
+                                           const double *val, uint8_t *pid_out, uint16_t *start_out,
+                                           int32_t *off_out, double *val_out, int *count, int *total,
+                                           int *exact_f32, int *qualifies) {
+    B200_REQUIRE(nrows >= 0 && ncols >= 0 && ptr && qualifies, "bad argument");
+    int rc = csr_validate(nrows, ncols, ptr, col, val != nullptr);
+    if (rc) return rc;
+    std::vector<int32_t> hptr((size_t)nrows + 1);
+    for (int64_t i = 0; i <= nrows; ++i) hptr[(size_t)i] = (int32_t)ptr[i];
+    PatternPlan o;
+    const bool ok = build_patterns(nrows, hptr.data(), col, o, val);
+    *qualifies = ok ? 1 : 0;
+    if (count) *count = ok ? o.count : 0;
+    if (total) *total = ok ? o.total : 0;
+    if (exact_f32) *exact_f32 = ok && o.val_f32 ? 1 : 0;
+    if (!ok) return B200_OK;
+    if (pid_out) std::copy(o.pid.begin(), o.pid.end(), pid_out);
+    if (start_out) std::copy(o.start.begin(), o.start.end(), start_out);
+    if (off_out) std::copy(o.off.begin(), o.off.end(), off_out);
+    if (val_out) memcpy(val_out, o.val.data(), (size_t)kPatOffCap * sizeof(double));
+    return B200_OK;
+}
+
 extern "C" int b200_narrow_plan_i64(int64_t nrows, int64_t ncols, const int64_t *ptr, const int64_t *col,
                                     int lanes, int nnz_cap, int32_t *base_out, int64_t base_capacity,
                                     uint16_t *lo16_out, uint8_t *hi8_out, uint16_t *ptr16_out,
@@ -856,7 +915,7 @@
 
 extern "C" int b200_csr_value_bytes(b200_csr_t A, int *bytes) {
     B200_REQUIRE(A && bytes, "null argument");
-    *bytes = A->val32 || A->dtype == B200_F32 ? 4 : A->vidx ? A->vidx_bytes : 8;
+    *bytes = A->val32 || A->pat_val32 || A->dtype == B200_F32 ? 4 : A->vidx ? A->vidx_bytes : 8;
     return B200_OK;
 }
 
diff --git a/amgcl_b200/csrc/api_patvals.cu b/amgcl_b200/csrc/api_patvals.cu
--- /dev/null
+++ b/amgcl_b200/csrc/api_patvals.cu
@@ -0,0 +1,37 @@
+#include "csr_launch.cuh"
+
+namespace b200 {
+
+template <int MODE, int L, class P>
+int launch_ring_pv(b200_ctx_t ctx, b200_csr_t A, const CsrArgsT<P> &args) {
+    return launch_ring_impl<MODE, L, false, P, FMT_PATVAL>(ctx, A, args);
+}
+
+#define B200_PV_INST(MODE, P)                                                                        \
+    template int launch_ring_pv<MODE, 1, P>(b200_ctx_t, b200_csr_t, const CsrArgsT<P> &);            \
+    template int launch_ring_pv<MODE, 2, P>(b200_ctx_t, b200_csr_t, const CsrArgsT<P> &);            \
+    template int launch_ring_pv<MODE, 4, P>(b200_ctx_t, b200_csr_t, const CsrArgsT<P> &);
+
+B200_PV_INST(MODE_SPMV, PrecDD)
+B200_PV_INST(MODE_SPMV, PrecFF)
+B200_PV_INST(MODE_SPMV, PrecFD)
+B200_PV_INST(MODE_SPMV, PrecFFD)
+B200_PV_INST(MODE_SPMV_ACC, PrecDD)
+B200_PV_INST(MODE_SPMV_ACC, PrecFF)
+B200_PV_INST(MODE_SPMV_ACC, PrecFD)
+B200_PV_INST(MODE_SPMV_ACC, PrecFFD)
+B200_PV_INST(MODE_RESID, PrecDD)
+B200_PV_INST(MODE_RESID, PrecFF)
+B200_PV_INST(MODE_RESID, PrecFD)
+B200_PV_INST(MODE_RESID, PrecFDF)
+B200_PV_INST(MODE_RESID_SCALED, PrecDD)
+B200_PV_INST(MODE_RELAX, PrecDD)
+B200_PV_INST(MODE_RELAX, PrecFF)
+B200_PV_INST(MODE_RELAX, PrecFD)
+B200_PV_INST(MODE_SPMV, PrecSD)
+B200_PV_INST(MODE_SPMV_ACC, PrecSD)
+B200_PV_INST(MODE_RESID, PrecSD)
+B200_PV_INST(MODE_RESID_SCALED, PrecSD)
+B200_PV_INST(MODE_RELAX, PrecSD)
+
+}
diff --git a/amgcl_b200/csrc/common.cuh b/amgcl_b200/csrc/common.cuh
--- a/amgcl_b200/csrc/common.cuh
+++ b/amgcl_b200/csrc/common.cuh
@@ -134,6 +134,7 @@
     int     big_fmt = 0;
     int64_t opt_patterns      = 1;
     int64_t opt_patterns_min_nnz = 1000000;
+    int64_t opt_pattern_values = 1;
     int64_t opt_offsets       = 1;
     int64_t opt_offsets_min_nnz = 1000000;
     int64_t opt_narrow        = 1;
@@ -233,6 +234,8 @@
     unsigned short *pat_start = nullptr;
     int            *pat_off   = nullptr;
     int        pat_count = 0, pat_total = 0;
+    double         *pat_val   = nullptr;
+    float          *pat_val32 = nullptr;
     unsigned short *ptr16 = nullptr;
     int        narrow   = 0;
     unsigned short *clo16 = nullptr;
diff --git a/amgcl_b200/csrc/csr_kernels.cuh b/amgcl_b200/csrc/csr_kernels.cuh
--- a/amgcl_b200/csrc/csr_kernels.cuh
+++ b/amgcl_b200/csrc/csr_kernels.cuh
@@ -10,9 +10,11 @@
        FMT_OFFSET = 2,
        FMT_PATTERN = 3,
        FMT_COL16 = 4,
-       FMT_COL24 = 5 };
+       FMT_COL24 = 5,
+       FMT_PATVAL = 6 };
 static_assert(FMT_PLAIN == B200_FMT_PLAIN && FMT_WINDOW == B200_FMT_WINDOW && FMT_OFFSET == B200_FMT_OFFSET &&
-              FMT_PATTERN == B200_FMT_PATTERN && FMT_COL16 == B200_FMT_COL16 && FMT_COL24 == B200_FMT_COL24,
+              FMT_PATTERN == B200_FMT_PATTERN && FMT_COL16 == B200_FMT_COL16 && FMT_COL24 == B200_FMT_COL24 &&
+              FMT_PATVAL == B200_FMT_PATVAL,
               "formats as include/amgcl_b200_formats.h reports them");
 
 enum { MODE_SPMV = 0, MODE_SPMV_ACC = 1, MODE_RESID = 2, MODE_RELAX = 3,
@@ -92,6 +94,7 @@
     const unsigned short *pat_start;
     const int    *pat_off;
     int           pat_total;
+    const typename P::TV *pat_val;
     const unsigned short *clo16;
     const unsigned char  *chi8;
     const int    *cbase;
@@ -114,26 +117,27 @@
                                                     int fmt = FMT_PLAIN, int run_cap = 0) {
     StageLayout s;
     s.val_off = 0;
-    int val_bytes = nnz_cap * val_size + 16;
+    const bool patval = fmt == FMT_PATVAL;
+    int val_bytes = patval ? 0 : nnz_cap * val_size + 16;
     val_bytes = (val_bytes + 15) & ~15;
     s.col_off = s.val_off + val_bytes;
     const bool narrow = fmt == FMT_COL16 || fmt == FMT_COL24;
     int col_bytes = fmt == FMT_WINDOW || narrow ? (nnz_cap + 16) * 2
                   : fmt == FMT_OFFSET  ? (nnz_cap + 32)
-                  : fmt == FMT_PATTERN ? 0
+                  : fmt == FMT_PATTERN || patval ? 0
                                        : (nnz_cap + 8) * 4;
     col_bytes = (col_bytes + 15) & ~15;
     s.hi_off = s.col_off + col_bytes;
     int hi_bytes = fmt == FMT_COL24 ? nnz_cap + 32 : 0;
     hi_bytes = (hi_bytes + 15) & ~15;
     s.ptr_off = s.hi_off + hi_bytes;
-    int ptr_bytes = (rows_cap + 16) * 2;
+    int ptr_bytes = patval ? 0 : (rows_cap + 16) * 2;
     ptr_bytes = (ptr_bytes + 15) & ~15;
     s.run_off = s.ptr_off + ptr_bytes;
     int run_bytes = fmt == FMT_WINDOW ? (run_cap + 2) * 8 : 0;
     run_bytes = (run_bytes + 15) & ~15;
     s.pid_off = s.run_off + run_bytes;
-    int pid_bytes = fmt == FMT_PATTERN ? rows_cap + 32 : 0;
+    int pid_bytes = fmt == FMT_PATTERN || patval ? rows_cap + 32 : 0;
     pid_bytes = (pid_bytes + 15) & ~15;
     s.bytes = s.pid_off + pid_bytes;
     return s;
@@ -145,8 +149,9 @@
 constexpr int kPatCap      = 256;
 constexpr int kPatOffCap   = 1024;
 constexpr int kPatTabBytes = kPatOffCap * 4 + ((kPatCap + 1) * 2 + 15) / 16 * 16;
-__host__ __device__ constexpr int fmt_table_bytes(int fmt) {
-    return fmt == FMT_OFFSET ? kOffTabLen * 4 : fmt == FMT_PATTERN ? kPatTabBytes : 0;
+__host__ __device__ constexpr int fmt_table_bytes(int fmt, int val_size) {
+    return fmt == FMT_OFFSET ? kOffTabLen * 4 : fmt == FMT_PATTERN ? kPatTabBytes
+         : fmt == FMT_PATVAL ? kPatTabBytes + kPatOffCap * val_size : 0;
 }
 
 struct BlockDesc {
@@ -186,10 +191,11 @@
                      : "memory");
         return false;
     }
+    constexpr bool PV = FMT == FMT_PATVAL;
     const int a0 = d.e0 & ~(VA - 1);
-    const int nval = ((d.e1 - a0) + VA - 1) & ~(VA - 1);
+    const int nval = PV ? 0 : ((d.e1 - a0) + VA - 1) & ~(VA - 1);
     const int p0 = d.r0 & ~7;
-    const int nptr = ((d.r1 + 1 - p0) + 7) & ~7;
+    const int nptr = PV ? 0 : ((d.r1 + 1 - p0) + 7) & ~7;
     int ncol = 0, nhi = 0, nrun = 0, npid = 0;
     const void *csrc = nullptr, *hsrc = nullptr, *psrc = nullptr;
     if (FMT == FMT_PLAIN) {
@@ -215,7 +221,7 @@
         nrun = (((d.q1 - qa) + 1) & ~1) * 8;
         psrc = a.wrun + qa;
     }
-    if (FMT == FMT_PATTERN) {
+    if (FMT == FMT_PATTERN || PV) {
         const int q0 = d.r0 & ~15;
         npid = ((d.r1 - q0) + 15) & ~15;
         psrc = a.pid + q0;
@@ -225,7 +231,7 @@
     if (nval) ptx::bulk_g2s(stage + lay.val_off, a.val + a0, nval * (int)sizeof(TV), bar, policy);
     if (ncol) ptx::bulk_g2s(stage + lay.col_off, csrc, ncol, bar, policy);
     if (nhi) ptx::bulk_g2s(stage + lay.hi_off, hsrc, nhi, bar, policy);
-    ptx::bulk_g2s(stage + lay.ptr_off, a.ptr16 + p0, nptr * 2, bar, policy);
+    if (nptr) ptx::bulk_g2s(stage + lay.ptr_off, a.ptr16 + p0, nptr * 2, bar, policy);
     if (nrun) ptx::bulk_g2s(stage + lay.run_off, psrc, nrun, bar, policy);
     if (npid) ptx::bulk_g2s(stage + lay.pid_off, psrc, npid, bar, policy);
     return true;
@@ -356,10 +362,12 @@
                                                const char *stage, const StageLayout &lay, RowAcc &acc,
                                                const typename P::TX *win = nullptr, const int *off = nullptr,
                                                const unsigned short *pstart = nullptr, int k0 = 0,
-                                               const double *vtab = nullptr) {
+                                               const double *vtab = nullptr,
+                                               const typename P::TV *pval = nullptr) {
     constexpr bool WIN = FMT == FMT_WINDOW;
     constexpr bool OFF = FMT == FMT_OFFSET;
-    constexpr bool PAT = FMT == FMT_PATTERN;
+    constexpr bool PV  = FMT == FMT_PATVAL;
+    constexpr bool PAT = FMT == FMT_PATTERN || PV;
     constexpr bool NAR = FMT == FMT_COL16 || FMT == FMT_COL24;
     typedef typename P::TV TV;
     typedef typename P::TX TX;
@@ -441,10 +449,10 @@
         ops.f = 0; ops.d = 0; ops.x = 0; ops.y = 0; ops.w = 0.0;
         if (valid) {
             if (lane == 0) ops = load_row_ops<MODE>(a, d.r0 + rr);
-            const int beg = row_beg(rr);
-            const int end = row_end(rr);
+            const int beg = PV ? (int)pstart[pid_s[rr]] : row_beg(rr);
+            const int end = PV ? (int)pstart[pid_s[rr] + 1] : row_end(rr);
             int pb = 0;
-            if (PAT) pb = (int)pstart[pid_s[rr]] - beg;
+            if (PAT && !PV) pb = (int)pstart[pid_s[rr]] - beg;
             constexpr int U = (L == 1) ? 2 * kGatherBatch : kGatherBatch;
             for (int e = beg + lane; e < end; e += U * L) {
                 int  c[U];
@@ -466,7 +474,7 @@
                     xv[u] = !p[u] ? (TX)0 : WIN ? win[c[u]] : gather_m<MODE, HALO>(a, x, c[u]);
 #pragma unroll
                 for (int u = 0; u < U; ++u)
-                    if (p[u]) sum = fma(value_of<TS>(val_s[e + u * L - vo], vtab), (TS)xv[u], sum);
+                    if (p[u]) sum = fma(value_of<TS>(PV ? pval[e + u * L] : val_s[e + u * L - vo], vtab), (TS)xv[u], sum);
             }
         }
         if (L > 1) {
@@ -587,9 +595,13 @@
     typename P::TX *win = reinterpret_cast<typename P::TX *>(stages + (size_t)nstages * lay.bytes);
     int *off_s = reinterpret_cast<int *>(stages + (size_t)nstages * lay.bytes);
     unsigned short *pstart_s = reinterpret_cast<unsigned short *>(off_s + kPatOffCap);
+    typename P::TV *pval_s = reinterpret_cast<typename P::TV *>(stages + (size_t)nstages * lay.bytes + kPatTabBytes);
     constexpr bool IDX = IndexedValues<typename P::TV>::value;
-    static_assert(!(IDX && (HALO || FMT == FMT_WINDOW)), "indexed values: single-GPU, fixed-size tables only");
-    double *vtab_s = reinterpret_cast<double *>(stages + (size_t)nstages * lay.bytes + fmt_table_bytes(FMT));
+    static_assert(!(IDX && (HALO || FMT == FMT_WINDOW || FMT == FMT_PATVAL)),
+                  "indexed values: single-GPU, fixed-size tables only, values streamed");
+    static_assert(!(HALO && FMT == FMT_PATVAL), "value-keyed patterns: single-GPU only");
+    double *vtab_s = reinterpret_cast<double *>(stages + (size_t)nstages * lay.bytes +
+                                                fmt_table_bytes(FMT, (int)sizeof(typename P::TV)));
 
     const int first = blockIdx.x;
     const int step  = gridDim.x;
@@ -610,9 +622,12 @@
         static_assert(kOffTabLen == kThreads, "one table entry per thread");
         off_s[threadIdx.x] = __ldg(a.off_tab + threadIdx.x);
     }
-    if constexpr (FMT == FMT_PATTERN) {
+    if constexpr (FMT == FMT_PATTERN || FMT == FMT_PATVAL) {
         for (int i = threadIdx.x; i < a.pat_total; i += kThreads) off_s[i] = __ldg(a.pat_off + i);
         for (int i = threadIdx.x; i <= kPatCap; i += kThreads) pstart_s[i] = __ldg(a.pat_start + i);
+    }
+    if constexpr (FMT == FMT_PATVAL) {
+        for (int i = threadIdx.x; i < a.pat_total; i += kThreads) pval_s[i] = __ldg(a.pat_val + i);
     }
     if constexpr (IDX) {
         for (int i = threadIdx.x; i < a.vtab_n; i += kThreads) vtab_s[i] = __ldg(a.vtab + i);
@@ -621,7 +636,8 @@
     ptx::pdl_wait();
     if (HALO) halo_push(a);
 
-    const bool decoupled = FMT == FMT_OFFSET || FMT == FMT_PATTERN || (FMT != FMT_WINDOW && a.row_stream);
+    const bool decoupled = FMT == FMT_OFFSET || FMT == FMT_PATTERN || FMT == FMT_PATVAL ||
+                           (FMT != FMT_WINDOW && a.row_stream);
     constexpr int LS = FMT == FMT_PLAIN || L < 16 ? L : 8;
     RowAcc acc = {0.0, 0.0};
     int k0 = 0;
@@ -635,7 +651,7 @@
             fill_window<MODE, HALO>(a, d, stage, lay, win);
             compute_staged<MODE, LS, HALO, P, FMT_WINDOW>(a, d, stage, lay, acc, win);
         } else if (FMT != FMT_PLAIN || (d.e1 - d.e0) <= a.nnz_cap) {
-            compute_staged<MODE, LS, HALO, P, FMT>(a, d, stage, lay, acc, nullptr, off_s, pstart_s, k0, vtab_s);
+            compute_staged<MODE, LS, HALO, P, FMT>(a, d, stage, lay, acc, nullptr, off_s, pstart_s, k0, vtab_s, pval_s);
             k0 += (d.r1 - d.r0 + 32 / LS - 1) / (32 / LS);
         } else {
             compute_long<MODE, HALO>(a, d, red_s, acc);
diff --git a/amgcl_b200/csrc/csr_launch.cuh b/amgcl_b200/csrc/csr_launch.cuh
--- a/amgcl_b200/csrc/csr_launch.cuh
+++ b/amgcl_b200/csrc/csr_launch.cuh
@@ -11,7 +11,7 @@
 inline bool value_index_fits(b200_ctx_t ctx, int rows_cap, int nnz_cap, int fmt, int idx_bytes, int count) {
     const StageLayout lay = stage_layout(rows_cap, nnz_cap, idx_bytes, fmt);
     return fmt != FMT_WINDOW && ctx->opt_stages >= 1 &&
-           kHeaderBytes + (int)ctx->opt_stages * lay.bytes + fmt_table_bytes(fmt) + value_table_bytes(count) <=
+           kHeaderBytes + (int)ctx->opt_stages * lay.bytes + fmt_table_bytes(fmt, idx_bytes) + value_table_bytes(count) <=
                ring_budget((int)ctx->opt_ctas_per_sm);
 }
 
@@ -19,7 +19,7 @@
 inline int ring_smem(b200_ctx_t ctx, b200_csr_t A, int fmt, int *stages_out) {
     const StageLayout lay = stage_layout(A->rows_cap, A->nnz_cap, (int)sizeof(typename P::TV), fmt, A->win_runs);
     const int extra = (fmt == FMT_WINDOW ? (int)(((size_t)A->win_slots * sizeof(typename P::TX) + 15) & ~(size_t)15)
-                                         : fmt_table_bytes(fmt)) +
+                                         : fmt_table_bytes(fmt, (int)sizeof(typename P::TV))) +
                       (IndexedValues<typename P::TV>::value ? value_table_bytes(A->vtab_n) : 0);
     int stages = (int)ctx->opt_stages;
     const int per_cta_budget = ring_budget((int)ctx->opt_ctas_per_sm);
@@ -55,23 +55,39 @@
 int launch_ring_off(b200_ctx_t ctx, b200_csr_t A, const CsrArgsT<P> &args);
 template <int MODE, int L, bool HALO, class P>
 int launch_ring_pat(b200_ctx_t ctx, b200_csr_t A, const CsrArgsT<P> &args);
+template <int MODE, int L, class P>
+int launch_ring_pv(b200_ctx_t ctx, b200_csr_t A, const CsrArgsT<P> &args);
 template <int MODE, int L, bool HALO, class P>
 int launch_ring_c16(b200_ctx_t ctx, b200_csr_t A, const CsrArgsT<P> &args);
 template <int MODE, int L, bool HALO, class P>
 int launch_ring_c24(b200_ctx_t ctx, b200_csr_t A, const CsrArgsT<P> &args);
 
 inline int stored_format(b200_csr_t A) {
-    if (A->pid) return FMT_PATTERN;
+    if (A->pid) return A->pat_val ? FMT_PATVAL : FMT_PATTERN;
     if (A->idx8) return FMT_OFFSET;
     if (A->col16) return FMT_WINDOW;
     if (A->narrow) return A->narrow == 24 ? FMT_COL24 : FMT_COL16;
     return FMT_PLAIN;
 }
 
+template <class TV>
+inline const TV *pattern_values(b200_csr_t A) {
+    if constexpr (std::is_same<TV, double>::value) return A->pat_val;
+    else if constexpr (std::is_same<TV, float>::value) return A->pat_val32;
+    else return nullptr;
+}
+
 template <class P>
 inline int launch_format(b200_ctx_t ctx, b200_csr_t A) {
     if (ctx->opt_spmv_variant != 1) return FMT_PLAIN;
-    if (A->pid && ctx->opt_patterns && A->lanes <= 4) return FMT_PATTERN;
+    if (A->pid && ctx->opt_patterns && A->lanes <= 4) {
+        const int vs = (int)sizeof(typename P::TV);
+        if (pattern_values<typename P::TV>(A) && ctx->opt_pattern_values && ctx->opt_stages >= 1 &&
+            kHeaderBytes + (int)ctx->opt_stages * stage_layout(A->rows_cap, A->nnz_cap, vs, FMT_PATVAL).bytes +
+                    fmt_table_bytes(FMT_PATVAL, vs) <= ring_budget((int)ctx->opt_ctas_per_sm))
+            return FMT_PATVAL;
+        return FMT_PATTERN;
+    }
     if (A->idx8 && ctx->opt_offsets && A->lanes <= 4) return FMT_OFFSET;
     if (A->col16 && ctx->opt_window && A->lanes <= 8 && A->win_runs >= 1) {
         int stages;
diff --git a/amgcl_b200/csrc/patterns.cuh b/amgcl_b200/csrc/patterns.cuh
--- a/amgcl_b200/csrc/patterns.cuh
+++ b/amgcl_b200/csrc/patterns.cuh
@@ -4,7 +4,9 @@
 
 #include <algorithm>
 #include <cstdint>
+#include <cstring>
 #include <map>
+#include <utility>
 #include <vector>
 #include <omp.h>
 
@@ -15,14 +17,25 @@
     std::vector<unsigned short> start;
     std::vector<int>            off;
     int count = 0, total = 0;
+    bool                        values = false;
+    std::vector<double>         val;
+    std::vector<float>          val32;
+    bool                        val_f32 = false;
 };
 
-template <class Col>
-inline bool build_patterns(int64_t nrows, const int32_t *ptr, const Col *col, PatternPlan &o) {
+inline uint64_t pattern_value_bits(const double *v) { uint64_t b; memcpy(&b, v, 8); return b; }
+inline uint64_t pattern_value_bits(const float *v) { uint32_t b; memcpy(&b, v, 4); return b; }
+
+template <class Col, class Val = double>
+inline bool build_patterns(int64_t nrows, const int32_t *ptr, const Col *col, PatternPlan &o,
+                           const Val *val = nullptr) {
     const int64_t nnz = nrows ? ptr[nrows] : 0;
     if (nrows <= 0 || nnz <= 0) return false;
     const int nth = std::max(1, omp_get_max_threads());
-    typedef std::vector<int> Pat;
+    typedef std::vector<std::pair<int, uint64_t>> Pat;
+    auto entry = [&](int64_t r, int64_t e) -> std::pair<int, uint64_t> {
+        return std::make_pair((int)((int64_t)col[e] - r), val ? pattern_value_bits(val + e) : (uint64_t)0);
+    };
     std::vector<std::vector<Pat>> lists((size_t)nth);
     std::vector<int> local((size_t)nrows);
     int bad = 0, used = 1;
@@ -43,12 +56,12 @@
             bool same = prev >= 0 && (int)list[(size_t)prev].size() == len;
             if (same) {
                 const Pat &p = list[(size_t)prev];
-                for (int k = 0; k < len && same; ++k) same = p[(size_t)k] == (int)((int64_t)col[e0 + k] - r);
+                for (int k = 0; k < len && same; ++k) same = p[(size_t)k] == entry(r, e0 + k);
             }
             if (!same) {
                 if (len > kPatOffCap) { fail = true; break; }
                 cur.resize((size_t)len);
-                for (int k = 0; k < len; ++k) cur[(size_t)k] = (int)((int64_t)col[e0 + k] - r);
+                for (int k = 0; k < len; ++k) cur[(size_t)k] = entry(r, e0 + k);
                 std::map<Pat, int>::iterator it = index.find(cur);
                 if (it == index.end()) {
                     if ((int)list.size() >= kPatCap) { fail = true; break; }
@@ -93,11 +106,34 @@
     o.total = total;
     o.start.assign((size_t)kPatCap + 1, (unsigned short)total);
     o.off.assign((size_t)kPatOffCap, 0);
+    o.values = val != nullptr;
+    o.val.assign(o.values ? (size_t)kPatOffCap : 0, 0.0);
+    o.val32.assign(o.values ? (size_t)kPatOffCap : 0, 0.0f);
+    o.val_f32 = o.values;
     int pos = 0;
     for (int g = 0; g < o.count; ++g) {
         o.start[(size_t)g] = (unsigned short)pos;
-        std::copy(gl[(size_t)g]->begin(), gl[(size_t)g]->end(), o.off.begin() + pos);
-        pos += (int)gl[(size_t)g]->size();
+        for (const std::pair<int, uint64_t> &p : *gl[(size_t)g]) {
+            o.off[(size_t)pos] = p.first;
+            if (o.values) {
+                if (sizeof(Val) == 8) {
+                    double d;
+                    memcpy(&d, &p.second, 8);
+                    const float f = (float)d;
+                    const double w = (double)f;
+                    o.val[(size_t)pos] = d;
+                    o.val32[(size_t)pos] = f;
+                    o.val_f32 = o.val_f32 && memcmp(&w, &d, 8) == 0;
+                } else {
+                    const uint32_t b = (uint32_t)p.second;
+                    float f;
+                    memcpy(&f, &b, 4);
+                    o.val[(size_t)pos] = (double)f;
+                    o.val32[(size_t)pos] = f;
+                }
+            }
+            ++pos;
+        }
     }
     o.pid.resize((size_t)nrows);
 #pragma omp parallel for schedule(static, 1)
diff --git a/include/amgcl_b200_formats.h b/include/amgcl_b200_formats.h
--- a/include/amgcl_b200_formats.h
+++ b/include/amgcl_b200_formats.h
@@ -13,6 +13,11 @@
 #define B200_FMT_PATTERN  3
 #define B200_FMT_COL16    4
 #define B200_FMT_COL24    5
+#define B200_FMT_PATVAL   6
+
+int b200_pattern_value_plan_i64(int64_t nrows, int64_t ncols, const int64_t *ptr, const int64_t *col,
+                                const double *val, uint8_t *pid_out, uint16_t *start_out, int32_t *off_out,
+                                double *val_out, int *count, int *total, int *exact_f32, int *qualifies);
 
 int b200_csr_narrow(b200_csr_t A, int *width);
 int b200_narrow_plan_i64(int64_t nrows, int64_t ncols, const int64_t *ptr, const int64_t *col, int lanes,
```
